# darioShar/DLPM

Hardware: AMD Instinct MI355X
Metric: samples/sec at T=1000 (CIFAR-10 32x32, alpha=1.7) (higher is better)
Workload: dtype f32 (1x1 / stride-2 convolutions: fp32 operands split exactly into 3 bf16 planes, bf16 MFMA products, fp32 accumulate)

## Files before the change

### dlpm_amd/_lib.py

```python
import ctypes as C
import os

_HERE = os.path.dirname(os.path.abspath(__file__))
LIB_PATH = os.environ.get('DLPM_LIB') or os.path.join(_HERE, 'lib', 'libdlpm_amd.so')

vp, i32, i64, u32, u64, f32, f64 = C.c_void_p, C.c_int32, C.c_int64, C.c_uint32, C.c_uint64, C.c_float, C.c_double

ABI_VERSION = 6
UPD_DLIM, UPD_CLIP, UPD_ADVANCE, SMP_NO_FUSED_MLP, UPD_ELEMENTWISE, SMP_LIM = 1, 2, 4, 8, 16, 32
MEAN_TYPES = {'EPSILON': 0, 'START_X': 1, 'Z': 2, 'PREVIOUS_X': 3}
PRED_TO_XSTART, PRED_CLIP, PRED_TO_EPS, PRED_ELEMENTWISE = 1, 2, 4, 16
CONV_AUTO, CONV_F4, CONV_F2, CONV_IGEMM = 0, 1, 2, 3
GEMM_AUTO, GEMM_F32, GEMM_BF16X3 = 0, 1, 2


class MT19937(C.Structure):
    _fields_ = [('key', u32 * 624), ('pos', i32), ('has_cached', i32), ('cached', f64)]


class UpdateArgs(C.Structure):
    _fields_ = [('x_dev', vp), ('eps_dev', vp), ('z_dev', vp), ('t_dev', vp), ('g_dev', vp), ('bg_dev', vp),
                ('bs_dev', vp), ('c_eps_dev', vp), ('c_noise_dev', vp), ('A_dev', vp), ('B', i64), ('D', i64),
                ('T', i32), ('flags', i32), ('dlim_eta', f32), ('alpha', f32), ('seed', u64), ('sample_offset', i64), ('key_dev', vp),
                ('hist_pp', vp)]


class PredictArgs(C.Structure):
    _fields_ = [('x_dev', vp), ('in_dev', vp), ('out_dev', vp), ('t_dev', vp), ('g_dev', vp), ('bg_dev', vp), ('bs_dev', vp),
                ('c_eps_dev', vp), ('A_dev', vp), ('B', i64), ('D', i64), ('T', i32), ('mean_type', i32), ('flags', i32)]


class LimUpdateArgs(C.Structure):
    _fields_ = [('x_dev', vp), ('eps_dev', vp), ('z_dev', vp), ('t_dev', vp), ('tmp_dev', vp), ('cx_dev', vp),
                ('cs_dev', vp), ('cn_dev', vp), ('A_dev', vp), ('B', i64), ('D', i64), ('T', i32), ('flags', i32),
                ('clamp_eps', f32), ('seed', u64), ('sample_offset', i64), ('key_dev', vp), ('hist_pp', vp)]


class UNetConfig(C.Structure):
    _fields_ = [('in_channels', i32), ('model_channels', i32), ('out_channels', i32), ('num_res_blocks', i32),
                ('num_heads', i32), ('image_size', i32), ('n_mult', i32), ('channel_mult', i32 * 8), ('n_attn', i32),
                ('attention_resolutions', i32 * 8)]


class ConvArgs(C.Structure):
    _fields_ = [('src0', vp), ('src1', vp), ('C0', i32), ('C1', i32), ('B', i32), ('Hin', i32), ('Win', i32),
                ('Hout', i32), ('Wout', i32), ('ksize', i32), ('stride', i32), ('upsample', i32), ('weight', vp),
                ('bias', vp), ('coefA', vp), ('coefB', vp), ('act_silu', i32), ('res0', vp), ('res1', vp), ('R0', i32),
                ('out', vp), ('Cout', i32), ('in_nchw', i32), ('out_nchw', i32), ('force_direct', i32), ('scratch_floats', i64)]


class ResBlockArgs(C.Structure):
    _fields_ = [('x0', vp), ('x1', vp), ('C0', i32), ('C1', i32), ('B', i32), ('H', i32), ('W', i32), ('gn1_w', vp), ('gn1_b', vp),
                ('conv1_w', vp), ('conv1_b', vp), ('ss', vp), ('ss_stride', i64), ('gn2_w', vp), ('gn2_b', vp), ('conv2_w', vp),
                ('conv2_b', vp), ('skip_w', vp), ('skip_b', vp), ('out', vp), ('stats_out', vp)]


class AttnBlockArgs(C.Structure):
    _fields_ = [('x', vp), ('C', i32), ('heads', i32), ('B', i32), ('H', i32), ('W', i32), ('gn_w', vp), ('gn_b', vp),
                ('qkv_w', vp), ('qkv_b', vp), ('proj_w', vp), ('proj_b', vp), ('out', vp), ('stats_out', vp)]


class SamplerConfig(C.Structure):
    _fields_ = [('unet', vp), ('mlp', vp), ('B', i64), ('C', i32), ('H', i32), ('W', i32), ('T', i32), ('alpha', f64),
                ('clamp_a', f64), ('clamp_eps', f64), ('flags', i32), ('dlim_eta', f32), ('seed', u64),
                ('sample_offset', i64), ('use_graph', i32), ('g', vp), ('bg', vp), ('s', vp), ('bs', vp),
                ('lim_ts', vp), ('lim_tmp', vp), ('lim_cx', vp), ('lim_cs', vp), ('lim_cn', vp), ('in_scale', vp),
                ('mean_type', i32)]


SIGNATURES = {
    'dlpm_last_error': (C.c_char_p, []),
    'dlpm_abi_version': (C.c_int, []),
    'dlpm_prof_enable': (C.c_int, [C.c_int]),
    'dlpm_prof_report': (C.c_int, [C.c_char_p, i64]),
    'dlpm_schedule_f32': (C.c_int, [C.c_int, f64, vp, vp, vp, vp]),
    'dlpm_schedule_exploding_f32': (C.c_int, [C.c_int, f64, vp, vp, vp, vp]),
    'dlpm_mt19937_seed': (C.c_int, [C.POINTER(MT19937), u32]),
    'dlpm_skewed_levy_host_f32': (C.c_int, [C.POINTER(MT19937), f64, i64, f64, vp]),
    'dlpm_randn_host_f32': (C.c_int, [C.POINTER(MT19937), i64, vp]),
    'dlpm_skewed_levy_philox_f32': (C.c_int, [vp, C.c_int, i64, f64, f64, u64, i64, vp]),
    'dlpm_skewed_levy_elem_philox_f32': (C.c_int, [vp, C.c_int, i64, i64, f64, f64, u64, i64, vp]),
    'dlpm_init_state_elem_philox_f32': (C.c_int, [vp, i64, i64, f64, f64, f32, u64, i64, vp]),
    'dlpm_init_state_philox_f32': (C.c_int, [vp, i64, i64, f64, f64, f32, u64, i64, vp]),
    'dlpm_coeff_tables_f32': (C.c_int, [vp, vp, vp, vp, C.c_int, i64, vp, vp, vp, vp]),
    'dlpm_update_f32': (C.c_int, [C.POINTER(UpdateArgs), vp]),
    'dlpm_predict_f32': (C.c_int, [C.POINTER(PredictArgs), vp]),
    'dlpm_fill_scaled_t_f32': (C.c_int, [vp, vp, i32, i64, vp]),
    'dlpm_postprocess_f32': (C.c_int, [vp, vp, i64, f32, C.c_int, vp]),
    'dlpm_scale_by_table_f32': (C.c_int, [vp, vp, i64, vp, vp, vp]),
    'dlpm_lim_tables_f32': (C.c_int, [f64, i32, i32, vp, vp, vp, vp, vp]),
    'dlpm_lim_update_f32': (C.c_int, [C.POINTER(LimUpdateArgs), vp]),
    'dlpm_fill_table_t_f32': (C.c_int, [vp, vp, vp, i32, i64, vp]),
    'dlpm_images_to_rgb8': (C.c_int, [vp, vp, i64, i32, i32, i32, vp]),
    'dlpm_png_bound': (i64, [i32, i32]),
    'dlpm_png_encode_rgb8': (C.c_int, [vp, i32, i32, i32, vp, i64, C.POINTER(i64)]),
    'dlpm_png_write_rgb8': (C.c_int, [vp, i64, i32, i32, C.c_char_p, i64, i32, i32]),
    'dlpm_unet_create': (C.c_int, [C.POINTER(UNetConfig), C.POINTER(vp)]),
    'dlpm_unet_set_param': (C.c_int, [vp, C.c_char_p, vp, i64]),
    'dlpm_unet_num_params': (C.c_int, [vp]),
    'dlpm_unet_param_key': (C.c_char_p, [vp, C.c_int, C.POINTER(i64)]),
    'dlpm_unet_finalize': (C.c_int, [vp]),
    'dlpm_unet_workspace_bytes': (i64, [vp, i64]),
    'dlpm_unet_forward': (C.c_int, [vp, vp, vp, vp, i64, vp, i64, vp]),
    'dlpm_unet_forward_uniform_t': (C.c_int, [vp, vp, vp, vp, i64, vp, i64, vp]),
    'dlpm_unet_forward_update': (C.c_int, [vp, vp, vp, C.POINTER(UpdateArgs), vp, i64, vp, i64, vp]),
    'dlpm_unet_time_embedding_width': (i64, [vp]),
    'dlpm_unet_time_embeddings_scratch_bytes': (i64, [vp, i64]),
    'dlpm_unet_time_embeddings': (C.c_int, [vp, vp, i64, vp, vp, i64, vp]),
    'dlpm_unet_bind_time_table': (C.c_int, [vp, vp, vp]),
    'dlpm_unet_keep_features': (C.c_int, [vp, C.c_int]),
    'dlpm_unet_num_features': (C.c_int, [vp]),
    'dlpm_unet_feature_shape': (C.c_int, [vp, C.c_int, C.POINTER(i32), C.POINTER(i32), C.POINTER(i32)]),
    'dlpm_unet_get_feature': (C.c_int, [vp, C.c_int, vp, i64, vp]),
    'dlpm_unet_flops_per_sample': (i64, [vp]),
    'dlpm_unet_set_conv_policy': (C.c_int, [vp, i32, i64]),
    'dlpm_unet_set_gemm_policy': (C.c_int, [vp, i32]),
    'dlpm_unet_plan_version': (i64, [vp]),
    'dlpm_unet_destroy': (None, [vp]),
    'dlpm_mlp_create': (C.c_int, [i32, i32, i32, i32, C.POINTER(vp)]),
    'dlpm_mlp_set_param': (C.c_int, [vp, C.c_char_p, vp, i64]),
    'dlpm_mlp_finalize': (C.c_int, [vp]),
    'dlpm_mlp_forward': (C.c_int, [vp, vp, vp, vp, i64, vp]),
    'dlpm_mlp_sample_steps_f32': (C.c_int, [vp, vp, vp, vp, vp, i32, i64, i32, i32, u64, i64, vp, vp]),
    'dlpm_mlp_destroy': (None, [vp]),
    'dlpm_conv2d_f32': (C.c_int, [C.POINTER(ConvArgs), vp, vp]),
    'dlpm_groupnorm_coeffs_f32': (C.c_int, [vp, vp, i32, i32, i32, i32, i32, vp, vp, vp, i64, i64, vp, vp, vp]),
    'dlpm_attention_f32': (C.c_int, [vp, vp, i32, i32, i32, i32, vp]),
    'dlpm_resblock_small_f32': (C.c_int, [C.POINTER(ResBlockArgs), vp, i64, vp]),
    'dlpm_resblock_img_f32': (C.c_int, [C.POINTER(ResBlockArgs), vp, i64, vp]),
    'dlpm_resblock_img_scratch_floats': (i64, [i64, i32]),
    'dlpm_attnblock_small_f32': (C.c_int, [C.POINTER(AttnBlockArgs), vp, i64, vp]),
    'dlpm_timestep_embedding_f32': (C.c_int, [vp, vp, i64, i32, vp]),
    'dlpm_nchw_to_nhwc_f32': (C.c_int, [vp, vp, i32, i32, i32, i32, vp]),
    'dlpm_nhwc_to_nchw_f32': (C.c_int, [vp, vp, i32, i32, i32, i32, vp]),
    'dlpm_sampler_create': (C.c_int, [C.POINTER(SamplerConfig), C.POINTER(vp)]),
    'dlpm_sampler_reseed': (C.c_int, [vp, u64, i64]),
    'dlpm_sampler_begin': (C.c_int, [vp, vp]),
    'dlpm_sampler_begin_injected': (C.c_int, [vp, vp, vp, vp]),
    'dlpm_sampler_set_state': (C.c_int, [vp, vp, i32, vp]),
    'dlpm_sampler_step_injected': (C.c_int, [vp, vp, vp]),
    'dlpm_sampler_steps': (C.c_int, [vp, i32, vp]),
    'dlpm_sampler_set_history': (C.c_int, [vp, vp, vp]),
    'dlpm_sampler_copy_state': (C.c_int, [vp, vp, vp]),
    'dlpm_sampler_state': (vp, [vp]),
    'dlpm_sampler_t': (i32, [vp]),
    'dlpm_sampler_table': (vp, [vp, C.c_int]),
    'dlpm_sampler_destroy': (None, [vp]),
}

_lib = None


class DlpmError(RuntimeError):
    pass


def lib():
    global _lib
    if _lib is None:
        if not os.path.exists(LIB_PATH):
            raise DlpmError('libdlpm_amd.so is missing at %s -- run `python -m dlpm_amd.build` '
                            '(or __graft_entry__.build()); there is no CPU fallback' % LIB_PATH)
        handle = C.CDLL(LIB_PATH)
        for name, (res, args) in SIGNATURES.items():
            fn = getattr(handle, name)
            fn.restype = res
            fn.argtypes = args
        got = handle.dlpm_abi_version()
        if got != ABI_VERSION:
            raise DlpmError('libdlpm_amd.so has ABI version %d, the Python mirror expects %d -- rebuild with '
                            '`python -m dlpm_amd.build`' % (got, ABI_VERSION))
        _lib = handle
    return _lib


def check(rc):
    if rc != 0:
        msg = lib().dlpm_last_error().decode('utf-8', 'replace')
        if rc == -1:
            raise ValueError(msg)
        raise DlpmError('[dlpm status %d] %s' % (rc, msg))


def stream_ptr():
    import torch
    return torch.cuda.current_stream().cuda_stream


def ptr(t):
    if t is None:
        return None
    import torch
    assert t.is_contiguous(), 'non-contiguous tensor crossing the C ABI'
    assert t.dtype in (torch.float32, torch.int32), t.dtype
    return t.data_ptr()
```

### dlpm_amd/csrc/conv.h

```cpp
#pragma once
#include "common.h"

namespace dlpm {

struct ConvLaunch {
    const float *src0 = nullptr, *src1 = nullptr;
    int C0 = 0, C1 = 0;
    int B = 0, Hin = 0, Win = 0, Hout = 0, Wout = 0;
    int ks = 1, stride = 1, ups = 0;
    const float *w = nullptr;
    const float *w_frag = nullptr;
    const float *w_wino = nullptr;
    const float *w_wino4 = nullptr;
    const float *w_wino4_n64 = nullptr, *w_wino4_n32 = nullptr;
    const void *w_split = nullptr;
    const float *w_small = nullptr;
    const float *w_taps = nullptr;
    const float *w_hfused = nullptr;
    const float *bias = nullptr;
    const float *coefA = nullptr, *coefB = nullptr;
    int act_silu = 0;
    const float *res0 = nullptr, *res1 = nullptr;
    int R0 = 0;
    float *out = nullptr;
    int Cout = 0;
    int in_nchw = 0, out_nchw = 0;
    int ws_gemm = 0;
    int abl = 0;
    int gen = 0;
    int64_t dispatch_B = 0;
    int gemm = 0;
    int ksplit = 0;
    int pers_total = 0;
    float2 *stats_out = nullptr;
#ifdef DLPM_PHASE_TIMING
    unsigned long long *phase = nullptr;
#endif
};

bool igemm_supported(const ConvLaunch &c);
int launch_conv_igemm(const ConvLaunch &c, hipStream_t st);
int launch_conv_direct(const ConvLaunch &c, hipStream_t st);
int launch_conv_stem(const ConvLaunch &c, hipStream_t st);
struct HeadUpdate {
    float *x = nullptr;
    const float *z = nullptr;
    const int32_t *t = nullptr;
    const float *g = nullptr, *c_eps = nullptr, *c_noise = nullptr;
    const uint64_t *key = nullptr;
    uint64_t seed = 0;
    int64_t sample_offset = 0;
    float *const *hist_pp = nullptr;
    float *eps_out = nullptr;
    int32_t T = 0;
    int64_t B = 0;
};
bool head_conv_ok(const ConvLaunch &c);
int launch_conv_head(const ConvLaunch &c, const HeadUpdate *hu, hipStream_t st);
int relayout_weight_head(const float *oihw_dev, float *dst_dev, int Cout, int Cin, hipStream_t st);
bool head_gemm_ok(const ConvLaunch &c);
int head_taps_rows(int Cout);
int64_t head_gemm_scratch_floats(const ConvLaunch &c);
int launch_conv_head_gemm(const ConvLaunch &c, const HeadUpdate *hu, float *P, hipStream_t st);
int relayout_weight_head_taps(const float *oihw_dev, float *dst_dev, int Cout, int Cin, hipStream_t st);
bool head_fused_ok(const ConvLaunch &c);
int64_t head_fused_weight_floats(int Cin);
int relayout_weight_head_fused(const float *oihw_dev, float *dst_dev, int Cout, int Cin, hipStream_t st);
int launch_conv_head_fused(const ConvLaunch &c, const HeadUpdate *hu, hipStream_t st);
bool wino_geometry(const ConvLaunch &c, int *bh, int *bw, int *nimg);
int wino_tiles(const ConvLaunch &c);
int launch_conv_wino(const ConvLaunch &c, hipStream_t st);
int64_t wino_weight_floats(int Cout, int Cin);
int relayout_weight_wino(const float *oihw_dev, float *dst_dev, int Cout, int Cin, hipStream_t st);
bool wino4_enabled();
bool wino4_vsplit();
bool wino4_image_stats(int cout);
bool wino4_geometry(const ConvLaunch &c, int *bh, int *bw, int *nimg);
bool wino4_preferred(const ConvLaunch &c, int *bh, int *bw, int *nimg);
int launch_conv_wino4(const ConvLaunch &c, hipStream_t st);
int64_t wino4_weight_floats(int Cout, int Cin);
int relayout_weight_wino4(const float *oihw_dev, float *dst_dev, int Cout, int Cin, hipStream_t st, int nq = 0);
struct ResImgLaunch {
    const float *x0 = nullptr, *x1 = nullptr;
    int C0 = 0, C1 = 0, B = 0;
    int H = 32;
    const float2 *st0 = nullptr, *st1 = nullptr;
    int nt0 = 1, nt1 = 1;
    const float *coefA1 = nullptr, *coefB1 = nullptr;
    const float *gn1_w = nullptr, *gn1_b = nullptr, *gn2_w = nullptr, *gn2_b = nullptr;
    const float *w1 = nullptr, *b1 = nullptr;
    const float *w2 = nullptr, *b2 = nullptr;
    const float *emb = nullptr;
    int64_t emb_stride = 0;
    int emb_off = 0;
    const float *res = nullptr;
    float *hbuf = nullptr;
    float *out = nullptr;
    float2 *stats_out = nullptr;
#ifdef DLPM_PHASE_TIMING
    unsigned long long *phase = nullptr;
#endif
};
bool res_img_ok(const ResImgLaunch &r);
int launch_resblock_img(const ResImgLaunch &r, hipStream_t st);

bool conv_split_ok(const ConvLaunch &c);
int launch_conv_split(const ConvLaunch &c, hipStream_t st);
int64_t split_weight_floats(int Cout, int Cin, int taps);
int relayout_weight_split(const float *oihw_dev, void *dst_dev, int Cout, int Cin, int taps, hipStream_t st);
int conv_stats_pixels(const ConvLaunch &c);
int conv_ksplit_for(const ConvLaunch &c);
int wino4_launch_nq(const ConvLaunch &c);
int64_t wino_grid_at(const ConvLaunch &c, int64_t B);
int wino_chunk_channels(const ConvLaunch &c);
int launch_splitk_reduce(const float *part, int S, int64_t npix, int Cout, const float *bias, const float *res0, const float *res1, int R0,
                         float *out, hipStream_t st);
inline int launch_conv_fallback(const ConvLaunch &L, hipStream_t st) {
    if (L.in_nchw && !L.out_nchw && L.ks == 3 && L.stride == 1 && !L.ups && L.C1 == 0 && L.Cout % 4 == 0 && !L.coefA &&
        !L.act_silu && !L.res0 && L.bias)
        return launch_conv_stem(L, st);
    return launch_conv_direct(L, st);
}

int relayout_weight(const float *oihw_dev, float *dst_dev, int Cout, int Cin, int ks, bool for_igemm, hipStream_t st);
int64_t frag_weight_floats(int Cout, int Cin, int taps = 9);
int relayout_weight_frag(const float *oihw_dev, float *dst_dev, int Cout, int Cin, hipStream_t st, int taps = 9);

int launch_gn_coeffs(const float *src0, const float *src1, int C0, int C1, int B, int HW, int groups,
                     const float *gamma, const float *beta, const float *ss, int64_t ss_stride, int64_t ss_offset,
                     float *coefA, float *coefB, hipStream_t st);
int launch_gn_coeffs_from_stats(const float2 *st0, const float2 *st1, int C0, int C1, int B, int nt0, int nt1, int HW, int groups,
                                const float *gamma, const float *beta, const float *ss, int64_t ss_stride,
                                int64_t ss_offset, float *coefA, float *coefB, hipStream_t st);
int launch_attention(const float *qkv, float *out, int B, int T, int C, int heads, hipStream_t st);

struct ResSmallLaunch {
    const float *x0 = nullptr, *x1 = nullptr;
    int C0 = 0, C1 = 0, B = 0, H = 0, W = 0;
    const float *gn1_w = nullptr, *gn1_b = nullptr, *gn2_w = nullptr, *gn2_b = nullptr;
    const float *w1f = nullptr, *b1 = nullptr;
    const float *w2f = nullptr, *b2 = nullptr;
    const float *wsf = nullptr, *bs = nullptr;
    const float *emb = nullptr;
    int64_t emb_stride = 0;
    int emb_off = 0;
    float *out = nullptr;
    float2 *stats_out = nullptr;
};
struct AttnSmallLaunch {
    const float *x = nullptr;
    int C = 0, heads = 0, B = 0, H = 0, W = 0;
    const float *gn_w = nullptr, *gn_b = nullptr;
    const float *wqkv = nullptr, *bqkv = nullptr;
    const float *wproj = nullptr, *bproj = nullptr;
    float *out = nullptr;
    float2 *stats_out = nullptr;
#ifdef DLPM_PHASE_TIMING
    unsigned long long *phase = nullptr;
#endif
};
bool attn_small_ok(const AttnSmallLaunch &a);
int launch_attnblock_small(const AttnSmallLaunch &a, hipStream_t st);
bool attn16_ok(const AttnSmallLaunch &a);
int launch_attnblock16(const AttnSmallLaunch &a, hipStream_t st);
bool gnqkv_small_ok(const AttnSmallLaunch &a);
int launch_gnqkv_small(const AttnSmallLaunch &a, hipStream_t st);
bool small_blocks_enabled();
bool small_weight_ok(int Cout, int Cin, int ks);
int64_t small_weight_floats(int Cout, int Cin, int ks);
int relayout_weight_small(const float *oihw_dev, float *dst_dev, int Cout, int Cin, int ks, hipStream_t st);
bool res_small_ok(const ResSmallLaunch &r);
int launch_resblock_small(const ResSmallLaunch &r, hipStream_t st);
int launch_timestep_embedding(const float *t, float *emb, int64_t B, int dim, hipStream_t st);

__device__ __forceinline__ float silu_f(float v) {
    return v * __builtin_amdgcn_rcpf(1.0f + __expf(-v));
}

}
```

### dlpm_amd/csrc/conv_igemm.hip

```cpp
#include <cstdlib>

#include <algorithm>

#include "conv.h"
#include "igemm_epilogue.h"

namespace dlpm {
namespace {

constexpr int KC = 32;
constexpr int LDS_LD = 36;

template <int BN, int WAVES_M, int WAVES_N, int RM, int RN>
__device__ __forceinline__ void epilogue_rows(const ConvLaunch &p, floatx16 (&acc)[RM][RN], float *lds, int64_t m0, int n0,
                                              int64_t M, int tid, int wm, int wn, int l31, int kh) {
    constexpr int LD = BN + 4, PR = RM * 32, C4 = BN / 4, RG = 256 / C4;
    const int R1 = p.Cout - p.R0;
    const bool do_stats = p.stats_out != nullptr;
    float4 K = make_float4(0.f, 0.f, 0.f, 0.f), s1 = K, s2 = K;
    int cnt = 0;
    for (int ph = 0; ph < WAVES_M; ph++) {
        if (wm == ph) {
#pragma unroll
            for (int i = 0; i < RM; i++)
// ... 719 lines not shown
    const float4 bias = reinterpret_cast<const float4 *>(p.bias)[nq];
    const int64_t m_lo = (int64_t)blockIdx.x * ppb;
    const bool do_stats = p.stats_out != nullptr;
    float4 K = make_float4(0.f, 0.f, 0.f, 0.f), s1 = K, s2 = K;
    for (int it = 0; it < ppb / pl_n; it++) {
        const int64_t m = m_lo + it * pl_n + pl;
        if (m >= M) break;
        const int b = (int)(m / HWo);
        const int rem = (int)(m - (int64_t)b * HWo);
        const int oy = rem / p.Wout, ox = rem - oy * p.Wout;
        float v[9 * CIN];
#pragma unroll
        for (int ky = 0; ky < 3; ky++)
#pragma unroll
            for (int kx = 0; kx < 3; kx++) {
                const int iy = oy + ky - 1, ix = ox + kx - 1;
                const bool ok = iy >= 0 && iy < p.Hin && ix >= 0 && ix < p.Win;
                const int cy = min(max(iy, 0), p.Hin - 1), cx = min(max(ix, 0), p.Win - 1);
#pragma unroll
                for (int c = 0; c < CIN; c++) {
                    const float x = p.src0[(((int64_t)b * CIN + c) * p.Hin + cy) * p.Win + cx];
                    v[(ky * 3 + kx) * CIN + c] = ok ? x : 0.f;
                }
            }
        float4 acc = bias;
#pragma unroll
        for (int k = 0; k < 9 * CIN; k++) {
            acc.x = fmaf(v[k], w[k].x, acc.x);
            acc.y = fmaf(v[k], w[k].y, acc.y);
            acc.z = fmaf(v[k], w[k].z, acc.z);
            acc.w = fmaf(v[k], w[k].w, acc.w);
        }
        reinterpret_cast<float4 *>(p.out + m * p.Cout)[nq] = acc;
        if (do_stats) {
            if (it == 0) K = acc;
            float d;
            d = acc.x - K.x; s1.x += d; s2.x = fmaf(d, d, s2.x);
            d = acc.y - K.y; s1.y += d; s2.y = fmaf(d, d, s2.y);
            d = acc.z - K.z; s1.z += d; s2.z = fmaf(d, d, s2.z);
            d = acc.w - K.w; s1.w += d; s2.w = fmaf(d, d, s2.w);
        }
    }
    if (do_stats) {
        __shared__ float2 part[1024];
        const float fc = (float)(ppb / pl_n);
        const float mx = s1.x / fc, my = s1.y / fc, mz = s1.z / fc, mw = s1.w / fc;
        part[pl * p.Cout + nq * 4 + 0] = make_float2(K.x + mx, fmaxf(s2.x - s1.x * mx, 0.f));
        part[pl * p.Cout + nq * 4 + 1] = make_float2(K.y + my, fmaxf(s2.y - s1.y * my, 0.f));
        part[pl * p.Cout + nq * 4 + 2] = make_float2(K.z + mz, fmaxf(s2.z - s1.z * mz, 0.f));
        part[pl * p.Cout + nq * 4 + 3] = make_float2(K.w + mw, fmaxf(s2.w - s1.w * mw, 0.f));
        __syncthreads();
        if ((int)threadIdx.x < p.Cout) {
            float mean = part[threadIdx.x].x, M2 = part[threadIdx.x].y, na = fc;
            for (int g = 1; g < pl_n; g++) {
                const float2 q = part[g * p.Cout + threadIdx.x];
                const float d = q.x - mean, N = na + fc;
                mean += d * (fc / N);
                M2 += q.y + d * d * (na * fc / N);
                na = N;
            }
            p.stats_out[(int64_t)blockIdx.x * p.Cout + threadIdx.x] = make_float2(mean, M2);
        }
    }
}

template <int CIN>
__global__ void __launch_bounds__(256) k_conv_stem_lds(ConvLaunch p, int ppb) {
    extern __shared__ __attribute__((aligned(16))) float4 patch[];
    const int Cq = p.Cout >> 2;
    const int pl_n = 256 / Cq;
    const int nq = threadIdx.x & (Cq - 1), pl = threadIdx.x / Cq;
    const int W = p.Wout, H = p.Hout, HWo = H * W, W2 = W + 2;
    const int rows = ppb / W, bpi = HWo / ppb;
    const int b = blockIdx.x / bpi, y0 = (blockIdx.x % bpi) * rows;
    float4 w[9 * CIN];
#pragma unroll
    for (int k = 0; k < 9 * CIN; k++) w[k] = reinterpret_cast<const float4 *>(p.w + (int64_t)k * p.Cout)[nq];
    const float4 bias = reinterpret_cast<const float4 *>(p.bias)[nq];
    const float *xb = p.src0 + (int64_t)b * CIN * HWo;
    for (int idx = threadIdx.x; idx < (rows + 2) * W2; idx += 256) {
        const int hy = idx / W2, hx = idx - hy * W2;
        const int iy = y0 + hy - 1, ix = hx - 1;
        float4 v = make_float4(0.f, 0.f, 0.f, 0.f);
        if ((unsigned)iy < (unsigned)H && (unsigned)ix < (unsigned)W) {
            const float *s = xb + iy * W + ix;
            v.x = s[0];
            if (CIN > 1) v.y = s[HWo];
            if (CIN > 2) v.z = s[2 * HWo];
        }
        patch[idx] = v;
    }
    __syncthreads();
    const bool do_stats = p.stats_out != nullptr;
    float4 K = make_float4(0.f, 0.f, 0.f, 0.f), s1 = K, s2 = K;
    const int lw = 31 - __builtin_clz(W);
    float *ob = p.out + ((int64_t)b * HWo + (int64_t)y0 * W) * p.Cout;
    for (int it = 0; it < ppb / pl_n; it++) {
        const int lp = it * pl_n + pl;
        const int ly = lp >> lw, lx = lp & (W - 1);
        const float4 *src = patch + ly * W2 + lx;
        float4 acc = bias;
#pragma unroll
        for (int ky = 0; ky < 3; ky++)
#pragma unroll
            for (int kx = 0; kx < 3; kx++) {
                const float4 t = src[ky * W2 + kx];
                const float v[3] = {t.x, t.y, t.z};
#pragma unroll
                for (int c = 0; c < CIN; c++) {
                    const float4 ww = w[(ky * 3 + kx) * CIN + c];
                    acc.x = fmaf(v[c], ww.x, acc.x);
                    acc.y = fmaf(v[c], ww.y, acc.y);
                    acc.z = fmaf(v[c], ww.z, acc.z);
                    acc.w = fmaf(v[c], ww.w, acc.w);
                }
            }
        reinterpret_cast<float4 *>(ob + (int64_t)lp * p.Cout)[nq] = acc;
        if (do_stats) {
            if (it == 0) K = acc;
            float d;
            d = acc.x - K.x; s1.x += d; s2.x = fmaf(d, d, s2.x);
            d = acc.y - K.y; s1.y += d; s2.y = fmaf(d, d, s2.y);
            d = acc.z - K.z; s1.z += d; s2.z = fmaf(d, d, s2.z);
            d = acc.w - K.w; s1.w += d; s2.w = fmaf(d, d, s2.w);
        }
    }
    if (do_stats) {
        __syncthreads();
        float2 *part = reinterpret_cast<float2 *>(patch);
        const float fc = (float)(ppb / pl_n);
        const float mx = s1.x / fc, my = s1.y / fc, mz = s1.z / fc, mw = s1.w / fc;
        part[pl * p.Cout + nq * 4 + 0] = make_float2(K.x + mx, fmaxf(s2.x - s1.x * mx, 0.f));
        part[pl * p.Cout + nq * 4 + 1] = make_float2(K.y + my, fmaxf(s2.y - s1.y * my, 0.f));
        part[pl * p.Cout + nq * 4 + 2] = make_float2(K.z + mz, fmaxf(s2.z - s1.z * mz, 0.f));
        part[pl * p.Cout + nq * 4 + 3] = make_float2(K.w + mw, fmaxf(s2.w - s1.w * mw, 0.f));
        __syncthreads();
        if ((int)threadIdx.x < p.Cout) {
            float mean = part[threadIdx.x].x, M2 = part[threadIdx.x].y, na = fc;
            for (int g = 1; g < pl_n; g++) {
                const float2 q = part[g * p.Cout + threadIdx.x];
                const float d = q.x - mean, N = na + fc;
                mean += d * (fc / N);
                M2 += q.y + d * d * (na * fc / N);
                na = N;
            }
            p.stats_out[(int64_t)blockIdx.x * p.Cout + threadIdx.x] = make_float2(mean, M2);
        }
    }
}

__global__ void k_relayout_weight(const float *oihw, float *dst, int Cout, int Cin, int ks, int for_igemm) {
    const int64_t n = (int64_t)Cout * Cin * ks * ks;
    int64_t i = (int64_t)blockIdx.x * blockDim.x + threadIdx.x;
    if (i >= n) return;
    const int taps = ks * ks;
    int tap = (int)(i % taps);
    int64_t r = i / taps;
    int ci = (int)(r % Cin);
    int co = (int)(r / Cin);
    int64_t d = for_igemm ? ((int64_t)tap * Cout + co) * Cin + ci : ((int64_t)tap * Cin + ci) * Cout + co;
    dst[d] = oihw[i];
}

}

bool igemm_supported(const ConvLaunch &c) {
    const int Cin = c.C0 + c.C1;
    if (c.in_nchw) return false;
    if (Cin % KC != 0 || c.C0 % KC != 0) return false;
    if (c.Cout < 16 && !c.out_nchw) return false;
    if (c.ks != 1 && c.ks != 3) return false;
    return true;
}

static bool ws_disabled() {
    static int v = -1;
    if (v < 0) { const char *e = getenv("DLPM_NO_WS"); v = (e && e[0] == '1') ? 1 : 0; }
    return v == 1;
}

static bool halo_ok(const ConvLaunch &c, int *th, int *nimg) {
    static int disabled = -1;
    if (disabled < 0) { const char *e = getenv("DLPM_NO_HALO"); disabled = (e && e[0] == '1') ? 1 : 0; }
    if (disabled || c.ks != 3 || c.stride != 1) return false;
    if (c.ups && (!c.w_frag || ws_disabled() || (c.Wout & 1) || (c.Hout & 1))) return false;
    const int W = c.Wout, HW = c.Hout * c.Wout;
    if (W < 4 || W > 64 || BM % W != 0) return false;
    if (HW >= BM) {
        if (HW % BM != 0) return false;
        *th = BM / W;
        *nimg = 1;
    } else {
        if (BM % HW != 0) return false;
        *th = c.Hout;
        *nimg = BM / HW;
    }
    if (c.ups && ((*th & 1) || (c.C0 + c.C1) % KC != 0 || c.abl)) return false;
    return *nimg * (*th + 2) * (W + 2) * 8 <= HALO_NIT * 256;
}

template <int BN, int WAVES_M, int WAVES_N, int RM, int RN, int RING, bool UPS, int TAPS = 9>
static int launch_halo_ws_r(const ConvLaunch &c, int th, int nimg, int64_t grid, hipStream_t st) {
    constexpr int PADW = TAPS == 9 ? 1 : 0;
    const int hp = nimg * ((UPS ? th / 2 : th) + 2 * PADW) * ((UPS ? c.Wout / 2 : c.Wout) + 2 * PADW);
    size_t shmem = (size_t)((hp + 3) & ~3) * LDS_LD * sizeof(float) + (size_t)nimg * 64 * sizeof(float);
    const size_t epi = (size_t)(RM * 32) * (BN + 4) * sizeof(float);
    const size_t stats = (size_t)(256 / (BN / 4)) * BN * 2 * sizeof(float);
    if (shmem < epi) shmem = epi;
    if (shmem < stats) shmem = stats;
    {
        int r = ensure_dynamic_lds(reinterpret_cast<const void *>(&k_conv3x3_halo_ws<BN, WAVES_M, WAVES_N, RM, RN, RING, UPS, TAPS>), 64 * 1024);
        if (r != DLPM_OK) return r;
    }
    k_conv3x3_halo_ws<BN, WAVES_M, WAVES_N, RM, RN, RING, UPS, TAPS><<<(unsigned)grid, 256, shmem, st>>>(c, th, nimg);
    return DLPM_OK;
}

template <int BN, int WAVES_M, int WAVES_N, int RM, int RN>
static int launch_halo_ws(const ConvLaunch &c, int th, int nimg, int64_t grid, hipStream_t st) {
    if (c.ups) return launch_halo_ws_r<BN, WAVES_M, WAVES_N, RM, RN, 2, true>(c, th, nimg, grid, st);
    return launch_halo_ws_r<BN, WAVES_M, WAVES_N, RM, RN, 2, false>(c, th, nimg, grid, st);
}

static bool gemm_ws_ok(const ConvLaunch &c, int *th, int *nimg) {
    if (!c.ws_gemm || ws_disabled() || !c.w_frag || c.ks != 1 || c.stride != 1 || c.ups || c.in_nchw || c.abl) return false;
    if ((c.C0 + c.C1) % KC != 0 || (c.C0 & 3) || c.Hin != c.Hout || c.Win != c.Wout) return false;
    const int W = c.Wout, HW = c.Hout * c.Wout;
    if (HW >= BM) {
        if (HW % BM != 0 || BM % W != 0) return false;
        *th = BM / W;
        *nimg = 1;
    } else {
        if (BM % HW != 0) return false;
        *th = c.Hout;
        *nimg = BM / HW;
        if (c.coefA && *nimg > 16) return false;
    }
    return true;
}

template <int BN, int WAVES_M, int WAVES_N, int RM, int RN>
static int launch_gemm_ws(const ConvLaunch &c, int th, int nimg, int64_t grid, hipStream_t st) {
    return launch_halo_ws_r<BN, WAVES_M, WAVES_N, RM, RN, 2, false, 1>(c, th, nimg, grid, st);
}

template <int BN, int WAVES_M, int WAVES_N, int RM, int RN>
static int launch_halo(const ConvLaunch &c, int th, int nimg, int64_t grid, hipStream_t st) {
    const int hp = nimg * (th + 2) * (c.Wout + 2);
    const size_t shmem = (size_t)(((hp + 3) & ~3) + 2 * BN) * LDS_LD * sizeof(float) + (size_t)nimg * 64 * sizeof(float);
    {
        int r = ensure_dynamic_lds(reinterpret_cast<const void *>(&k_conv3x3_halo<BN, WAVES_M, WAVES_N, RM, RN>), 100 * 1024);
        if (r != DLPM_OK) return r;
    }
    k_conv3x3_halo<BN, WAVES_M, WAVES_N, RM, RN><<<(unsigned)grid, 256, shmem, st>>>(c, th, nimg);
    return DLPM_OK;
}

static bool stem_stats_ok(const ConvLaunch &c) {
    const int Cq = c.Cout / 4;
    return c.in_nchw && !c.out_nchw && c.ks == 3 && c.stride == 1 && !c.ups && c.C1 == 0 && (c.C0 == 3 || c.C0 == 1) && c.Cout % 4 == 0 &&
           Cq >= 1 && Cq <= 256 && (Cq & (Cq - 1)) == 0 && ((int64_t)c.Hout * c.Wout) % 1024 == 0;
}

int launch_conv_stem(const ConvLaunch &c, hipStream_t st) {
    const int64_t total = (int64_t)c.B * c.Hout * c.Wout * (c.Cout / 4);
    ProfScope ps("conv_stem", 2.0 * total * 4 * c.C0 * 9, 4.0 * ((double)c.B * c.Hin * c.Win * c.C0 + total * 4.0), st);
    const int Cq = c.Cout / 4;
    const bool regw = Cq >= 1 && Cq <= 256 && (Cq & (Cq - 1)) == 0;
    const int64_t Mpix = (int64_t)c.B * c.Hout * c.Wout;
    const int ppb = 1024;
    if (c.stats_out && !stem_stats_ok(c)) {
        set_error("launch_conv_stem: statistics requested for a shape that cannot emit them");
        return DLPM_ERR_UNSUPPORTED;
    }
    static int nolds = -1;
    if (nolds < 0) { const char *e = getenv("DLPM_NO_STEM_LDS"); nolds = (e && e[0] == '1') ? 1 : 0; }
    const int W = c.Wout;
    const bool lds_ok = !nolds && regw && c.Hin == c.Hout && c.Win == c.Wout && (W & (W - 1)) == 0 && W >= 4 && W <= 64 && ppb % W == 0 &&
                        ((int64_t)c.Hout * W) % ppb == 0 && c.bias;
    if (lds_ok && (c.C0 == 3 || c.C0 == 1)) {
        const size_t shmem = std::max((size_t)(ppb / W + 2) * (W + 2) * sizeof(float4), (size_t)(256 / Cq) * c.Cout * sizeof(float2));
        if (c.C0 == 3) k_conv_stem_lds<3><<<(unsigned)(Mpix / ppb), 256, shmem, st>>>(c, ppb);
        else k_conv_stem_lds<1><<<(unsigned)(Mpix / ppb), 256, shmem, st>>>(c, ppb);
        DLPM_LAUNCH_CHECK();
        return DLPM_OK;
    }
    if (c.C0 == 3 && regw) k_conv_stem_regw<3><<<(unsigned)ceil_div(Mpix, ppb), 256, 0, st>>>(c, ppb);
    else if (c.C0 == 1 && regw) k_conv_stem_regw<1><<<(unsigned)ceil_div(Mpix, ppb), 256, 0, st>>>(c, ppb);
    else if (c.C0 == 3) k_conv_stem<3><<<(unsigned)ceil_div(total, 256), 256, 0, st>>>(c);
    else if (c.C0 == 1) k_conv_stem<1><<<(unsigned)ceil_div(total, 256), 256, 0, st>>>(c);
    else return launch_conv_direct(c, st);
    DLPM_LAUNCH_CHECK();
    return DLPM_OK;
}

int conv_stats_pixels(const ConvLaunch &c) {
    int a, b, n;
    if (conv_ksplit_for(c) > 1) return 0;
    if (c.in_nchw) return stem_stats_ok(c) ? 1024 : 0;
    if (conv_split_ok(c)) {
        const int64_t hw = (int64_t)c.Hout * c.Wout;
        return (c.R0 & 3) ? 0 : hw % BM == 0 ? BM : hw == 64 ? 64 : 0;
    }
    if (wino4_preferred(c, &a, &b, &n)) return n == 1 ? 256 : (n == 4 && a * b == 4 && wino4_image_stats(c.Cout)) ? 64 : 0;
    if (wino_geometry(c, &a, &b, &n)) return n == 1 ? 4 * wino_tiles(c) : 0;
    if (c.out_nchw || (c.Cout & 3) || (c.R0 & 3)) return 0;
    return ((int64_t)c.Hout * c.Wout) % BM == 0 ? BM : 0;
}

int launch_conv_igemm(const ConvLaunch &c, hipStream_t st) {
    const int64_t M = (int64_t)c.B * c.Hout * c.Wout;
    const int64_t mt = ceil_div(M, BM);
    const double K = (double)(c.C0 + c.C1) * c.ks * c.ks;
    const double bytes = 4.0 * ((double)c.B * c.Hin * c.Win * (c.C0 + c.C1) + K * c.Cout + (double)M * c.Cout * (c.res0 ? 2 : 1));
    char pname[96];
    int th = 0, nimg = 1;
    if (prof_enabled() && prof_detail())
        snprintf(pname, sizeof(pname), "conv%dx%d_igemm:H%d:Cin%d+%d:Cout%d:s%d:u%d:coef%d", c.ks, c.ks, c.Hout, c.C0, c.C1, c.Cout,
                 c.stride, c.ups, c.coefA ? 1 : 0);
    else
        snprintf(pname, sizeof(pname), "%s", c.ks == 3 ? (halo_ok(c, &th, &nimg) ? "conv3x3_halo" : "conv3x3_igemm") : "conv1x1_igemm");
    if (conv_split_ok(c)) {
        if (prof_enabled() && prof_detail())
            snprintf(pname, sizeof(pname), "conv%dx%d_bf16x3:H%d:Cin%d+%d:Cout%d:s%d:coef%d", c.ks, c.ks, c.Hout, c.C0, c.C1, c.Cout, c.stride,
                     c.coefA ? 1 : 0);
        else
            snprintf(pname, sizeof(pname), c.ks == 1 ? "conv1x1_bf16x3" : "conv3x3_bf16x3");
        ProfScope pss(pname, 2.0 * M * c.Cout * K, bytes + 2.0 * K * c.Cout, st);
#ifdef DLPM_PHASE_TIMING
        const_cast<ConvLaunch &>(c).phase = phase_buffer();
#endif
#ifdef DLPM_IGEMM_ABLATIONS
        { const char *e = getenv("DLPM_ABL"); if (e) const_cast<ConvLaunch &>(c).abl = atoi(e); }
#endif
        return launch_conv_split(c, st);
    }
    {
        int wb, ww, wi;
        if (wino4_preferred(c, &wb, &ww, &wi)) {
            if (prof_enabled() && prof_detail())
                snprintf(pname, sizeof(pname), "conv3x3_wino4:H%d:Cin%d+%d:Cout%d:u%d:coef%d", c.Hout, c.C0, c.C1, c.Cout, c.ups, c.coefA ? 1 : 0);
            else
                snprintf(pname, sizeof(pname), "conv3x3_wino4");
            ProfScope psw(pname, 2.0 * M * c.Cout * K, bytes, st);
            return launch_conv_wino4(c, st);
        }
        if (wino_geometry(c, &wb, &ww, &wi)) {
            if (prof_enabled() && prof_detail())
                snprintf(pname, sizeof(pname), "conv3x3_wino:H%d:Cin%d+%d:Cout%d:u%d:coef%d", c.Hout, c.C0, c.C1, c.Cout, c.ups, c.coefA ? 1 : 0);
            else
                snprintf(pname, sizeof(pname), "conv3x3_wino");
            ProfScope psw(pname, 2.0 * M * c.Cout * K, bytes, st);
            return launch_conv_wino(c, st);
        }
    }
    ProfScope ps(pname, 2.0 * M * c.Cout * K, bytes, st);
#ifdef DLPM_IGEMM_ABLATIONS
    static int abl = -1;
    if (abl < 0) { const char *e = getenv("DLPM_ABL"); abl = e ? atoi(e) : 0; }
    if (abl) const_cast<ConvLaunch &>(c).abl = abl;
#endif
#ifdef DLPM_PHASE_TIMING
    const_cast<ConvLaunch &>(c).phase = phase_buffer();
#endif
    if (gemm_ws_ok(c, &th, &nimg)) {
        int r;
        if (c.Cout > 64) r = launch_gemm_ws<128, 2, 2, 2, 2>(c, th, nimg, mt * ceil_div(c.Cout, 128), st);
        else if (c.Cout > 32) r = launch_gemm_ws<64, 2, 2, 2, 1>(c, th, nimg, mt * ceil_div(c.Cout, 64), st);
        else r = launch_gemm_ws<32, 4, 1, 1, 1>(c, th, nimg, mt * ceil_div(c.Cout, 32), st);
        if (r != DLPM_OK) return r;
        DLPM_LAUNCH_CHECK();
        return DLPM_OK;
    }
    if (halo_ok(c, &th, &nimg)) {
        int r;
        if (c.w_frag && !ws_disabled() && !c.abl && (c.C0 + c.C1) % KC == 0) {
            if (c.Cout > 64) r = launch_halo_ws<128, 2, 2, 2, 2>(c, th, nimg, mt * ceil_div(c.Cout, 128), st);
            else if (c.Cout > 32) r = launch_halo_ws<64, 2, 2, 2, 1>(c, th, nimg, mt * ceil_div(c.Cout, 64), st);
            else r = launch_halo_ws<32, 4, 1, 1, 1>(c, th, nimg, mt * ceil_div(c.Cout, 32), st);
            if (r != DLPM_OK) return r;
            DLPM_LAUNCH_CHECK();
            return DLPM_OK;
        }
        if (c.Cout > 64) r = launch_halo<128, 2, 2, 2, 2>(c, th, nimg, mt * ceil_div(c.Cout, 128), st);
        else if (c.Cout > 32) r = launch_halo<64, 2, 2, 2, 1>(c, th, nimg, mt * ceil_div(c.Cout, 64), st);
        else r = launch_halo<32, 4, 1, 1, 1>(c, th, nimg, mt * ceil_div(c.Cout, 32), st);
        if (r != DLPM_OK) return r;
        DLPM_LAUNCH_CHECK();
        return DLPM_OK;
    }
    static int nofast = -1;
    if (nofast < 0) { const char *e = getenv("DLPM_NO_FAST_IGEMM"); nofast = (e && e[0] == '1') ? 1 : 0; }
    const int bn = c.Cout > 64 ? 128 : c.Cout > 32 ? 64 : 32;
    const bool full = !nofast && !c.abl && M % BM == 0 && c.Cout % bn == 0 && !c.out_nchw && (c.R0 & 3) == 0;
    const bool g1 = full && c.ks == 1 && c.stride == 1 && !c.ups && !c.in_nchw && c.C0 % KC == 0 && (c.C0 + c.C1) % KC == 0;
    const int mode = g1 ? 2 : full ? 1 : 0;
    const unsigned grid = (unsigned)(mt * ceil_div(c.Cout, bn));
#define DLPM_IGEMM_LAUNCH(BN_, WM_, WN_, RM_, RN_)                                                   \
    do {                                                                                             \
        if (mode == 2) k_conv_igemm<BN_, WM_, WN_, RM_, RN_, 2><<<grid, 256, 0, st>>>(c);            \
        else if (mode == 1) k_conv_igemm<BN_, WM_, WN_, RM_, RN_, 1><<<grid, 256, 0, st>>>(c);       \
        else k_conv_igemm<BN_, WM_, WN_, RM_, RN_, 0><<<grid, 256, 0, st>>>(c);                      \
    } while (0)
    if (bn == 128) DLPM_IGEMM_LAUNCH(128, 2, 2, 2, 2);
    else if (bn == 64) DLPM_IGEMM_LAUNCH(64, 2, 2, 2, 1);
    else DLPM_IGEMM_LAUNCH(32, 4, 1, 1, 1);
#undef DLPM_IGEMM_LAUNCH
    DLPM_LAUNCH_CHECK();
    return DLPM_OK;
}

int64_t frag_weight_floats(int Cout, int Cin, int taps) {
    return ((int64_t)((Cout + 31) / 32) * (Cin / 32) * taps * 4 + 2) * 256;
}

int relayout_weight_frag(const float *oihw_dev, float *dst_dev, int Cout, int Cin, hipStream_t st, int taps) {
    const int64_t n = (int64_t)((Cout + 31) / 32) * (Cin / 32) * taps * 4 * 256;
    DLPM_HIP(hipMemsetAsync(dst_dev + n, 0, 2 * 256 * sizeof(float), st));
    k_relayout_weight_frag<<<(unsigned)ceil_div(n, 256), 256, 0, st>>>(oihw_dev, dst_dev, Cout, Cin, taps);
    DLPM_LAUNCH_CHECK();
    return DLPM_OK;
}

int relayout_weight(const float *oihw_dev, float *dst_dev, int Cout, int Cin, int ks, bool for_igemm, hipStream_t st) {
    const int64_t n = (int64_t)Cout * Cin * ks * ks;
    k_relayout_weight<<<(unsigned)ceil_div(n, 256), 256, 0, st>>>(oihw_dev, dst_dev, Cout, Cin, ks, for_igemm ? 1 : 0);
    DLPM_LAUNCH_CHECK();
    return DLPM_OK;
}

}
```

### dlpm_amd/csrc/conv_wino4.hip

```cpp
#include <cstdlib>
#include <type_traits>

#include "conv.h"
#include "gn_stats.h"

namespace dlpm {
namespace {

typedef float floatx4 __attribute__((ext_vector_type(4)));

constexpr int F4_TILES = 16;
constexpr int F4_NQ = 128;
constexpr int F4_KC = 8;
constexpr int F4_RAWPIX = 576;
constexpr int F4_PRLD = F4_KC + 4;
constexpr int F4_NT = 512;
constexpr int F4_QNIT = (F4_RAWPIX * 2 + F4_NT - 1) / F4_NT;
constexpr int F4_RAWBUF = F4_RAWPIX * F4_PRLD + 16;
constexpr int F4_RAWPIX_N = 400;
constexpr int F4_RAWBUF_N = F4_RAWPIX_N * F4_PRLD + 16;
constexpr int f4_nq_of(int cout) { return cout % 128 == 0 ? 128 : cout % 64 == 0 ? 64 : 32; }
constexpr int F4_CFS = 16 * 2 * F4_KC;
constexpr int F4_VBUF = 36 * F4_TILES * F4_KC;
#ifndef F4_RING_DEPTH
// ... 1272 lines not shown
    };
    int rbase, vofs;
    {
        const int cp = (wave >> 1) & 1, tile = lane & 15, pair = 4 * cp + (lane >> 4);
        const int ty = tile >> 2, tx = tile & 3;
        rbase = (4 * ty * F6_RW + 4 * tx) * F6_PRLD + pair * 2 + 4 * ty;
        vofs = (pair * F6_TILES + tile) * 4;
    }
    const int th = wave & 1;
    auto transform = [&]() __attribute__((always_inline)) {
        const float *rb = raw + rbase;
        float *vb = V + vofs;
        auto d = [&](int i, int c) {
            return *reinterpret_cast<const float2 *>(rb + (i * F6_RW + c) * F6_PRLD + (i >= 4 ? 4 : 0));
        };
        auto row_out = [&](const float2 (&T)[6], int a) {
            float *vr = vb + a * 3 * F6_VPP;
            const float2 e1 = f2fma(-PB2, T[2], T[4]), o1 = f2fma(-PB2, T[1], T[3]);
            const float2 e2 = f2fma(-PA2, T[2], T[4]), o2 = f2fma(-PA2, T[1], T[3]);
            const float2 v0 = f2fma(PP2, T[0], f2fma(-PS2, T[2], T[4])), v1 = f2fma(PA, o1, e1), v2 = f2fma(-PA, o1, e1);
            const float2 v3 = f2fma(PB, o2, e2), v4 = f2fma(-PB, o2, e2), v5 = f2fma(PP2, T[1], f2fma(-PS2, T[3], T[5]));
            *reinterpret_cast<float4 *>(vr + 0 * F6_VPP) = make_float4(v0.x, v0.y, v1.x, v1.y);
            *reinterpret_cast<float4 *>(vr + 1 * F6_VPP) = make_float4(v2.x, v2.y, v3.x, v3.y);
            *reinterpret_cast<float4 *>(vr + 2 * F6_VPP) = make_float4(v4.x, v4.y, v5.x, v5.y);
        };
        float2 Ta[6], Tb[6];
        if (th == 0) {
#pragma unroll
            for (int c = 0; c < 6; c++) {
                const float2 e = f2fma(-PB2, d(2, c), d(4, c)), o = f2fma(-PB2, d(1, c), d(3, c));
                Ta[c] = f2fma(PA, o, e);
                Tb[c] = f2fma(-PA, o, e);
            }
            row_out(Ta, 1);
            row_out(Tb, 2);
#pragma unroll
            for (int c = 0; c < 6; c++) Ta[c] = f2fma(PP2, d(0, c), f2fma(-PS2, d(2, c), d(4, c)));
            row_out(Ta, 0);
        } else {
#pragma unroll
            for (int c = 0; c < 6; c++) {
                const float2 e = f2fma(-PA2, d(2, c), d(4, c)), o = f2fma(-PA2, d(1, c), d(3, c));
                Ta[c] = f2fma(PB, o, e);
                Tb[c] = f2fma(-PB, o, e);
            }
            row_out(Ta, 3);
            row_out(Tb, 4);
#pragma unroll
            for (int c = 0; c < 6; c++) Tb[c] = f2fma(PP2, d(1, c), f2fma(-PS2, d(3, c), d(5, c)));
            row_out(Tb, 5);
        }
    };
    constexpr int AHEAD = F4_RING - 1;
    const float *asrc = V + ((4 * kh + lk) * F6_TILES + li) * 4;
    floatx4 acc[36];
    auto conv_pass = [&](const float *wfrag, int nch16, auto first_pass) __attribute__((always_inline)) {
        constexpr bool P1 = decltype(first_pass)::value;
        const int last = nch16 - 1;
        const float4 *__restrict__ wp = reinterpret_cast<const float4 *>(wfrag) + ((int64_t)nw * (2 * nch16) + kh) * 18 * 64;
        float4 bq[F4_RING];
#pragma unroll
        for (int q = 0; q < 36; q++)
#pragma unroll
            for (int r = 0; r < 4; r++) acc[q][r] = 0.f;
        store_raw(0, first_pass);
        F4_LDS_BARRIER();
#pragma unroll 1
        for (int chunk = 0; chunk < nch16; chunk++) {
            if (wave < 4) transform();
#pragma unroll
            for (int a = 0; a < AHEAD; a++) bq[a] = wp[a * 64 + lane];
            if (P1) load_raw(min(chunk + 1, last));
            F4_LDS_BARRIER();
            float4 aq[2];
            aq[0] = *reinterpret_cast<const float4 *>(asrc);
#pragma unroll
            for (int pp = 0; pp < 18; pp++) {
                if (pp + AHEAD < 18) bq[(pp + AHEAD) % F4_RING] = wp[(pp + AHEAD) * 64 + lane];
                if (pp + 1 < 18) aq[(pp + 1) & 1] = *reinterpret_cast<const float4 *>(asrc + (pp + 1) * F6_VPP);
                const float4 aa = aq[pp & 1];
                const float4 b = bq[pp % F4_RING];
                acc[2 * pp] = __builtin_amdgcn_mfma_f32_16x16x4f32(aa.x, b.x, acc[2 * pp], 0, 0, 0);
                acc[2 * pp + 1] = __builtin_amdgcn_mfma_f32_16x16x4f32(aa.z, b.z, acc[2 * pp + 1], 0, 0, 0);
                acc[2 * pp] = __builtin_amdgcn_mfma_f32_16x16x4f32(aa.y, b.y, acc[2 * pp], 0, 0, 0);
                acc[2 * pp + 1] = __builtin_amdgcn_mfma_f32_16x16x4f32(aa.w, b.w, acc[2 * pp + 1], 0, 0, 0);
            }
            wp += 2 * 18 * 64;
            if (chunk < last) store_raw(chunk + 1, first_pass);
            F4_LDS_BARRIER();
        }
    };
    auto exchange = [&](auto ra_c) __attribute__((always_inline)) {
        constexpr int RA = decltype(ra_c)::value, RO = 2 - RA;
        float2 *xb2 = reinterpret_cast<float2 *>(xb);
#pragma unroll
        for (int hh = 0; hh < 2; hh++) {
#pragma unroll
            for (int q = 0; q < 18; q++) xb2[(wave * 18 + q) * 64 + lane] = make_float2(acc[18 * hh + q][RO], acc[18 * hh + q][RO + 1]);
            F4_LDS_BARRIER();
#pragma unroll
            for (int q0 = 0; q0 < 18; q0 += 6) {
                float2 t[6];
#pragma unroll
                for (int q = 0; q < 6; q++) t[q] = xb2[((wave ^ 4) * 18 + q0 + q) * 64 + lane];
#pragma unroll
                for (int q = 0; q < 6; q++) {
                    acc[18 * hh + q0 + q][RA] += t[q].x;
                    acc[18 * hh + q0 + q][RA + 1] += t[q].y;
                }
                asm volatile("" ::: "memory");
            }
            F4_LDS_BARRIER();
        }
    };
    auto out_tile = [&](auto r_c, float (&Yt)[16]) __attribute__((always_inline)) {
        constexpr int r = decltype(r_c)::value;
        float Z[4][6];
#pragma unroll
        for (int b = 0; b < 6; b++) {
            const float m0 = acc[0 * 6 + b][r], m1 = acc[1 * 6 + b][r], m2 = acc[2 * 6 + b][r];
            const float m3 = acc[3 * 6 + b][r], m4 = acc[4 * 6 + b][r], m5 = acc[5 * 6 + b][r];
            const float s12 = m1 + m2, d12 = m1 - m2, s34 = m3 + m4, d34 = m3 - m4;
            Z[0][b] = m0 + s12 + s34;
            Z[1][b] = fmaf(PB, d34, PA * d12);
            Z[2][b] = fmaf(PB2, s34, PA2 * s12);
            Z[3][b] = fmaf(PB3, d34, PA3 * d12) + m5;
        }
#pragma unroll
        for (int i = 0; i < 4; i++) {
            const float s12 = Z[i][1] + Z[i][2], d12 = Z[i][1] - Z[i][2], s34 = Z[i][3] + Z[i][4], d34 = Z[i][3] - Z[i][4];
            Yt[i * 4 + 0] = Z[i][0] + s12 + s34;
            Yt[i * 4 + 1] = fmaf(PB, d34, PA * d12);
            Yt[i * 4 + 2] = fmaf(PB2, s34, PA2 * s12);
            Yt[i * 4 + 3] = fmaf(PB3, d34, PA3 * d12) + Z[i][5];
        }
    };
    auto half_stats = [&](float K, float s1, float s2, float &mean, float &M2) __attribute__((always_inline)) {
        mean = K + s1 * (1.f / 32.f);
        M2 = fmaxf(s2 - s1 * s1 * (1.f / 32.f), 0.f);
        float na = 32.f;
#pragma unroll
        for (int sft = 16; sft <= 32; sft <<= 1) {
            const float om = __shfl_xor(mean, sft), oM2 = __shfl_xor(M2, sft);
            const float lo_m = (lane & sft) ? om : mean, hi_m = (lane & sft) ? mean : om;
            const float lo_M = (lane & sft) ? oM2 : M2, hi_M = (lane & sft) ? M2 : oM2;
            const float dd = hi_m - lo_m;
            mean = lo_m + dd * 0.5f;
            M2 = lo_M + hi_M + dd * dd * (na * 0.5f);
            na *= 2.f;
        }
    };

    const int Cin = p.C0 + p.C1;
    load_raw(0);
    if (p.st0) {
        gn_coeffs_from_stats_image(p.st0 + (int64_t)img * p.nt0 * p.C0, p.st1 ? p.st1 + (int64_t)img * p.nt1 * p.C1 : nullptr, p.C0, p.C1, p.nt0,
                                   p.nt1, H * W, Cin < 32 ? Cin : 32, p.gn1_w, p.gn1_b, nullptr, gsh, Cf, Cf + 128, 1e-5f, tid, FI_NT,
                                   [] { F4_LDS_BARRIER(); });
    } else {
        for (int i = tid; i < 2 * Cin; i += FI_NT) {
            if (i < Cin) Cf[i] = p.coefA1[(int64_t)img * Cin + i];
            else Cf[128 + (i - Cin)] = p.coefB1[(int64_t)img * Cin + (i - Cin)];
        }
    }
    F4_LDS_BARRIER();
    conv_pass(p.w1, Cin / F6_KC, std::integral_constant<bool, true>());
    DLPM_PHASE(p, 8);

    auto between = [&](auto ra_c) __attribute__((always_inline)) {
        constexpr int RA = decltype(ra_c)::value;
        exchange(ra_c);
        int chv = ch, lkv = lk;
        asm volatile("" : "+v"(chv), "+v"(lkv));
        const float bias_v = p.b1[chv];
        float hv[2][16];
        float K = 0.f, s1 = 0.f, s2 = 0.f;
        {
            float Yt[16];
            out_tile(std::integral_constant<int, RA>(), Yt);
#pragma unroll
            for (int k = 0; k < 16; k++) {
                const float v = Yt[k] + bias_v;
                if (k == 0) K = v;
                const float dd = v - K;
                s1 += dd;
                s2 = fmaf(dd, dd, s2);
                hv[0][k] = v;
            }
            out_tile(std::integral_constant<int, RA + 1>(), Yt);
#pragma unroll
            for (int k = 0; k < 16; k++) {
                const float v = Yt[k] + bias_v;
                const float dd = v - K;
                s1 += dd;
                s2 = fmaf(dd, dd, s2);
                hv[1][k] = v;
            }
        }
        float mean, M2;
        half_stats(K, s1, s2, mean, M2);
        if (lkv == 0) part[kh * CO + chv] = make_float2(mean, M2);
        F4_LDS_BARRIER();
        gn_coeffs_from_stats_image(part, nullptr, CO, 0, 2, 1, H * W, 32, p.gn2_w, p.gn2_b, p.emb + (int64_t)img * p.emb_stride + p.emb_off, gsh, Cf,
                                   Cf + 128, 1e-5f, tid, FI_NT, [] { F4_LDS_BARRIER(); });
        F4_LDS_BARRIER();
        const float a2 = Cf[chv], b2 = Cf[128 + chv];
#pragma unroll
        for (int rr = 0; rr < 2; rr++) {
            const int tile = 4 * lkv + RA + rr;
            const int tpix = (4 * (tile >> 2)) * W + 4 * (tile & 3);
#pragma unroll
            for (int k = 0; k < 16; k++) hL[(tpix + (k >> 2) * W + (k & 3)) * F6_HLD + chv] = silu_f(fmaf(hv[rr][k], a2, b2));
        }
    };
    if (kh == 0) between(std::integral_constant<int, 0>());
    else between(std::integral_constant<int, 2>());
    F4_LDS_BARRIER();

    conv_pass(p.w2, CO / F6_KC, std::integral_constant<bool, false>());
    DLPM_PHASE(p, 9);
    auto epilogue = [&](auto ra_c) __attribute__((always_inline)) {
        constexpr int RA = decltype(ra_c)::value;
        exchange(ra_c);
        int chv = ch, lkv = lk;
        asm volatile("" : "+v"(chv), "+v"(lkv));
        const float bias_v = p.b2[chv];
        const int64_t pix0 = (int64_t)img * H * W;
        float *__restrict__ out_blk = p.out + pix0 * CO;
        const float *__restrict__ res_blk = p.res + pix0 * CO;
        const bool do_stats = p.stats_out != nullptr;
        float K = 0.f, s1 = 0.f, s2 = 0.f;
        auto one = [&](auto r_c, int rr) __attribute__((always_inline)) {
            const int tile = 4 * lkv + RA + rr;
            const int tpix = (4 * (tile >> 2)) * W + 4 * (tile & 3);
            float rs[16];
#pragma unroll
            for (int k = 0; k < 16; k++) rs[k] = res_blk[(tpix + (k >> 2) * W + (k & 3)) * CO + chv];
            float Yt[16];
            out_tile(r_c, Yt);
#pragma unroll
            for (int k = 0; k < 16; k++) {
                const float v = (Yt[k] + bias_v) + rs[k];
                if (rr == 0 && k == 0) K = v;
                const float dd = v - K;
                s1 += dd;
                s2 = fmaf(dd, dd, s2);
                out_blk[(tpix + (k >> 2) * W + (k & 3)) * CO + chv] = v;
            }
        };
        one(std::integral_constant<int, RA>(), 0);
        one(std::integral_constant<int, RA + 1>(), 1);
        if (do_stats) {
            float mean, M2;
            half_stats(K, s1, s2, mean, M2);
            if (lkv == 0) part[kh * CO + chv] = make_float2(mean, M2);
            F4_LDS_BARRIER();
            if (kh == 0 && lkv == 0) {
                const float2 a = part[chv], b = part[CO + chv];
                const float dd = b.x - a.x;
                p.stats_out[(int64_t)img * CO + chv] = make_float2(a.x + dd * 0.5f, a.y + b.y + dd * dd * 64.f);
            }
        }
    };
    if (kh == 0) epilogue(std::integral_constant<int, 0>());
    else epilogue(std::integral_constant<int, 2>());
    DLPM_PHASE(p, 10);
    DLPM_PHASE_FLUSH(p, 8);
#ifdef DLPM_PHASE_TIMING
    if (p.phase && tid == 0) atomicAdd(p.phase + 11, 1ull);
#endif
}

__global__ void k_relayout_weight_wino4(const float *oihw, float *dst, int Cout, int Cin, int vs, int nw) {
    const int nch = Cin / F4_KC;
    const int64_t total = (int64_t)Cout * Cin * 36;
    const int64_t i = (int64_t)blockIdx.x * blockDim.x + threadIdx.x;
    if (i >= total) return;
    const int e = (int)(i & 3);
    const int lane = (int)((i >> 2) & 63);
    int64_t r = i >> 8;
    const int pp = (int)(r % 18); r /= 18;
    const int chunk = (int)(r % nch); r /= nch;
    const int wave = (int)(r % nw);
    const int nt = (int)(r / nw);
    const int lk = lane >> 4, li = lane & 15;
    const int pos = vs ? 18 * (wave >> 2) + 2 * (pp >> 1) + (e >> 1) : 2 * pp + (e >> 1);
    const int cin = chunk * F4_KC + 2 * lk + (e & 1);
    const int cout = vs ? nt * F4_NQ + 32 * (wave & 3) + 16 * (pp & 1) + li : nt * (16 * nw) + wave * 16 + li;
    const float *g = oihw + ((int64_t)cout * Cin + cin) * 9;
    const double a = F4_PA, b = F4_PB, a2 = a * a, b2 = b * b;
    const double n0 = a2 * b2, na = 2. * a2 * (a2 - b2), nb = 2. * b2 * (b2 - a2);
    const double G[6][3] = {{1. / n0, 0., 0.},         {1. / na, a / na, a2 / na}, {1. / na, -a / na, a2 / na},
                            {1. / nb, b / nb, b2 / nb}, {1. / nb, -b / nb, b2 / nb}, {0., 0., 1.}};
    const int ra = pos / 6, rb = pos % 6;
    double u = 0.;
    for (int ii = 0; ii < 3; ii++) {
        double row = 0.;
        for (int jj = 0; jj < 3; jj++) row += (double)g[ii * 3 + jj] * G[rb][jj];
        u += G[ra][ii] * row;
    }
    dst[i] = (float)u;
}

int f4_mode() {
    static int v = -1;
    if (v < 0) { const char *e = getenv("DLPM_WINO_F4"); v = e ? atoi(e) : 1; }
    return v;
}

}

bool wino4_enabled() { return f4_mode() != 0; }
bool wino4_vsplit() {
    static int v = -1;
    if (v < 0) { const char *e = getenv("DLPM_WINO_VS"); v = e ? atoi(e) : 0; }
    return v != 0;
}
bool wino4_image_stats(int cout) { (void)cout; return F4_EPI_T == 0; }

static bool narrow_enabled() {
    static int v = -1;
    if (v < 0) { const char *e = getenv("DLPM_WINO4_NARROW"); v = e ? atoi(e) : 1; }
    return v != 0;
}

static bool wino4_geometry_nq(const ConvLaunch &c, int nq, int *bh, int *bw, int *nimg) {
    if (nq != F4_NQ && !narrow_enabled()) return false;
    if (!c.w_wino4 || c.ks != 3 || c.stride != 1 || c.in_nchw || c.out_nchw || c.abl) return false;
    if ((c.Hout & 3) || (c.Wout & 3) || c.Cout % 32 != 0 || (c.C0 + c.C1) % F4_KC != 0 || c.C0 % F4_KC != 0) return false;
    const int rawpix = nq == F4_NQ ? F4_RAWPIX : F4_RAWPIX_N;
    if ((c.R0 & 15) != 0) return false;
    const int TH = c.Hout / 4, TW = c.Wout / 4;
    int h, w, n;
    if (TH * TW >= F4_TILES) {
        w = TW < 4 ? TW : 4;
        if (F4_TILES % w != 0) return false;
        h = F4_TILES / w;
        if (TW % w != 0 || TH % h != 0) return false;
        n = 1;
    } else {
        if (F4_TILES % (TH * TW) != 0) return false;
        h = TH; w = TW; n = F4_TILES / (TH * TW);
    }
    const int RH = c.ups ? 2 * h + 2 : 4 * h + 2, RW = c.ups ? 2 * w + 2 : 4 * w + 2;
    if (n * RH * RW > rawpix) return false;
    *bh = h; *bw = w; *nimg = n;
    return true;
}

static int wino4_nq_for(const ConvLaunch &c) {
    const int base = f4_nq_of(c.Cout);
    if (base != F4_NQ || c.dispatch_B <= 0 || (!c.w_wino4_n64 && !c.w_wino4_n32)) return base;
    static int floor_nq = -1;
    if (floor_nq < 0) { const char *e = getenv("DLPM_WINO4_NQ"); floor_nq = e ? atoi(e) : 32; }
    int best = F4_NQ;
    for (int nq = F4_NQ; nq >= 32 && nq >= floor_nq; nq >>= 1) {
        if (nq == 64 && !c.w_wino4_n64) continue;
        if (nq == 32 && !c.w_wino4_n32) continue;
        int h, w, n;
        if (!wino4_geometry_nq(c, nq, &h, &w, &n)) continue;
        best = nq;
        const int64_t tiles = c.dispatch_B * (c.Hout / 4) * (c.Wout / 4);
        const int64_t mblocks = n == 1 ? tiles / F4_TILES : ceil_div(c.dispatch_B, (int64_t)n);
        if (mblocks * (c.Cout / nq) >= 256) break;
    }
    return best;
}

bool wino4_geometry(const ConvLaunch &c, int *bh, int *bw, int *nimg) { return wino4_geometry_nq(c, wino4_nq_for(c), bh, bw, nimg); }
int wino4_launch_nq(const ConvLaunch &c) { return wino4_nq_for(c); }

bool wino4_preferred(const ConvLaunch &c, int *bh, int *bw, int *nimg) {
    if (c.gen == DLPM_CONV_F2 || c.gen == DLPM_CONV_IGEMM) return false;
    if (!wino4_geometry(c, bh, bw, nimg)) return false;
    if (!c.w_wino || c.gen == DLPM_CONV_F4) return true;
    if (*nimg > 4) return false;
    if (c.dispatch_B <= 0) return true;
    const int64_t tiles = c.dispatch_B * (c.Hout / 4) * (c.Wout / 4);
    const int64_t mblocks = *nimg == 1 ? tiles / F4_TILES : ceil_div(c.dispatch_B, (int64_t)*nimg);
    return mblocks * (c.Cout / wino4_nq_for(c)) >= 256;
}

static bool wino4_whole_image(const ConvLaunch &c) {
    static int v = -1;
    if (v < 0) { const char *e = getenv("DLPM_WINO4_IMG"); v = e ? atoi(e) : 1; }
    return v != 0 && c.Cout == 32 && !c.ups && c.Hout == 32 && c.Wout == 32 && (c.C0 + c.C1) <= 1024;
}

static int launch_conv_wino4_nq(const ConvLaunch &c, int nq, int bh, int bw, int nimg, hipStream_t st);

int launch_conv_wino4(const ConvLaunch &c, hipStream_t st) {
    int bh, bw, nimg;
    if (!wino4_geometry(c, &bh, &bw, &nimg)) {
        set_error("launch_conv_wino4: unsupported shape");
        return DLPM_ERR_UNSUPPORTED;
    }
#ifdef DLPM_PHASE_TIMING
    const_cast<ConvLaunch &>(c).phase = phase_buffer();
#endif
    const int nq = wino4_nq_for(c);
    if (nq != f4_nq_of(c.Cout)) {
        ConvLaunch cn = c;
        cn.w_wino4 = nq == 64 ? c.w_wino4_n64 : c.w_wino4_n32;
        cn.w_wino4_n64 = cn.w_wino4_n32 = nullptr;
        cn.dispatch_B = 0;
        return launch_conv_wino4_nq(cn, nq, bh, bw, nimg, st);
    }
    return launch_conv_wino4_nq(c, nq, bh, bw, nimg, st);
}

static int launch_conv_wino4_nq(const ConvLaunch &c, int nq, int bh, int bw, int nimg, hipStream_t st) {
    using KFn = void (*)(ConvLaunch, int, int, int);
    const int64_t tiles = (int64_t)c.B * (c.Hout / 4) * (c.Wout / 4);
    const int64_t mblocks = nimg == 1 ? tiles / F4_TILES : ceil_div(c.B, nimg);
    if (wino4_whole_image(c)) {
        const int r = ensure_dynamic_lds(reinterpret_cast<const void *>(&k_conv3x3_wino4_img), 160 * 1024);
        if (r != DLPM_OK) return r;
        const size_t lds = (size_t)(FI_VBUF + FI_RAWBUF + 2 * (c.C0 + c.C1)) * sizeof(float);
        k_conv3x3_wino4_img<<<(unsigned)c.B, FI_NT, lds, st>>>(c);
        DLPM_LAUNCH_CHECK();
        return DLPM_OK;
    }
    if (nq != F4_NQ) {
        KFn fn = nq == 64 ? (c.ups ? &k_conv3x3_wino4<true, 0, 2, 0, 0, 4> : &k_conv3x3_wino4<false, 0, 2, 0, 0, 4>)
                          : (c.ups ? &k_conv3x3_wino4<true, 0, 4, 0, 0, 2> : &k_conv3x3_wino4<false, 0, 4, 0, 0, 2>);
        const int r = ensure_dynamic_lds(reinterpret_cast<const void *>(fn), 160 * 1024);
        if (r != DLPM_OK) return r;
        const size_t lds = (size_t)(2 * F4_VBUF + 2 * F4_RAWBUF_N + 2 * F4_CFS) * sizeof(float);
        const int ks = c.ksplit > 1 ? c.ksplit : 1;
        if (ks > 1 && (c.bias || c.res0 || c.stats_out || ((c.C0 + c.C1) / F4_KC) % ks != 0)) {
            set_error("launch_conv_wino4: a split-K launch carries no bias / residual / statistics and divides its chunks evenly");
            return DLPM_ERR_ARG;
        }
        fn<<<(unsigned)(mblocks * (c.Cout / nq) * ks), (nq == 64 ? 7 : 4) * 64, lds, st>>>(c, bh, bw, nimg);
        DLPM_LAUNCH_CHECK();
        return DLPM_OK;
    }
    if (c.ksplit > 1) {
        set_error("launch_conv_wino4: split-K is a narrow-shape launch");
        return DLPM_ERR_ARG;
    }
    const int RHp = c.ups ? 2 * bh + 2 : 4 * bh + 2, RWp = c.ups ? 2 * bw + 2 : 4 * bw + 2;
    const bool small = nimg * RHp * RWp <= F4_NT;
    KFn fn = c.ups ? (small ? &k_conv3x3_wino4<true, 0, 2> : &k_conv3x3_wino4<true>) : (small ? &k_conv3x3_wino4<false, 0, 2> : &k_conv3x3_wino4<false>);
    if (wino4_vsplit()) fn = c.ups ? (small ? &k_conv3x3_wino4<true, 0, 2, 0, 1> : &k_conv3x3_wino4<true, 0, F4_QNIT, 0, 1>)
                                   : (small ? &k_conv3x3_wino4<false, 0, 2, 0, 1> : &k_conv3x3_wino4<false, 0, F4_QNIT, 0, 1>);
    static int spec_on = -1;
    if (spec_on < 0) { const char *e = getenv("DLPM_WINO_SPEC"); spec_on = e ? atoi(e) : 0; }
    if (spec_on && !wino4_vsplit() && !c.ups && c.Hout == 32 && c.Wout == 32 && c.C0 == 128 && c.C1 == 0 && c.Cout == 128 && c.coefA && c.coefB && c.bias &&
        c.act_silu && bh == 4 && bw == 4 && nimg == 1 && !c.res1 && (!c.res0 || c.R0 == 128))
        fn = c.res0 ? &k_conv3x3_wino4<false, 0, 2, 2> : &k_conv3x3_wino4<false, 0, 2, 1>;

#ifdef DLPM_WINO_ABLATIONS
    static int abl = -1;
    if (abl < 0) { const char *e = getenv("DLPM_WABL"); abl = e ? atoi(e) : 0; }
    if (!c.ups && small) {
        switch (abl) {
            case 1: fn = &k_conv3x3_wino4<false, 1, 2>; break;
            case 2: fn = &k_conv3x3_wino4<false, 2, 2>; break;
            case 3: fn = &k_conv3x3_wino4<false, 3, 2>; break;
            case 7: fn = &k_conv3x3_wino4<false, 7, 2>; break;
            case 8: fn = &k_conv3x3_wino4<false, 8, 2>; break;
            case 16: fn = &k_conv3x3_wino4<false, 16, 2>; break;
            case 32: fn = &k_conv3x3_wino4<false, 32, 2>; break;
            case 64: fn = &k_conv3x3_wino4<false, 64, 2>; break;
            case 80: fn = &k_conv3x3_wino4<false, 80, 2>; break;
            case 87: fn = &k_conv3x3_wino4<false, 87, 2>; break;
            default: break;
        }
    }
#endif
    {
        int r = ensure_dynamic_lds(reinterpret_cast<const void *>(fn), 160 * 1024);
        if (r != DLPM_OK) return r;
    }
    size_t loop_b = (size_t)(2 * F4_VBUF + 2 * F4_RAWBUF + 2 * F4_CFS) * sizeof(float);
    if (wino4_vsplit() && loop_b < (size_t)8 * 4 * 16 * 64 * sizeof(float)) loop_b = (size_t)8 * 4 * 16 * 64 * sizeof(float);
    const int64_t total = mblocks * (c.Cout / F4_NQ);
    static int pers = -1, ncu = 0;
    if (pers < 0) {
        const char *e = getenv("DLPM_WINO4_PERSIST"); pers = e ? atoi(e) : 0;
        int dev = 0; hipDeviceProp_t pr;
        if (hipGetDevice(&dev) == hipSuccess && hipGetDeviceProperties(&pr, dev) == hipSuccess) ncu = pr.multiProcessorCount;
    }
    if (pers && ncu > 0 && total > 2 * ncu && !wino4_vsplit() && fn == (c.ups ? (small ? (KFn)&k_conv3x3_wino4<true, 0, 2> : (KFn)&k_conv3x3_wino4<true>)
                                                                            : (small ? (KFn)&k_conv3x3_wino4<false, 0, 2> : (KFn)&k_conv3x3_wino4<false>))) {
        KFn pf = c.ups ? (small ? &k_conv3x3_wino4<true, 0, 2, 0, 0, 8, 1> : &k_conv3x3_wino4<true, 0, F4_QNIT, 0, 0, 8, 1>)
                       : (small ? &k_conv3x3_wino4<false, 0, 2, 0, 0, 8, 1> : &k_conv3x3_wino4<false, 0, F4_QNIT, 0, 0, 8, 1>);
        const int r = ensure_dynamic_lds(reinterpret_cast<const void *>(pf), 160 * 1024);
        if (r != DLPM_OK) return r;
        ConvLaunch cp = c;
        cp.pers_total = (int)total;
        pf<<<(unsigned)ncu, F4_NT, loop_b, st>>>(cp, bh, bw, nimg);
        DLPM_LAUNCH_CHECK();
        return DLPM_OK;
    }
    fn<<<(unsigned)total, F4_NT, loop_b, st>>>(c, bh, bw, nimg);
    DLPM_LAUNCH_CHECK();
    return DLPM_OK;
}

bool res_img_ok(const ResImgLaunch &r) {
    static int v = -1;
    if (v < 0) { const char *e = getenv("DLPM_RES_IMG"); v = e ? atoi(e) : 1; }
    const int Cin = r.C0 + r.C1;
    const bool common = v != 0 && wino4_enabled() && r.w1 && r.w2 && r.res && Cin <= 128 && Cin >= 32 &&
                        (r.st0 ? (r.C1 == 0 || r.st1 != nullptr) : (r.coefA1 && r.coefB1));
    if (r.H == 16) {
        static int v16 = -1;
        if (v16 < 0) { const char *e = getenv("DLPM_RES_IMG16"); v16 = e ? atoi(e) : 1; }
        return common && v16 != 0 && Cin % F6_KC == 0 && r.C0 % F6_KC == 0;
    }
    return common && r.H == 32 && r.hbuf && Cin % F4_KC == 0 && r.C0 % F4_KC == 0;
}

int launch_resblock_img(const ResImgLaunch &r, hipStream_t st) {
    if (!res_img_ok(r)) {
        set_error("launch_resblock_img: unsupported block");
        return DLPM_ERR_UNSUPPORTED;
    }
    const int Cin = r.C0 + r.C1;
#ifdef DLPM_PHASE_TIMING
    const_cast<ResImgLaunch &>(r).phase = phase_buffer();
#endif
    if (r.H == 16) {
        const double M16 = (double)r.B * 256;
        ProfScope ps16("resblock_img:H16", 2.0 * M16 * 64 * 9.0 * (Cin + 64), 4.0 * (M16 * (Cin + 64 + 64) + 64 * 9.0 * (Cin + 64)), st);
        const int e16 = ensure_dynamic_lds(reinterpret_cast<const void *>(&k_resblock_wino4_img16), 160 * 1024);
        if (e16 != DLPM_OK) return e16;
        const size_t lds16 = (size_t)(F6_VBUF + F6_RAWBUF + F6_HBUF + 256 + 512 + 256 + F6_QN * FI_NT) * sizeof(float);
        k_resblock_wino4_img16<<<(unsigned)r.B, FI_NT, lds16, st>>>(r);
        DLPM_LAUNCH_CHECK();
        return DLPM_OK;
    }
    const double M = (double)r.B * 1024;
    ProfScope ps("resblock_img:H32", 2.0 * M * 32 * 9.0 * (Cin + 32), 4.0 * (M * (Cin + 32 + 32) + 32 * 9.0 * (Cin + 32)), st);
    const int e = ensure_dynamic_lds(reinterpret_cast<const void *>(&k_resblock_wino4_img), 160 * 1024);
    if (e != DLPM_OK) return e;
    const size_t lds = (size_t)(FI_VBUF + FI_RAWBUF + 256 + 512 + 256 + FI_QN * FI_NT) * sizeof(float);
    k_resblock_wino4_img<<<(unsigned)r.B, FI_NT, lds, st>>>(r);
    DLPM_LAUNCH_CHECK();
    return DLPM_OK;
}

int64_t wino4_weight_floats(int Cout, int Cin) { return (int64_t)Cout * Cin * 36 + F4_PAD * 256; }

int relayout_weight_wino4(const float *oihw_dev, float *dst_dev, int Cout, int Cin, hipStream_t st, int nq_in) {
    const int64_t n = (int64_t)Cout * Cin * 36;
    DLPM_HIP(hipMemsetAsync(dst_dev + n, 0, (size_t)F4_PAD * 256 * sizeof(float), st));
    const int nq = nq_in > 0 ? nq_in : f4_nq_of(Cout);
    k_relayout_weight_wino4<<<(unsigned)ceil_div(n, 256), 256, 0, st>>>(oihw_dev, dst_dev, Cout, Cin, (nq == F4_NQ && wino4_vsplit()) ? 1 : 0, nq / 16);
    DLPM_LAUNCH_CHECK();
    return DLPM_OK;
}

}
```

### dlpm_amd/csrc/unet.hip

```cpp
#include <cmath>
#include <cstdlib>
#include <map>
#include <string>
#include <utility>
#include <vector>

#include "conv.h"

using namespace dlpm;

namespace {

struct Param {
    std::string key;
    int64_t numel = 0;
    float *dev = nullptr;
    bool set = false;
};

enum LayerKind { L_STEM, L_RES, L_ATTN, L_DOWN, L_UP };

struct ConvW {
    int p_w = -1, p_b = -1;
    int cout = 0, cin = 0, ks = 1;
    bool use_igemm = false;
    float *w_dev = nullptr;
    float *w_frag = nullptr;
    float *w_wino = nullptr;
    float *w_wino4 = nullptr;
    float *w_wino4_n64 = nullptr, *w_wino4_n32 = nullptr;
    float *w_small = nullptr;
    float *w_taps = nullptr;
    void *w_split = nullptr;
    float *w_rs = nullptr;
    float *w_hfused = nullptr;
    bool owns = false;
};

struct Layer {
    LayerKind kind;
    std::string pre;
    int cin = 0, cout = 0;
    int emb_off = 0;
    ConvW c1, c2, skip;
    bool has_skip = false;
    int p_gn1_w = -1, p_gn1_b = -1, p_gn2_w = -1, p_gn2_b = -1;
    int p_emb_w = -1, p_emb_b = -1;
};

struct Tensor4 {
    float *p = nullptr;
    int C = 0, H = 0, W = 0;
    float2 *stats = nullptr;
    int stats_px = 0;
};

struct Bump {
    char *base = nullptr;
    int64_t cap = 0, off = 0, peak = 0;
    bool dry = false, overflow = false, reuse = true;
    std::vector<std::pair<int64_t, int64_t>> holes;
    std::map<int64_t, int64_t> live;
    char *origin() const { return dry ? reinterpret_cast<char *>(uintptr_t(1) << 20) : base; }
    float *alloc(int64_t nfloats) {
        const int64_t bytes = (nfloats * 4 + 255) / 256 * 256;
        int64_t at = -1;
        if (reuse) {
            size_t best = holes.size();
            for (size_t i = 0; i < holes.size(); i++)
                if (holes[i].second >= bytes && (best == holes.size() || holes[i].second < holes[best].second)) best = i;
            if (best != holes.size()) {
                at = holes[best].first;
                if (holes[best].second == bytes) holes.erase(holes.begin() + best);
                else { holes[best].first += bytes; holes[best].second -= bytes; }
            }
        }
        if (at < 0) {
            at = off;
            off += bytes;
            if (off > peak) peak = off;
            if (!dry && off > cap) overflow = true;
        }
        live[at] = bytes;
        return reinterpret_cast<float *>(origin() + at);
    }
    void release(const void *p) {
        if (!p || !reuse) return;
        const int64_t at = reinterpret_cast<const char *>(p) - origin();
        auto it = live.find(at);
        if (it == live.end()) return;
        int64_t lo = at, n = it->second;
        live.erase(it);
        size_t i = 0;
        while (i < holes.size() && holes[i].first < lo) i++;
        if (i > 0 && holes[i - 1].first + holes[i - 1].second == lo) { lo = holes[i - 1].first; n += holes[i - 1].second; holes.erase(holes.begin() + --i); }
        if (i < holes.size() && lo + n == holes[i].first) { n += holes[i].second; holes.erase(holes.begin() + i); }
        if (lo + n == off) { off = lo; return; }
        holes.insert(holes.begin() + i, std::make_pair(lo, n));
    }
};

void policy_of(const dlpm_unet *u, ConvLaunch &L);

void plan_stats(const dlpm_unet *u, Bump &ws, Tensor4 &t, const ConvW &c, int B, int C0, int stride, int ups, bool stem = false) {
    static int off = -1;
    if (off < 0) { const char *e = getenv("DLPM_NO_GN_FUSION"); off = (e && e[0] == '1') ? 1 : 0; }
    t.stats = nullptr;
    t.stats_px = 0;
    if (off || (!c.use_igemm && !stem)) return;
    ConvLaunch L;
    L.w_wino = c.w_wino; L.w_wino4 = c.w_wino4; L.w_wino4_n64 = c.w_wino4_n64; L.w_wino4_n32 = c.w_wino4_n32; L.w_split = c.w_split; L.ks = c.ks; L.stride = stride; L.ups = ups; L.Hout = t.H; L.Wout = t.W; L.Cout = c.cout;
    L.Hin = ups ? t.H / 2 : t.H * stride; L.Win = ups ? t.W / 2 : t.W * stride;
    L.C0 = C0; L.C1 = c.cin - C0; L.B = B;
    L.in_nchw = stem ? 1 : 0;
    policy_of(u, L);
    const int px = conv_stats_pixels(L);
    if (px <= 0) return;
    t.stats_px = px;
    t.stats = reinterpret_cast<float2 *>(ws.alloc((int64_t)2 * B * (t.H * t.W / px) * t.C));
}

int gn_any(Tensor4 x0, Tensor4 x1, int B, int groups, const float *gamma, const float *beta, const float *ss,
           int64_t ss_stride, int64_t ss_offset, float *cA, float *cB, hipStream_t st) {
    const int HW = x0.H * x0.W;
    if (x0.stats && (x1.C == 0 || x1.stats))
        return launch_gn_coeffs_from_stats(x0.stats, x1.stats, x0.C, x1.C, B, HW / x0.stats_px, x1.C ? HW / x1.stats_px : 1, HW,
                                           groups, gamma, beta, ss, ss_stride, ss_offset, cA, cB, st);
    return launch_gn_coeffs(x0.p, x1.p, x0.C, x1.C, B, HW, groups, gamma, beta, ss, ss_stride, ss_offset, cA, cB, st);
}


void drop(Bump &ws, Tensor4 &t) {
    ws.release(t.p);
    ws.release(t.stats);
    t.p = nullptr;
    t.stats = nullptr;
}

}

struct dlpm_unet {
    dlpm_unet_config cfg;
    std::vector<Param> params;
    std::map<std::string, int> index;
    std::vector<std::vector<Layer>> in_blocks, out_blocks;
    std::vector<Layer> mid;
    std::vector<int> skip_ch;
    ConvW te0, te2, embcat, head;
    int p_head_gn_w = -1, p_head_gn_b = -1;
    float *embcat_w = nullptr, *embcat_b = nullptr;
    int emb_total = 0, ted = 0, final_ch = 0;
    bool finalized = false;
    std::vector<Tensor4> feats;
    int64_t flops = 0;
    bool keep_feats = false;
    int gen = DLPM_CONV_AUTO;
    int64_t dispatch_B = 0;
    int gemm = DLPM_GEMM_AUTO;
    int64_t plan_version = 0;

    int add(const std::string &key, int64_t numel) {
        Param p;
        p.key = key;
        p.numel = numel;
        params.push_back(p);
        index[key] = (int)params.size() - 1;
        return (int)params.size() - 1;
    }
    ConvW conv(const std::string &pre, int cout, int cin, int ks) {
        ConvW c;
        c.cout = cout; c.cin = cin; c.ks = ks;
        c.p_w = add(pre + "weight", (int64_t)cout * cin * ks * ks);
        c.p_b = add(pre + "bias", cout);
        return c;
    }
    Layer res(const std::string &pre, int cin, int cout) {
        Layer L;
        L.kind = L_RES; L.pre = pre; L.cin = cin; L.cout = cout;
        L.p_gn1_w = add(pre + "in_layers.0.weight", cin);
        L.p_gn1_b = add(pre + "in_layers.0.bias", cin);
        L.c1 = conv(pre + "in_layers.2.", cout, cin, 3);
        L.p_emb_w = add(pre + "emb_layers.1.weight", (int64_t)2 * cout * ted);
        L.p_emb_b = add(pre + "emb_layers.1.bias", 2 * cout);
        L.p_gn2_w = add(pre + "out_layers.0.weight", cout);
        L.p_gn2_b = add(pre + "out_layers.0.bias", cout);
        L.c2 = conv(pre + "out_layers.3.", cout, cout, 3);
        L.has_skip = cin != cout;
        if (L.has_skip) L.skip = conv(pre + "skip_connection.", cout, cin, 1);
        L.emb_off = emb_total;
        emb_total += 2 * cout;
        return L;
    }
    Layer attn(const std::string &pre, int ch) {
        Layer L;
        L.kind = L_ATTN; L.pre = pre; L.cin = L.cout = ch;
        L.p_gn1_w = add(pre + "norm.weight", ch);
        L.p_gn1_b = add(pre + "norm.bias", ch);
        L.c1 = conv(pre + "qkv.", 3 * ch, ch, 1);
        L.c2 = conv(pre + "proj_out.", ch, ch, 1);
        return L;
    }
    bool has_attn(int ds) const {
        for (int i = 0; i < cfg.n_attn; i++)
            if (cfg.attention_resolutions[i] == ds) return true;
        return false;
    }
};

namespace {

void policy_of(const dlpm_unet *u, ConvLaunch &L) {
    L.gen = u->gen;
    L.dispatch_B = u->dispatch_B;
    L.gemm = u->gemm;
}

void build_arch(dlpm_unet *u) {
    const dlpm_unet_config &c = u->cfg;
    const int mc = c.model_channels;
    u->ted = 4 * mc;
    u->te0 = u->conv("time_embed.0.", u->ted, mc, 1);
    u->te2 = u->conv("time_embed.2.", u->ted, u->ted, 1);
    {
        Layer L;
        L.kind = L_STEM; L.pre = "input_blocks.0.0."; L.cin = c.in_channels; L.cout = mc;
        L.c1 = u->conv(L.pre, mc, c.in_channels, 3);
        u->in_blocks.push_back({L});
        u->skip_ch.push_back(mc);
    }
    int ch = mc, ds = 1;
    for (int level = 0; level < c.n_mult; level++) {
        const int mult = c.channel_mult[level];
        for (int r = 0; r < c.num_res_blocks; r++) {
            const std::string pre = "input_blocks." + std::to_string(u->in_blocks.size()) + ".";
            std::vector<Layer> seq;
            seq.push_back(u->res(pre + "0.", ch, mult * mc));
            ch = mult * mc;
            if (u->has_attn(ds)) seq.push_back(u->attn(pre + "1.", ch));
            u->in_blocks.push_back(seq);
            u->skip_ch.push_back(ch);
        }
        if (level != c.n_mult - 1) {
            Layer L;
            L.kind = L_DOWN; L.pre = "input_blocks." + std::to_string(u->in_blocks.size()) + ".0.op.";
            L.cin = L.cout = ch;
            L.c1 = u->conv(L.pre, ch, ch, 3);
            u->in_blocks.push_back({L});
            u->skip_ch.push_back(ch);
            ds *= 2;
        }
    }
    u->mid.push_back(u->res("middle_block.0.", ch, ch));
    u->mid.push_back(u->attn("middle_block.1.", ch));
    u->mid.push_back(u->res("middle_block.2.", ch, ch));
    std::vector<int> stack = u->skip_ch;
    for (int level = c.n_mult - 1; level >= 0; level--) {
        const int mult = c.channel_mult[level];
        for (int i = 0; i <= c.num_res_blocks; i++) {
            const std::string pre = "output_blocks." + std::to_string(u->out_blocks.size()) + ".";
            const int ich = stack.back();
            stack.pop_back();
            std::vector<Layer> seq;
            seq.push_back(u->res(pre + "0.", ch + ich, mc * mult));
            ch = mc * mult;
            int k = 1;
            if (u->has_attn(ds)) seq.push_back(u->attn(pre + std::to_string(k++) + ".", ch));
            if (level && i == c.num_res_blocks) {
                Layer L;
                L.kind = L_UP; L.pre = pre + std::to_string(k++) + ".conv.";
                L.cin = L.cout = ch;
                L.c1 = u->conv(L.pre, ch, ch, 3);
                seq.push_back(L);
                ds /= 2;
            }
            u->out_blocks.push_back(seq);
        }
    }
    u->final_ch = ch;
    u->p_head_gn_w = u->add("out.0.weight", ch);
    u->p_head_gn_b = u->add("out.0.bias", ch);
    u->head = u->conv("out.2.", c.out_channels, mc, 3);
}

bool ws_gemm_enabled() {
    static int v = -1;
    if (v < 0) { const char *e = getenv("DLPM_WS1X1"); v = (e && e[0] == '1') ? 1 : 0; }
    return v == 1;
}

int prep_conv(dlpm_unet *u, ConvW &c, int C0, int boundary) {
    ConvLaunch probe;
    probe.C0 = C0; probe.C1 = c.cin - C0; probe.Cout = c.cout; probe.ks = c.ks;
    probe.in_nchw = boundary == 1; probe.out_nchw = boundary == 2;
    c.use_igemm = igemm_supported(probe);
    const float *src = u->params[c.p_w].dev;
    if (c.use_igemm && c.ks == 1) {
        c.w_dev = const_cast<float *>(src);
        if (small_weight_ok(c.cout, c.cin, 1) && boundary == 0) {
            DLPM_HIP(hipMalloc(&c.w_rs, (size_t)small_weight_floats(c.cout, c.cin, 1) * sizeof(float)));
            int r = relayout_weight_small(src, c.w_rs, c.cout, c.cin, 1, nullptr);
            if (r != DLPM_OK) return r;
        }
        if (c.cout % 128 == 0 && c.cin % 32 == 0 && boundary == 0) {
            DLPM_HIP(hipMalloc(&c.w_split, (size_t)split_weight_floats(c.cout, c.cin, 1) * sizeof(float)));
            int r = relayout_weight_split(src, c.w_split, c.cout, c.cin, 1, nullptr);
            if (r != DLPM_OK) return r;
        }
        if (ws_gemm_enabled() && c.cin % 32 == 0 && boundary == 0) {
            DLPM_HIP(hipMalloc(&c.w_frag, (size_t)frag_weight_floats(c.cout, c.cin, 1) * sizeof(float)));
            return relayout_weight_frag(src, c.w_frag, c.cout, c.cin, nullptr, 1);
        }
        return DLPM_OK;
    }
    DLPM_HIP(hipMalloc(&c.w_dev, (size_t)c.cout * c.cin * c.ks * c.ks * sizeof(float)));
    c.owns = true;
    if (c.ks == 3 && c.cout <= 4 && c.cin % 32 == 0) {
        DLPM_HIP(hipMalloc(&c.w_small, (size_t)9 * c.cin * 4 * sizeof(float)));
        int r = relayout_weight_head(src, c.w_small, c.cout, c.cin, nullptr);
        if (r != DLPM_OK) return r;
        if (c.cout <= 3) {
            DLPM_HIP(hipMalloc(&c.w_taps, (size_t)head_taps_rows(c.cout) * c.cin * sizeof(float)));
            r = relayout_weight_head_taps(src, c.w_taps, c.cout, c.cin, nullptr);
            if (r != DLPM_OK) return r;
            if (c.cin <= 128) {
                DLPM_HIP(hipMalloc(&c.w_hfused, (size_t)head_fused_weight_floats(c.cin) * sizeof(float)));
                r = relayout_weight_head_fused(src, c.w_hfused, c.cout, c.cin, nullptr);
                if (r != DLPM_OK) return r;
            }
        }
    }
    if (c.use_igemm && c.ks == 3 && boundary == 4 && c.cout % 128 == 0 && c.cin % 32 == 0) {
        DLPM_HIP(hipMalloc(&c.w_split, (size_t)split_weight_floats(c.cout, c.cin, 9) * sizeof(float)));
        int r = relayout_weight_split(src, c.w_split, c.cout, c.cin, 9, nullptr);
        if (r != DLPM_OK) return r;
    }
    if (c.use_igemm && c.ks == 3 && c.cin % 32 == 0) {
        DLPM_HIP(hipMalloc(&c.w_frag, (size_t)frag_weight_floats(c.cout, c.cin) * sizeof(float)));
        int r = relayout_weight_frag(src, c.w_frag, c.cout, c.cin, nullptr);
        if (r != DLPM_OK) return r;
        if (c.cout % 64 == 0 && c.cin % 16 == 0 && boundary == 0) {
            DLPM_HIP(hipMalloc(&c.w_wino, (size_t)wino_weight_floats(c.cout, c.cin) * sizeof(float)));
            r = relayout_weight_wino(src, c.w_wino, c.cout, c.cin, nullptr);
            if (r != DLPM_OK) return r;
        }
        if (wino4_enabled() && c.cout % 32 == 0 && c.cin % 8 == 0 && boundary == 0) {
            DLPM_HIP(hipMalloc(&c.w_wino4, (size_t)wino4_weight_floats(c.cout, c.cin) * sizeof(float)));
            r = relayout_weight_wino4(src, c.w_wino4, c.cout, c.cin, nullptr);
            if (r != DLPM_OK) return r;
        }
    }
    if (small_weight_ok(c.cout, c.cin, c.ks) && boundary == 0) {
        DLPM_HIP(hipMalloc(&c.w_rs, (size_t)small_weight_floats(c.cout, c.cin, c.ks) * sizeof(float)));
        int r = relayout_weight_small(src, c.w_rs, c.cout, c.cin, c.ks, nullptr);
        if (r != DLPM_OK) return r;
    }
    return relayout_weight(src, c.w_dev, c.cout, c.cin, c.ks, c.use_igemm, nullptr);
}

void attach_conv(const dlpm_unet *u, const ConvW &c, ConvLaunch &L) {
    policy_of(u, L);
    L.w = c.w_dev;
    L.w_frag = c.w_frag;
    L.w_wino = c.w_wino;
    L.w_wino4 = c.w_wino4;
    L.w_wino4_n64 = c.w_wino4_n64;
    L.w_wino4_n32 = c.w_wino4_n32;
    L.w_small = c.w_small;
    L.w_taps = c.w_taps;
    L.w_hfused = c.w_hfused;
    L.w_split = c.w_split;
    L.ws_gemm = (c.ks == 1 && c.w_frag) ? 1 : 0;
    L.ks = c.ks;
    L.Cout = c.cout;
}

int run_conv(const dlpm_unet *u, const ConvW &c, ConvLaunch L, hipStream_t st, const HeadUpdate *hu = nullptr, float *head_scratch = nullptr) {
    policy_of(u, L);
    L.w = c.w_dev;
    L.w_frag = c.w_frag;
    L.w_wino = c.w_wino;
    L.w_wino4 = c.w_wino4;
    L.w_wino4_n64 = c.w_wino4_n64;
    L.w_wino4_n32 = c.w_wino4_n32;
    L.w_small = c.w_small;
    L.w_taps = c.w_taps;
    L.w_hfused = c.w_hfused;
    L.w_split = c.w_split;
    L.ws_gemm = (c.ks == 1 && c.w_frag) ? 1 : 0;
    L.ks = c.ks;
    L.Cout = c.cout;
    if (head_fused_ok(L)) return launch_conv_head_fused(L, hu, st);
    if (head_scratch && head_gemm_ok(L)) return launch_conv_head_gemm(L, hu, head_scratch, st);
    if (head_conv_ok(L)) return launch_conv_head(L, hu, st);
    if (hu) { set_error("unet: the head convolution of this net cannot carry the fused update"); return DLPM_ERR_UNSUPPORTED; }
    return c.use_igemm ? launch_conv_igemm(L, st) : launch_conv_fallback(L, st);
}

#define TRY(expr)                  \
    do {                           \
        int _r = (expr);           \
        if (_r != DLPM_OK) return _r; \
    } while (0)

struct Ctx {
    dlpm_unet *u;
    int B;
    Bump ws;
    hipStream_t st;
    float *embout = nullptr;
    bool uniform_t = false;
    const HeadUpdate *hu = nullptr;
    bool dry() const { return ws.dry; }
};

int ksplit_of(const Ctx &cx, const ConvW &c, ConvLaunch L) {
    attach_conv(cx.u, c, L);
    L.bias = nullptr;
    return conv_ksplit_for(L);
}
int run_conv3(Ctx &cx, const ConvW &c, const ConvLaunch &L) {
    const int S = ksplit_of(cx, c, L);
    if (S <= 1) return run_conv(cx.u, c, L, cx.st);
    const int64_t npix = (int64_t)L.B * L.Hout * L.Wout;
    float *part = cx.ws.alloc((int64_t)S * npix * c.cout);
    ConvLaunch P = L;
    P.bias = nullptr; P.res0 = nullptr; P.res1 = nullptr; P.R0 = 0; P.stats_out = nullptr; P.out = part; P.ksplit = S;
    int rc = run_conv(cx.u, c, P, cx.st);
    if (rc == DLPM_OK) rc = launch_splitk_reduce(part, S, npix, c.cout, L.bias, L.res0, L.res1, L.R0, L.out, cx.st);
    cx.ws.release(part);
    return rc;
}
void reserve_ksplit(Ctx &cx, const ConvW &c, const ConvLaunch &L) {
    const int S = ksplit_of(cx, c, L);
    if (S > 1) cx.ws.release(cx.ws.alloc((int64_t)S * L.B * L.Hout * L.Wout * c.cout));
}

void release_res_temps(Ctx &cx, float *cA1, float *cB1, Tensor4 &h1, float *cA2, float *cB2, float *sk) {
    cx.ws.release(cA1);
    cx.ws.release(cB1);
    drop(cx.ws, h1);
    cx.ws.release(cA2);
    cx.ws.release(cB2);
    cx.ws.release(sk);
}

int run_res(Ctx &cx, const Layer &L, Tensor4 x0, Tensor4 x1, Tensor4 *out) {
    dlpm_unet *u = cx.u;
    const int B = cx.B, H = x0.H, W = x0.W, HW = H * W;
    const int C0 = x0.C, C1 = x1.C, Cin = C0 + C1, Co = L.cout;
    {
        ResSmallLaunch r;
        r.x0 = x0.p; r.x1 = x1.p; r.C0 = C0; r.C1 = C1; r.B = B; r.H = H; r.W = W;
        r.w1f = L.c1.w_rs; r.w2f = L.c2.w_rs; r.wsf = L.has_skip ? L.skip.w_rs : nullptr;
        if (u->gen == DLPM_CONV_AUTO && Co == 64 && (!L.has_skip || r.wsf) && res_small_ok(r)) {
            float *o = cx.ws.alloc((int64_t)B * HW * Co);
            out->p = o; out->C = Co; out->H = H; out->W = W;
            out->stats = reinterpret_cast<float2 *>(cx.ws.alloc((int64_t)2 * B * Co));
            out->stats_px = HW;
            if (cx.dry()) return DLPM_OK;
            r.gn1_w = u->params[L.p_gn1_w].dev; r.gn1_b = u->params[L.p_gn1_b].dev;
            r.gn2_w = u->params[L.p_gn2_w].dev; r.gn2_b = u->params[L.p_gn2_b].dev;
            r.b1 = u->params[L.c1.p_b].dev; r.b2 = u->params[L.c2.p_b].dev;
            r.bs = L.has_skip ? u->params[L.skip.p_b].dev : nullptr;
            r.emb = cx.embout; r.emb_stride = cx.uniform_t ? 0 : u->emb_total; r.emb_off = L.emb_off;
            r.out = o; r.stats_out = out->stats;
            return launch_resblock_small(r, cx.st);
        }
    }
    if (u->gen == DLPM_CONV_AUTO && ((Co == 32 && H == 32 && W == 32) || (Co == 64 && H == 16 && W == 16)) && L.c1.w_wino4 && L.c2.w_wino4) {
        ResImgLaunch r;
        r.x0 = x0.p; r.x1 = x1.p; r.C0 = C0; r.C1 = C1; r.B = B; r.H = H;
        const bool from_stats = x0.stats && (C1 == 0 || x1.stats);
        r.w1 = L.c1.w_wino4; r.w2 = L.c2.w_wino4;
        float *cA1 = from_stats ? nullptr : cx.ws.alloc((int64_t)B * Cin), *cB1 = from_stats ? nullptr : cx.ws.alloc((int64_t)B * Cin);
        float *sk = L.has_skip ? cx.ws.alloc((int64_t)B * HW * Co) : nullptr;
        float *hb = H == 32 ? cx.ws.alloc((int64_t)B * HW * Co) : nullptr;
        float *o = cx.ws.alloc((int64_t)B * HW * Co);
        r.hbuf = hb; r.res = L.has_skip ? sk : x0.p;
        if (from_stats) {
            r.st0 = x0.stats; r.nt0 = HW / x0.stats_px;
            if (C1) { r.st1 = x1.stats; r.nt1 = HW / x1.stats_px; }
        } else {
            r.coefA1 = cA1; r.coefB1 = cB1;
        }
        if ((L.has_skip || C1 == 0) && res_img_ok(r)) {
            out->p = o; out->C = Co; out->H = H; out->W = W;
            plan_stats(cx.u, cx.ws, *out, L.c2, B, Co, 1, 0);
            auto done = [&]() { cx.ws.release(cA1); cx.ws.release(cB1); cx.ws.release(sk); cx.ws.release(hb); };
            if (cx.dry()) { done(); return DLPM_OK; }
            if (!from_stats)
                TRY(gn_any(x0, x1, B, Cin < 32 ? Cin : 32, u->params[L.p_gn1_w].dev, u->params[L.p_gn1_b].dev, nullptr, 0, 0, cA1, cB1, cx.st));
            if (L.has_skip) {
                ConvLaunch s;
                s.src0 = x0.p; s.src1 = x1.p; s.C0 = C0; s.C1 = C1; s.B = B; s.Hin = s.Hout = H; s.Win = s.Wout = W;
                s.bias = u->params[L.skip.p_b].dev; s.out = sk;
                TRY(run_conv(u, L.skip, s, cx.st));
            }
            r.gn1_w = u->params[L.p_gn1_w].dev; r.gn1_b = u->params[L.p_gn1_b].dev;
            r.gn2_w = u->params[L.p_gn2_w].dev; r.gn2_b = u->params[L.p_gn2_b].dev;
            r.b1 = u->params[L.c1.p_b].dev; r.b2 = u->params[L.c2.p_b].dev;
            r.emb = cx.embout; r.emb_stride = cx.uniform_t ? 0 : u->emb_total; r.emb_off = L.emb_off;
            r.out = o; r.stats_out = out->stats;
            TRY(launch_resblock_img(r, cx.st));
            done();
            return DLPM_OK;
        }
        cx.ws.release(cA1); cx.ws.release(cB1); cx.ws.release(sk); cx.ws.release(hb); cx.ws.release(o);
    }
    float *cA1 = cx.ws.alloc((int64_t)B * Cin), *cB1 = cx.ws.alloc((int64_t)B * Cin);
    Tensor4 h1;
    h1.C = Co; h1.H = H; h1.W = W;
    h1.p = cx.ws.alloc((int64_t)B * HW * Co);
    plan_stats(cx.u, cx.ws, h1, L.c1, B, C0, 1, 0);
    float *cA2 = cx.ws.alloc((int64_t)B * Co), *cB2 = cx.ws.alloc((int64_t)B * Co);
    float *sk = L.has_skip ? cx.ws.alloc((int64_t)B * HW * Co) : nullptr;
    float *o = cx.ws.alloc((int64_t)B * HW * Co);
    out->p = o; out->C = Co; out->H = H; out->W = W;
    plan_stats(cx.u, cx.ws, *out, L.c2, B, Co, 1, 0);
    if (cx.dry()) {
        ConvLaunch g;
        g.C0 = C0; g.C1 = C1; g.B = B; g.Hin = g.Hout = H; g.Win = g.Wout = W;
        reserve_ksplit(cx, L.c1, g);
        g.C0 = Co; g.C1 = 0;
        reserve_ksplit(cx, L.c2, g);
        release_res_temps(cx, cA1, cB1, h1, cA2, cB2, sk);
        return DLPM_OK;
    }
    const int G1 = Cin < 32 ? Cin : 32, G2 = Co < 32 ? Co : 32;
    TRY(gn_any(x0, x1, B, G1, u->params[L.p_gn1_w].dev, u->params[L.p_gn1_b].dev, nullptr, 0, 0, cA1, cB1, cx.st));
    ConvLaunch a;
    a.src0 = x0.p; a.src1 = x1.p; a.C0 = C0; a.C1 = C1; a.B = B; a.Hin = a.Hout = H; a.Win = a.Wout = W;
    a.bias = u->params[L.c1.p_b].dev; a.coefA = cA1; a.coefB = cB1; a.act_silu = 1; a.out = h1.p; a.stats_out = h1.stats;
    TRY(run_conv3(cx, L.c1, a));
    TRY(gn_any(h1, Tensor4(), B, G2, u->params[L.p_gn2_w].dev, u->params[L.p_gn2_b].dev, cx.embout,
               cx.uniform_t ? 0 : u->emb_total, L.emb_off, cA2, cB2, cx.st));
    ConvLaunch b;
    b.src0 = h1.p; b.C0 = Co; b.B = B; b.Hin = b.Hout = H; b.Win = b.Wout = W;
    b.bias = u->params[L.c2.p_b].dev; b.coefA = cA2; b.coefB = cB2; b.act_silu = 1; b.out = o; b.stats_out = out->stats;
    if (L.has_skip) {
        ConvLaunch s;
        s.src0 = x0.p; s.src1 = x1.p; s.C0 = C0; s.C1 = C1; s.B = B; s.Hin = s.Hout = H; s.Win = s.Wout = W;
        s.bias = u->params[L.skip.p_b].dev; s.out = sk;
        TRY(run_conv(u, L.skip, s, cx.st));
        b.res0 = sk; b.R0 = Co;
    } else {
        b.res0 = x0.p; b.res1 = x1.p; b.R0 = C0;
    }
    TRY(run_conv3(cx, L.c2, b));
    release_res_temps(cx, cA1, cB1, h1, cA2, cB2, sk);
    return DLPM_OK;
}

int run_attn(Ctx &cx, const Layer &L, Tensor4 x, Tensor4 *out) {
    dlpm_unet *u = cx.u;
    const int B = cx.B, C = x.C, T = x.H * x.W;
    {
        AttnSmallLaunch a;
        a.x = x.p; a.C = C; a.heads = u->cfg.num_heads; a.B = B; a.H = x.H; a.W = x.W;
        a.wqkv = L.c1.w_rs; a.wproj = L.c2.w_rs;
        const bool whole16 = attn16_ok(a);
        if (u->gen == DLPM_CONV_AUTO && (attn_small_ok(a) || whole16)) {
            *out = x;
            out->p = cx.ws.alloc((int64_t)B * T * C);
            out->stats = reinterpret_cast<float2 *>(cx.ws.alloc((int64_t)2 * B * C));
            out->stats_px = T;
            if (cx.dry()) return DLPM_OK;
            a.gn_w = u->params[L.p_gn1_w].dev; a.gn_b = u->params[L.p_gn1_b].dev;
            a.bqkv = u->params[L.c1.p_b].dev; a.bproj = u->params[L.c2.p_b].dev;
            a.out = out->p; a.stats_out = out->stats;
            return whole16 ? launch_attnblock16(a, cx.st) : launch_attnblock_small(a, cx.st);
        }
    }
    float *cA = cx.ws.alloc((int64_t)B * C), *cB = cx.ws.alloc((int64_t)B * C);
    float *qkv = cx.ws.alloc((int64_t)B * T * 3 * C);
    float *av = cx.ws.alloc((int64_t)B * T * C);
    float *o = cx.ws.alloc((int64_t)B * T * C);
    const Tensor4 xin = x;
    *out = x;
    out->p = o;
    plan_stats(cx.u, cx.ws, *out, L.c2, B, C, 1, 0);
    auto done = [&]() { cx.ws.release(cA); cx.ws.release(cB); cx.ws.release(qkv); cx.ws.release(av); };
    if (cx.dry()) {
        done();
        return DLPM_OK;
    }
    AttnSmallLaunch gq;
    gq.x = x.p; gq.C = C; gq.heads = u->cfg.num_heads; gq.B = B; gq.H = x.H; gq.W = x.W; gq.wqkv = L.c1.w_rs;
    if (u->gen == DLPM_CONV_AUTO && gnqkv_small_ok(gq)) {
        gq.gn_w = u->params[L.p_gn1_w].dev; gq.gn_b = u->params[L.p_gn1_b].dev; gq.bqkv = u->params[L.c1.p_b].dev; gq.out = qkv;
        TRY(launch_gnqkv_small(gq, cx.st));
    } else {
        TRY(gn_any(xin, Tensor4(), B, C < 32 ? C : 32, u->params[L.p_gn1_w].dev, u->params[L.p_gn1_b].dev, nullptr, 0, 0, cA, cB,
                   cx.st));
        ConvLaunch q;
        q.src0 = x.p; q.C0 = C; q.B = B; q.Hin = q.Hout = x.H; q.Win = q.Wout = x.W;
        q.bias = u->params[L.c1.p_b].dev; q.coefA = cA; q.coefB = cB; q.out = qkv;
        TRY(run_conv(u, L.c1, q, cx.st));
    }
    TRY(launch_attention(qkv, av, B, T, C, u->cfg.num_heads, cx.st));
    ConvLaunch p;
    p.src0 = av; p.C0 = C; p.B = B; p.Hin = p.Hout = x.H; p.Win = p.Wout = x.W;
    p.bias = u->params[L.c2.p_b].dev; p.res0 = x.p; p.R0 = C; p.out = o; p.stats_out = out->stats;
    TRY(run_conv(u, L.c2, p, cx.st));
    done();
    return DLPM_OK;
}

int run_seq(Ctx &cx, const std::vector<Layer> &seq, Tensor4 x0, Tensor4 x1, const float *x_nchw, Tensor4 *out, bool free0 = false,
            bool free1 = false) {
    dlpm_unet *u = cx.u;
    const int B = cx.B;
    Tensor4 h = x0;
    for (size_t i = 0; i < seq.size(); i++) {
        const Layer &L = seq[i];
        Tensor4 o;
        switch (L.kind) {
            case L_STEM: {
                const int S = u->cfg.image_size;
                o.C = L.cout; o.H = S; o.W = S;
                o.p = cx.ws.alloc((int64_t)B * S * S * L.cout);
                plan_stats(cx.u, cx.ws, o, L.c1, B, L.cin, 1, 0, true);
                if (!cx.dry()) {
                    ConvLaunch a;
                    a.src0 = x_nchw; a.C0 = L.cin; a.B = B; a.Hin = a.Hout = S; a.Win = a.Wout = S;
                    a.bias = u->params[L.c1.p_b].dev; a.out = o.p; a.in_nchw = 1; a.stats_out = o.stats;
                    TRY(run_conv(u, L.c1, a, cx.st));
                }
                break;
            }
            case L_RES:
                TRY(run_res(cx, L, h, (i == 0) ? x1 : Tensor4(), &o));
                break;
            case L_ATTN:
                TRY(run_attn(cx, L, h, &o));
                break;
            case L_DOWN:
            case L_UP: {
                const bool up = L.kind == L_UP;
                o.C = h.C;
                o.H = up ? h.H * 2 : (h.H - 1) / 2 + 1;
                o.W = up ? h.W * 2 : (h.W - 1) / 2 + 1;
                o.p = cx.ws.alloc((int64_t)B * o.H * o.W * o.C);
                plan_stats(cx.u, cx.ws, o, L.c1, B, h.C, up ? 1 : 2, up ? 1 : 0);
                {
                    ConvLaunch a;
                    a.src0 = h.p; a.C0 = h.C; a.B = B; a.Hin = h.H; a.Win = h.W; a.Hout = o.H; a.Wout = o.W;
                    a.stride = up ? 1 : 2; a.ups = up ? 1 : 0;
                    a.bias = u->params[L.c1.p_b].dev; a.out = o.p; a.stats_out = o.stats;
                    if (cx.dry()) { if (up) reserve_ksplit(cx, L.c1, a); }
                    else TRY(up ? run_conv3(cx, L.c1, a) : run_conv(u, L.c1, a, cx.st));
                }
                break;
            }
        }
        if (i == 0) {
            if (free0) drop(cx.ws, x0);
            if (free1) drop(cx.ws, x1);
        } else {
            drop(cx.ws, h);
        }
        h = o;
    }
    *out = h;
    return DLPM_OK;
}

__global__ void k_table_row(const float *__restrict__ table, const int32_t *__restrict__ row, int n, float *__restrict__ out) {
    const int i = blockIdx.x * blockDim.x + threadIdx.x;
    if (i < n) out[i] = table[(int64_t)(*row) * n + i];
}

int time_path(dlpm_unet *u, const float *t, int M, float *e0, float *e1, float *e2, float *out, hipStream_t st) {
    const int mc = u->cfg.model_channels, ted = u->ted;
    TRY(launch_timestep_embedding(t, e0, M, mc, st));
    ConvLaunch g;
    g.B = M; g.Hin = g.Win = g.Hout = g.Wout = 1;
    g.src0 = e0; g.C0 = mc; g.bias = u->params[u->te0.p_b].dev; g.out = e1;
    TRY(run_conv(u, u->te0, g, st));
    g.src0 = e1; g.C0 = ted; g.bias = u->params[u->te2.p_b].dev; g.out = e2; g.act_silu = 1;
    TRY(run_conv(u, u->te2, g, st));
    g.src0 = e2; g.bias = u->embcat_b; g.out = out;
    return run_conv(u, u->embcat, g, st);
}

thread_local const dlpm_unet *tl_time_net = nullptr;
thread_local const float *tl_time_table = nullptr;
thread_local const int32_t *tl_time_index = nullptr;

int walk(dlpm_unet *u, Ctx &cx, const float *x, const float *t, float *eps) {
    const int B = cx.B, mc = u->cfg.model_channels, ted = u->ted;
    const int Bt = cx.uniform_t ? 1 : B;
    float *e0 = cx.ws.alloc((int64_t)B * mc), *e1 = cx.ws.alloc((int64_t)B * ted), *e2 = cx.ws.alloc((int64_t)B * ted);
    cx.embout = cx.ws.alloc((int64_t)B * u->emb_total);
    if (!cx.dry()) {
        if (cx.uniform_t && tl_time_net == u && tl_time_table) {
            k_table_row<<<(unsigned)ceil_div(u->emb_total, 256), 256, 0, cx.st>>>(tl_time_table, tl_time_index, u->emb_total, cx.embout);
            DLPM_LAUNCH_CHECK();
        } else {
            TRY(time_path(u, t, Bt, e0, e1, e2, cx.embout, cx.st));
        }
    }
    cx.ws.release(e0);
    cx.ws.release(e1);
    cx.ws.release(e2);
    u->feats.clear();
    std::vector<Tensor4> hs;
    Tensor4 h;
    for (auto &seq : u->in_blocks) {
        TRY(run_seq(cx, seq, h, Tensor4(), x, &h));
        hs.push_back(h);
        u->feats.push_back(h);
    }
    TRY(run_seq(cx, u->mid, h, Tensor4(), nullptr, &h));
    u->feats.push_back(h);
    for (auto &seq : u->out_blocks) {
        Tensor4 skip = hs.back();
        hs.pop_back();
        if (skip.H != h.H || skip.W != h.W) {
            set_error("unet: skip connection %dx%d does not match %dx%d (image_size must be divisible by 2^(levels-1))",
                      skip.H, skip.W, h.H, h.W);
            return DLPM_ERR_ARG;
        }
        TRY(run_seq(cx, seq, h, skip, nullptr, &h, true, true));
        u->feats.push_back(h);
    }
    float *cA = cx.ws.alloc((int64_t)B * h.C), *cB = cx.ws.alloc((int64_t)B * h.C);
    float *P = nullptr;
    {
        ConvLaunch a;
        a.C0 = h.C; a.B = B; a.Hin = a.Hout = h.H; a.Win = a.Wout = h.W; a.ks = 3; a.Cout = u->head.cout; a.w_taps = u->head.w_taps; a.out_nchw = 1;
        a.w_hfused = u->head.w_hfused; a.coefA = cA; a.coefB = cB; a.act_silu = 1;
        if (!head_fused_ok(a) && head_gemm_ok(a)) P = cx.ws.alloc(head_gemm_scratch_floats(a));
    }
    if (!cx.dry()) {
        TRY(gn_any(h, Tensor4(), B, h.C < 32 ? h.C : 32, u->params[u->p_head_gn_w].dev, u->params[u->p_head_gn_b].dev, nullptr,
                   0, 0, cA, cB, cx.st));
        ConvLaunch a;
        a.src0 = h.p; a.C0 = h.C; a.B = B; a.Hin = a.Hout = h.H; a.Win = a.Wout = h.W;
        a.bias = u->params[u->head.p_b].dev; a.coefA = cA; a.coefB = cB; a.act_silu = 1; a.out = eps; a.out_nchw = 1;
        TRY(run_conv(u, u->head, a, cx.st, cx.hu, P));
    }
    if (!cx.ws.reuse) return DLPM_OK;
    for (auto &f : u->feats) f.p = nullptr;
    return DLPM_OK;
}

int64_t count_flops(dlpm_unet *u) {
    int64_t f = 0;
    const int S = u->cfg.image_size;
    auto convf = [&](const ConvW &c, int H, int W) { f += 2LL * c.cout * c.cin * c.ks * c.ks * H * W; };
    convf(u->te0, 1, 1);
    convf(u->te2, 1, 1);
    f += 2LL * u->emb_total * u->ted;
    int H = S;
    auto seqf = [&](const std::vector<Layer> &seq) {
        for (auto &L : seq) {
            switch (L.kind) {
                case L_STEM: convf(L.c1, H, H); break;
                case L_RES:
                    convf(L.c1, H, H); convf(L.c2, H, H);
                    if (L.has_skip) convf(L.skip, H, H);
                    break;
                case L_ATTN:
                    convf(L.c1, H, H); convf(L.c2, H, H);
                    f += 4LL * (H * H) * (H * H) * L.cin;
                    break;
                case L_DOWN: H = (H - 1) / 2 + 1; convf(L.c1, H, H); break;
                case L_UP: H *= 2; convf(L.c1, H, H); break;
            }
        }
    };
    for (auto &s : u->in_blocks) seqf(s);
    seqf(u->mid);
    for (auto &s : u->out_blocks) seqf(s);
    convf(u->head, H, H);
    return f;
}

}

extern "C" int dlpm_unet_create(const dlpm_unet_config *cfg, dlpm_unet **out) {
    DLPM_CHECK_ARG(cfg && out, "dlpm_unet_create: null argument");
    DLPM_CHECK_ARG(cfg->in_channels > 0 && cfg->model_channels > 0 && cfg->out_channels > 0 && cfg->num_res_blocks > 0,
                   "dlpm_unet_create: channels / res blocks must be positive");
    DLPM_CHECK_ARG(cfg->n_mult > 0 && cfg->n_mult <= 8 && cfg->n_attn >= 0 && cfg->n_attn <= 8,
                   "dlpm_unet_create: bad channel_mult / attention_resolutions length");
    DLPM_CHECK_ARG(cfg->num_heads > 0 && cfg->image_size > 0, "dlpm_unet_create: bad num_heads / image_size");
    DLPM_CHECK_ARG(cfg->image_size % (1 << (cfg->n_mult - 1)) == 0,
                   "dlpm_unet_create: image_size %d not divisible by 2^%d (the reference UNet fails on such sizes too)",
                   cfg->image_size, cfg->n_mult - 1);
    dlpm_unet *u = new dlpm_unet();
    u->cfg = *cfg;
    build_arch(u);
    *out = u;
    return DLPM_OK;
}

extern "C" int dlpm_unet_num_params(const dlpm_unet *net) { return net ? (int)net->params.size() : 0; }

extern "C" const char *dlpm_unet_param_key(const dlpm_unet *net, int i, int64_t *numel_out) {
    if (!net || i < 0 || i >= (int)net->params.size()) return nullptr;
    if (numel_out) *numel_out = net->params[i].numel;
    return net->params[i].key.c_str();
}

extern "C" int dlpm_unet_set_param(dlpm_unet *net, const char *key, const float *host, int64_t numel) {
    DLPM_CHECK_ARG(net && key && host, "dlpm_unet_set_param: null argument");
    auto it = net->index.find(key);
    DLPM_CHECK_ARG(it != net->index.end(), "dlpm_unet_set_param: unexpected key '%s' for this architecture", key);
    Param &p = net->params[it->second];
    DLPM_CHECK_ARG(p.numel == numel, "dlpm_unet_set_param: '%s' has %lld elements, expected %lld", key, (long long)numel,
                   (long long)p.numel);
    if (!p.dev) DLPM_HIP(hipMalloc(&p.dev, (size_t)numel * sizeof(float)));
    DLPM_HIP(hipMemcpy(p.dev, host, (size_t)numel * sizeof(float), hipMemcpyHostToDevice));
    p.set = true;
    net->finalized = false;
    return DLPM_OK;
}

static void free_conv(ConvW &c) {
    if (c.owns && c.w_dev) (void)hipFree(c.w_dev);
    if (c.w_frag) (void)hipFree(c.w_frag);
    c.w_frag = nullptr;
    if (c.w_wino) (void)hipFree(c.w_wino);
    c.w_wino = nullptr;
    if (c.w_wino4) (void)hipFree(c.w_wino4);
    c.w_wino4 = nullptr;
    if (c.w_wino4_n64) (void)hipFree(c.w_wino4_n64);
    if (c.w_wino4_n32) (void)hipFree(c.w_wino4_n32);
    c.w_wino4_n64 = c.w_wino4_n32 = nullptr;
    if (c.w_small) (void)hipFree(c.w_small);
    c.w_small = nullptr;
    if (c.w_taps) (void)hipFree(c.w_taps);
    c.w_taps = nullptr;
    if (c.w_rs) (void)hipFree(c.w_rs);
    c.w_rs = nullptr;
    if (c.w_hfused) (void)hipFree(c.w_hfused);
    c.w_hfused = nullptr;
    if (c.w_split) (void)hipFree(c.w_split);
    c.w_split = nullptr;
    c.w_dev = nullptr;
    c.owns = false;
}

static void for_each_conv(dlpm_unet *u, void (*fn)(ConvW &)) {
    auto seq = [&](std::vector<Layer> &s) {
        for (auto &L : s) {
            fn(L.c1);
            if (L.kind == L_RES || L.kind == L_ATTN) fn(L.c2);
            if (L.kind == L_RES && L.has_skip) fn(L.skip);
        }
    };
    for (auto &s : u->in_blocks) seq(s);
    seq(u->mid);
    for (auto &s : u->out_blocks) seq(s);
    fn(u->te0);
    fn(u->te2);
    fn(u->head);
}

constexpr int64_t NARROW_COPIES_MAX_BATCH = 512;
static int narrow_wino4_copies(dlpm_unet *u) {
    const bool want = u->dispatch_B > 0 && u->dispatch_B <= NARROW_COPIES_MAX_BATCH;
    int rc = DLPM_OK;
    auto one = [&](ConvW &c) {
        if (rc != DLPM_OK || !c.w_wino4 || c.cout % 128 != 0) return;
        if (!want) {
            if (c.w_wino4_n64) (void)hipFree(c.w_wino4_n64);
            if (c.w_wino4_n32) (void)hipFree(c.w_wino4_n32);
            c.w_wino4_n64 = c.w_wino4_n32 = nullptr;
            return;
        }
        for (int nq : {64, 32}) {
            float *&dst = nq == 64 ? c.w_wino4_n64 : c.w_wino4_n32;
            if (dst) continue;
            if (hipMalloc(&dst, (size_t)wino4_weight_floats(c.cout, c.cin) * sizeof(float)) != hipSuccess) { dst = nullptr; rc = DLPM_ERR_HIP; set_error("narrow_wino4_copies: hipMalloc failed"); return; }
            rc = relayout_weight_wino4(u->params[c.p_w].dev, dst, c.cout, c.cin, nullptr, nq);
            if (rc != DLPM_OK) return;
        }
    };
    auto seq = [&](std::vector<Layer> &s) {
        for (auto &L : s) {
            one(L.c1);
            if (L.kind == L_RES) one(L.c2);
        }
    };
    for (auto &s : u->in_blocks) seq(s);
    seq(u->mid);
    for (auto &s : u->out_blocks) seq(s);
    if (rc == DLPM_OK && hipDeviceSynchronize() != hipSuccess) { set_error("narrow_wino4_copies: synchronize failed"); rc = DLPM_ERR_HIP; }
    return rc;
}

extern "C" int dlpm_unet_finalize(dlpm_unet *u) {
    DLPM_CHECK_ARG(u, "dlpm_unet_finalize: null handle");
    for (auto &p : u->params)
        if (!p.set) {
            set_error("dlpm_unet_finalize: parameter '%s' was never set", p.key.c_str());
            return DLPM_ERR_STATE;
        }
    for_each_conv(u, free_conv);
    auto prep_seq = [&](std::vector<Layer> &s, int C0_first) -> int {
        for (size_t i = 0; i < s.size(); i++) {
            Layer &L = s[i];
            const bool cat = (i == 0 && L.kind == L_RES && C0_first > 0);
            const int C0 = cat ? C0_first : L.c1.cin;
            TRY(prep_conv(u, L.c1, L.kind == L_STEM ? L.c1.cin : C0, L.kind == L_STEM ? 1 : L.kind == L_DOWN ? 4 : 0));
            if (L.kind == L_RES || L.kind == L_ATTN) TRY(prep_conv(u, L.c2, L.c2.cin, 0));
            if (L.kind == L_RES && L.has_skip) TRY(prep_conv(u, L.skip, cat ? C0_first : L.skip.cin, 0));
        }
        return DLPM_OK;
    };
    for (auto &s : u->in_blocks) TRY(prep_seq(s, 0));
    TRY(prep_seq(u->mid, 0));
    {
        int ch = u->mid.back().cout;
        for (auto &s : u->out_blocks) {
            TRY(prep_seq(s, ch));
            ch = s[0].cout;
        }
    }
    TRY(prep_conv(u, u->te0, u->te0.cin, 3));
    TRY(prep_conv(u, u->te2, u->te2.cin, 3));
    TRY(prep_conv(u, u->head, u->head.cin, 2));
    if (u->embcat_w) (void)hipFree(u->embcat_w);
    if (u->embcat_b) (void)hipFree(u->embcat_b);
    DLPM_HIP(hipMalloc(&u->embcat_w, (size_t)u->emb_total * u->ted * sizeof(float)));
    DLPM_HIP(hipMalloc(&u->embcat_b, (size_t)u->emb_total * sizeof(float)));
    auto cat_seq = [&](std::vector<Layer> &s) -> int {
        for (auto &L : s)
            if (L.kind == L_RES) {
                DLPM_HIP(hipMemcpy(u->embcat_w + (size_t)L.emb_off * u->ted, u->params[L.p_emb_w].dev,
                                   (size_t)2 * L.cout * u->ted * sizeof(float), hipMemcpyDeviceToDevice));
                DLPM_HIP(hipMemcpy(u->embcat_b + L.emb_off, u->params[L.p_emb_b].dev, (size_t)2 * L.cout * sizeof(float),
                                   hipMemcpyDeviceToDevice));
            }
        return DLPM_OK;
    };
    for (auto &s : u->in_blocks) TRY(cat_seq(s));
    TRY(cat_seq(u->mid));
    for (auto &s : u->out_blocks) TRY(cat_seq(s));
    u->embcat.cout = u->emb_total; u->embcat.cin = u->ted; u->embcat.ks = 1;
    {
        ConvLaunch probe;
        probe.C0 = u->ted; probe.Cout = u->emb_total; probe.ks = 1;
        u->embcat.use_igemm = igemm_supported(probe);
        if (u->embcat.use_igemm) {
            u->embcat.w_dev = u->embcat_w;
        } else {
            DLPM_HIP(hipMalloc(&u->embcat.w_dev, (size_t)u->emb_total * u->ted * sizeof(float)));
            u->embcat.owns = true;
            TRY(relayout_weight(u->embcat_w, u->embcat.w_dev, u->emb_total, u->ted, 1, false, nullptr));
        }
    }
    TRY(narrow_wino4_copies(u));
    DLPM_HIP(hipDeviceSynchronize());
    u->flops = count_flops(u);
    u->finalized = true;
    u->plan_version++;
    return DLPM_OK;
}

extern "C" int dlpm_unet_set_conv_policy(dlpm_unet *u, int32_t generation, int64_t dispatch_batch) {
    DLPM_CHECK_ARG(u, "dlpm_unet_set_conv_policy: null handle");
    DLPM_CHECK_ARG(generation >= DLPM_CONV_AUTO && generation <= DLPM_CONV_IGEMM, "dlpm_unet_set_conv_policy: unknown generation %d",
                   generation);
    DLPM_CHECK_ARG(dispatch_batch >= 0, "dlpm_unet_set_conv_policy: negative dispatch batch");
    if (u->gen == generation && u->dispatch_B == dispatch_batch) return DLPM_OK;
    u->gen = generation;
    u->dispatch_B = dispatch_batch;
    u->plan_version++;
    if (u->finalized) TRY(narrow_wino4_copies(u));
    return DLPM_OK;
}

extern "C" int dlpm_unet_set_gemm_policy(dlpm_unet *u, int32_t mode) {
    DLPM_CHECK_ARG(u, "dlpm_unet_set_gemm_policy: null handle");
    DLPM_CHECK_ARG(mode >= DLPM_GEMM_AUTO && mode <= DLPM_GEMM_BF16X3, "dlpm_unet_set_gemm_policy: unknown mode %d", mode);
    if (u->gemm == mode) return DLPM_OK;
    u->gemm = mode;
    u->plan_version++;
    return DLPM_OK;
}

extern "C" int64_t dlpm_unet_time_embedding_width(const dlpm_unet *u) { return u ? u->emb_total : -1; }
extern "C" int64_t dlpm_unet_time_embeddings_scratch_bytes(const dlpm_unet *u, int64_t M) {
    return (u && M > 0) ? M * (u->cfg.model_channels + 2 * (int64_t)u->ted) * (int64_t)sizeof(float) : -1;
}

extern "C" int dlpm_unet_time_embeddings(dlpm_unet *net, const float *t_dev, int64_t M, float *out_dev, void *scratch_dev, int64_t scratch_bytes,
                                         dlpm_stream_t stream) {
    DLPM_CHECK_ARG(net && t_dev && out_dev && scratch_dev && M > 0 && M < (1 << 24), "dlpm_unet_time_embeddings: bad argument");
    if (!net->finalized) {
        set_error("dlpm_unet_time_embeddings: call dlpm_unet_finalize first");
        return DLPM_ERR_STATE;
    }
    const int64_t need = dlpm_unet_time_embeddings_scratch_bytes(net, M);
    if (scratch_bytes < need) {
        set_error("dlpm_unet_time_embeddings: scratch of %lld bytes, need %lld", (long long)scratch_bytes, (long long)need);
        return DLPM_ERR_NOMEM;
    }
    float *e0 = static_cast<float *>(scratch_dev), *e1 = e0 + M * net->cfg.model_channels, *e2 = e1 + M * net->ted;
    return time_path(net, t_dev, (int)M, e0, e1, e2, out_dev, as_stream(stream));
}

extern "C" int dlpm_unet_bind_time_table(dlpm_unet *net, const float *table_dev, const int32_t *row_index_dev) {
    DLPM_CHECK_ARG(net && ((table_dev == nullptr) == (row_index_dev == nullptr)), "dlpm_unet_bind_time_table: give both pointers or neither");
    if (!table_dev && tl_time_net != net) return DLPM_OK;
    tl_time_net = table_dev ? net : nullptr;
    tl_time_table = table_dev;
    tl_time_index = row_index_dev;
    return DLPM_OK;
}

extern "C" int64_t dlpm_unet_plan_version(const dlpm_unet *u) { return u ? u->plan_version : -1; }

extern "C" int64_t dlpm_unet_workspace_bytes(const dlpm_unet *net, int64_t B) {
    if (!net || B <= 0) return -1;
    Ctx cx;
    cx.u = const_cast<dlpm_unet *>(net);
    cx.B = (int)B;
    cx.ws.dry = true;
    cx.ws.reuse = !net->keep_feats;
    cx.st = nullptr;
    std::vector<Tensor4> keep = net->feats;
    int r = walk(cx.u, cx, nullptr, nullptr, nullptr);
    cx.u->feats = keep;
    return r == DLPM_OK ? cx.ws.peak : -1;
}

static int unet_forward(dlpm_unet *net, const float *x_dev, const float *t_dev, float *eps_dev, int64_t B, void *workspace_dev,
                        int64_t workspace_bytes, dlpm_stream_t stream, bool uniform_t, const HeadUpdate *hu = nullptr);

extern "C" int dlpm_unet_forward(dlpm_unet *net, const float *x_dev, const float *t_dev, float *eps_dev, int64_t B,
                                 void *workspace_dev, int64_t workspace_bytes, dlpm_stream_t stream) {
    return unet_forward(net, x_dev, t_dev, eps_dev, B, workspace_dev, workspace_bytes, stream, false);
}

extern "C" int dlpm_unet_forward_uniform_t(dlpm_unet *net, const float *x_dev, const float *t_dev, float *eps_dev, int64_t B,
                                           void *workspace_dev, int64_t workspace_bytes, dlpm_stream_t stream) {
    return unet_forward(net, x_dev, t_dev, eps_dev, B, workspace_dev, workspace_bytes, stream, true);
}

static bool head_fusable(const dlpm_unet *u) {
    ConvLaunch L;
    const int H = u->cfg.image_size;
    L.C0 = u->head.cin; L.Hin = L.Hout = H; L.Win = L.Wout = H; L.ks = 3; L.Cout = u->head.cout; L.out_nchw = 1;
    L.w_small = u->head.w_small;
    L.w_taps = u->head.w_taps;
    L.w_hfused = u->head.w_hfused;
    L.coefA = L.coefB = reinterpret_cast<const float *>(u);
    L.act_silu = 1;
    return head_fused_ok(L) || head_gemm_ok(L) || head_conv_ok(L);
}

extern "C" int dlpm_unet_forward_update(dlpm_unet *net, const float *x_in_dev, const float *t_dev, const dlpm_update_args *upd,
                                        float *eps_scratch_dev, int64_t B, void *workspace_dev, int64_t workspace_bytes,
                                        dlpm_stream_t stream) {
    DLPM_CHECK_ARG(net && x_in_dev && t_dev && upd && upd->x_dev && upd->t_dev && upd->g_dev && upd->c_eps_dev && upd->c_noise_dev,
                   "dlpm_unet_forward_update: null argument");
    DLPM_CHECK_ARG(upd->B == B, "dlpm_unet_forward_update: update batch %lld != %lld", (long long)upd->B, (long long)B);
    const int64_t D = (int64_t)net->cfg.out_channels * net->cfg.image_size * net->cfg.image_size;
    DLPM_CHECK_ARG(upd->D == D, "dlpm_unet_forward_update: state of %lld elements per sample, the net emits %lld", (long long)upd->D,
                   (long long)D);
    const bool aligned = ((reinterpret_cast<uintptr_t>(upd->x_dev) | reinterpret_cast<uintptr_t>(upd->z_dev)) % 16) == 0;
    const bool fuse = net->finalized && head_fusable(net) && aligned &&
                      !(upd->flags & (DLPM_UPD_DLIM | DLPM_UPD_CLIP | DLPM_UPD_ELEMENTWISE));
    if (!fuse) {
        DLPM_CHECK_ARG(eps_scratch_dev, "dlpm_unet_forward_update: this update variant needs the eps scratch buffer");
        int r = unet_forward(net, x_in_dev, t_dev, eps_scratch_dev, B, workspace_dev, workspace_bytes, stream, true);
        if (r != DLPM_OK) return r;
        dlpm_update_args a = *upd;
        a.eps_dev = eps_scratch_dev;
        return dlpm_update_f32(&a, stream);
    }
    HeadUpdate hu;
    hu.x = upd->x_dev; hu.z = upd->z_dev; hu.t = upd->t_dev; hu.g = upd->g_dev; hu.c_eps = upd->c_eps_dev; hu.c_noise = upd->c_noise_dev;
    hu.key = upd->key_dev; hu.seed = upd->seed; hu.sample_offset = upd->sample_offset; hu.hist_pp = upd->hist_pp;
    hu.T = upd->T; hu.B = B;
    float dummy;
    int r = unet_forward(net, x_in_dev, t_dev, eps_scratch_dev ? eps_scratch_dev : &dummy, B, workspace_dev, workspace_bytes, stream, true, &hu);
    if (r != DLPM_OK) return r;
    if (upd->flags & DLPM_UPD_ADVANCE) return launch_step_advance(const_cast<int32_t *>(upd->t_dev), as_stream(stream));
    return DLPM_OK;
}

static int unet_forward(dlpm_unet *net, const float *x_dev, const float *t_dev, float *eps_dev, int64_t B, void *workspace_dev,
                        int64_t workspace_bytes, dlpm_stream_t stream, bool uniform_t, const HeadUpdate *hu) {
    DLPM_CHECK_ARG(net && x_dev && t_dev && eps_dev && workspace_dev, "dlpm_unet_forward: null argument");
    DLPM_CHECK_ARG(B > 0 && B < (1 << 24), "dlpm_unet_forward: bad batch %lld", (long long)B);
    if (!net->finalized) {
        set_error("dlpm_unet_forward: call dlpm_unet_finalize first");
        return DLPM_ERR_STATE;
    }
    const int64_t need = dlpm_unet_workspace_bytes(net, B);
    if (need < 0) return DLPM_ERR_ARG;
    if (workspace_bytes < need) {
        set_error("dlpm_unet_forward: workspace of %lld bytes, need %lld", (long long)workspace_bytes, (long long)need);
        return DLPM_ERR_NOMEM;
    }
    Ctx cx;
    cx.u = net;
    cx.B = (int)B;
    cx.ws.base = static_cast<char *>(workspace_dev);
    cx.ws.cap = workspace_bytes;
    cx.ws.reuse = !net->keep_feats;
    cx.st = as_stream(stream);
    cx.uniform_t = uniform_t;
    cx.hu = hu;
    return walk(net, cx, x_dev, t_dev, eps_dev);
}

extern "C" int dlpm_unet_keep_features(dlpm_unet *net, int on) {
    DLPM_CHECK_ARG(net, "dlpm_unet_keep_features: null handle");
    net->keep_feats = on != 0;
    net->plan_version++;
    return DLPM_OK;
}

extern "C" int dlpm_unet_num_features(const dlpm_unet *net) {
    return net ? (int)(net->in_blocks.size() + 1 + net->out_blocks.size()) : 0;
}

extern "C" int dlpm_unet_feature_shape(const dlpm_unet *net, int i, int32_t *C, int32_t *H, int32_t *W) {
    DLPM_CHECK_ARG(net && i >= 0 && i < (int)net->feats.size(), "dlpm_unet_feature_shape: no such feature (run a forward first)");
    if (C) *C = net->feats[i].C;
    if (H) *H = net->feats[i].H;
    if (W) *W = net->feats[i].W;
    return DLPM_OK;
}

extern "C" int dlpm_unet_get_feature(dlpm_unet *net, int i, float *out_nchw_dev, int64_t B, dlpm_stream_t stream) {
    DLPM_CHECK_ARG(net && out_nchw_dev && i >= 0 && i < (int)net->feats.size() && net->feats[i].p,
                   "dlpm_unet_get_feature: no such feature (call dlpm_unet_keep_features(net, 1), then run a forward)");
    const Tensor4 &f = net->feats[i];
    return dlpm_nhwc_to_nchw_f32(f.p, out_nchw_dev, (int32_t)B, f.C, f.H, f.W, stream);
}

extern "C" int64_t dlpm_unet_flops_per_sample(const dlpm_unet *net) { return net ? net->flops : 0; }

extern "C" void dlpm_unet_destroy(dlpm_unet *u) {
    if (!u) return;
    for_each_conv(u, free_conv);
    if (u->embcat.owns && u->embcat.w_dev) (void)hipFree(u->embcat.w_dev);
    if (u->embcat_w) (void)hipFree(u->embcat_w);
    if (u->embcat_b) (void)hipFree(u->embcat_b);
    for (auto &p : u->params)
        if (p.dev) (void)hipFree(p.dev);
    delete u;
}

extern "C" int dlpm_conv2d_f32(const dlpm_conv_args *a, float *scratch_dev, dlpm_stream_t stream) {
    DLPM_CHECK_ARG(a && a->src0 && a->weight && a->out && scratch_dev, "dlpm_conv2d_f32: null argument");
    DLPM_CHECK_ARG(a->ksize == 1 || a->ksize == 3, "dlpm_conv2d_f32: ksize must be 1 or 3");
    DLPM_CHECK_ARG(a->stride == 1 || a->stride == 2, "dlpm_conv2d_f32: stride must be 1 or 2");
    DLPM_CHECK_ARG((a->C1 == 0) == (a->src1 == nullptr), "dlpm_conv2d_f32: src1/C1 mismatch");
    ConvLaunch L;
    L.src0 = a->src0; L.src1 = a->src1; L.C0 = a->C0; L.C1 = a->C1; L.B = a->B;
    L.Hin = a->Hin; L.Win = a->Win; L.Hout = a->Hout; L.Wout = a->Wout;
    L.ks = a->ksize; L.stride = a->stride; L.ups = a->upsample;
    L.bias = a->bias; L.coefA = a->coefA; L.coefB = a->coefB; L.act_silu = a->act_silu;
    L.res0 = a->res0; L.res1 = a->res1; L.R0 = a->R0; L.out = a->out; L.Cout = a->Cout;
    L.in_nchw = a->in_nchw; L.out_nchw = a->out_nchw;
    const bool ig = !(a->force_direct & 1) && igemm_supported(L);
    if ((a->in_nchw || a->out_nchw) && a->C1 != 0) {
        set_error("dlpm_conv2d_f32: NCHW boundary layouts do not combine with a concat input");
        return DLPM_ERR_UNSUPPORTED;
    }
    hipStream_t st = as_stream(stream);
    TRY(relayout_weight(a->weight, scratch_dev, a->Cout, a->C0 + a->C1, a->ksize, ig, st));
    L.w = scratch_dev;
    if (ig && a->ksize == 1 && (a->C0 + a->C1) % 32 == 0 && (a->force_direct & 4) &&
        a->scratch_floats >= (int64_t)a->Cout * (a->C0 + a->C1) + frag_weight_floats(a->Cout, a->C0 + a->C1, 1)) {
        float *wf = scratch_dev + (int64_t)a->Cout * (a->C0 + a->C1);
        TRY(relayout_weight_frag(a->weight, wf, a->Cout, a->C0 + a->C1, st, 1));
        L.w_frag = wf;
        L.ws_gemm = 1;
    }
    L.gemm = DLPM_GEMM_F32;
    const int taps = a->ksize * a->ksize;
    if (ig && (a->force_direct & 16) && a->Cout % 128 == 0 && (a->C0 + a->C1) % 32 == 0 &&
        a->scratch_floats >= (int64_t)a->Cout * (a->C0 + a->C1) * taps + split_weight_floats(a->Cout, a->C0 + a->C1, taps)) {
        float *wsp = scratch_dev + (int64_t)a->Cout * (a->C0 + a->C1) * taps;
        TRY(relayout_weight_split(a->weight, wsp, a->Cout, a->C0 + a->C1, taps, st));
        L.w_split = wsp;
        L.gemm = DLPM_GEMM_BF16X3;
    }
    if (ig && a->ksize == 3 && !L.w_split && (a->C0 + a->C1) % 32 == 0 &&
        a->scratch_floats >= (int64_t)a->Cout * (a->C0 + a->C1) * 9 + frag_weight_floats(a->Cout, a->C0 + a->C1)) {
        float *wf = scratch_dev + (int64_t)a->Cout * (a->C0 + a->C1) * 9;
        TRY(relayout_weight_frag(a->weight, wf, a->Cout, a->C0 + a->C1, st));
        L.w_frag = wf;
        int64_t used = (int64_t)a->Cout * (a->C0 + a->C1) * 9 + frag_weight_floats(a->Cout, a->C0 + a->C1);
        const bool wino_shape = !(a->force_direct & 2) && a->stride == 1 && !a->in_nchw && !a->out_nchw;
        if (wino_shape && a->Cout % 64 == 0 && a->scratch_floats >= used + wino_weight_floats(a->Cout, a->C0 + a->C1)) {
            float *ww = scratch_dev + used;
            TRY(relayout_weight_wino(a->weight, ww, a->Cout, a->C0 + a->C1, st));
            L.w_wino = ww;
            used += wino_weight_floats(a->Cout, a->C0 + a->C1);
        }
        if (wino_shape && (a->force_direct & 8) && a->Cout % 32 == 0 && (a->C0 + a->C1) % 8 == 0 &&
            a->scratch_floats >= used + wino4_weight_floats(a->Cout, a->C0 + a->C1)) {
            float *w4 = scratch_dev + used;
            TRY(relayout_weight_wino4(a->weight, w4, a->Cout, a->C0 + a->C1, st));
            L.w_wino4 = w4;
            int bh_, bw_, ni_;
            if (!wino4_geometry(L, &bh_, &bw_, &ni_)) {
                set_error("dlpm_conv2d_f32: force_direct bit 8 asks for the F(4x4,3x3) kernel, which does not take this geometry");
                return DLPM_ERR_UNSUPPORTED;
            }
            L.w_wino = nullptr;
        }
    }
    if ((a->force_direct & 64) && a->ksize == 3 && a->Cout <= 3 && a->C0 % 32 == 0 && a->C1 == 0) {
        L.w_hfused = scratch_dev;
        L.gemm = (a->force_direct & 128) ? DLPM_GEMM_F32 : DLPM_GEMM_AUTO;
        if (a->scratch_floats >= head_fused_weight_floats(a->C0) && head_fused_ok(L)) {
            TRY(relayout_weight_head_fused(a->weight, scratch_dev, a->Cout, a->C0, st));
            return launch_conv_head_fused(L, nullptr, st);
        }
        set_error("dlpm_conv2d_f32: the one-pass head kernel does not take this shape / scratch size");
        return DLPM_ERR_UNSUPPORTED;
    }
    if ((a->force_direct & 32) && a->ksize == 3 && a->Cout <= 3 && a->C0 % 32 == 0 && a->C1 == 0) {
        const int64_t wsz = (int64_t)head_taps_rows(a->Cout) * a->C0;
        L.w_taps = scratch_dev;
        if (a->scratch_floats >= wsz + head_gemm_scratch_floats(L) && head_gemm_ok(L)) {
            TRY(relayout_weight_head_taps(a->weight, scratch_dev, a->Cout, a->C0, st));
            return launch_conv_head_gemm(L, nullptr, scratch_dev + wsz, st);
        }
        set_error("dlpm_conv2d_f32: the GEMM + gather head does not take this shape / scratch size");
        return DLPM_ERR_UNSUPPORTED;
    }
    if (!(a->force_direct & 7) && a->ksize == 3 && a->Cout <= 4 && a->C0 % 32 == 0 && a->C1 == 0) {
        const int64_t front = (int64_t)a->Cout * a->C0 * 9 + frag_weight_floats(a->Cout, a->C0);
        const int64_t wsz = (int64_t)9 * a->C0 * 4;
        if (a->scratch_floats >= front + wsz) {
            float *ws = scratch_dev + (a->scratch_floats - wsz);
            TRY(relayout_weight_head(a->weight, ws, a->Cout, a->C0, st));
            L.w_small = ws;
            if (head_conv_ok(L)) return launch_conv_head(L, nullptr, st);
        }
    }
    if (ig) return launch_conv_igemm(L, st);
    return (a->force_direct & 1) ? launch_conv_direct(L, st) : launch_conv_fallback(L, st);
}

extern "C" int dlpm_groupnorm_coeffs_f32(const float *src0, const float *src1, int32_t C0, int32_t C1, int32_t B, int32_t HW,
                                         int32_t groups, const float *gamma, const float *beta, const float *ss,
                                         int64_t ss_stride, int64_t ss_offset, float *coefA, float *coefB,
                                         dlpm_stream_t stream) {
    DLPM_CHECK_ARG(src0 && gamma && beta && coefA && coefB, "dlpm_groupnorm_coeffs_f32: null argument");
    DLPM_CHECK_ARG(groups > 0 && (C0 + C1) % groups == 0, "dlpm_groupnorm_coeffs_f32: %d channels not divisible by %d groups",
                   C0 + C1, groups);
    return launch_gn_coeffs(src0, src1, C0, C1, B, HW, groups, gamma, beta, ss, ss_stride, ss_offset, coefA, coefB,
                            as_stream(stream));
}

extern "C" int dlpm_attention_f32(const float *qkv, float *out, int32_t B, int32_t T, int32_t C, int32_t heads,
                                  dlpm_stream_t stream) {
    DLPM_CHECK_ARG(qkv && out && B > 0, "dlpm_attention_f32: null argument");
    return launch_attention(qkv, out, B, T, C, heads, as_stream(stream));
}

extern "C" int dlpm_resblock_small_f32(const dlpm_resblock_args *a, float *scratch_dev, int64_t scratch_floats, dlpm_stream_t stream) {
    DLPM_CHECK_ARG(a && a->x0 && a->conv1_w && a->conv2_w && a->ss && a->out && scratch_dev, "dlpm_resblock_small_f32: null argument");
    DLPM_CHECK_ARG(a->gn1_w && a->gn1_b && a->gn2_w && a->gn2_b && a->conv1_b && a->conv2_b, "dlpm_resblock_small_f32: null GroupNorm / bias parameter");
    DLPM_CHECK_ARG(!a->skip_w || a->skip_b, "dlpm_resblock_small_f32: skip_w without skip_b");
    DLPM_CHECK_ARG(a->B > 0 && a->H == a->W && (a->H == 8 || a->H == 4), "dlpm_resblock_small_f32: B %d, %d x %d images (8x8 or 4x4)", a->B, a->H, a->W);
    DLPM_CHECK_ARG((a->C1 == 0) == (a->x1 == nullptr), "dlpm_resblock_small_f32: x1/C1 mismatch");
    const int Cin = a->C0 + a->C1;
    const int64_t n1 = (int64_t)64 * Cin * 9, n2 = (int64_t)64 * 64 * 9, ns = a->skip_w ? (int64_t)64 * Cin : 0;
    DLPM_CHECK_ARG(scratch_floats >= n1 + n2 + ns, "dlpm_resblock_small_f32: scratch of %lld floats, need %lld", (long long)scratch_floats,
                   (long long)(n1 + n2 + ns));
    DLPM_CHECK_ARG(small_weight_ok(64, Cin, 3), "dlpm_resblock_small_f32: %d input channels (64 or 128)", Cin);
    hipStream_t st = as_stream(stream);
    TRY(relayout_weight_small(a->conv1_w, scratch_dev, 64, Cin, 3, st));
    TRY(relayout_weight_small(a->conv2_w, scratch_dev + n1, 64, 64, 3, st));
    if (a->skip_w) TRY(relayout_weight_small(a->skip_w, scratch_dev + n1 + n2, 64, Cin, 1, st));
    ResSmallLaunch r;
    r.x0 = a->x0; r.x1 = a->x1; r.C0 = a->C0; r.C1 = a->C1; r.B = a->B; r.H = a->H; r.W = a->W;
    r.gn1_w = a->gn1_w; r.gn1_b = a->gn1_b; r.gn2_w = a->gn2_w; r.gn2_b = a->gn2_b;
    r.w1f = scratch_dev; r.b1 = a->conv1_b; r.w2f = scratch_dev + n1; r.b2 = a->conv2_b;
    r.wsf = a->skip_w ? scratch_dev + n1 + n2 : nullptr; r.bs = a->skip_b;
    r.emb = a->ss; r.emb_stride = a->ss_stride; r.emb_off = 0;
    r.out = a->out; r.stats_out = reinterpret_cast<float2 *>(a->stats_out);
    return launch_resblock_small(r, st);
}

extern "C" int64_t dlpm_resblock_img_scratch_floats(int64_t B, int32_t Cin) {
    if (B <= 0 || Cin <= 0) return -1;
    return wino4_weight_floats(64, Cin) + wino4_weight_floats(64, 64) + 2 * B * Cin + 2 * B * 1024 * 32 + 64;
}

extern "C" int dlpm_resblock_img_f32(const dlpm_resblock_args *a, float *scratch_dev, int64_t scratch_floats, dlpm_stream_t stream) {
    DLPM_CHECK_ARG(a && a->x0 && a->conv1_w && a->conv2_w && a->ss && a->out && scratch_dev, "dlpm_resblock_img_f32: null argument");
    DLPM_CHECK_ARG(a->gn1_w && a->gn1_b && a->gn2_w && a->gn2_b && a->conv1_b && a->conv2_b, "dlpm_resblock_img_f32: null GroupNorm / bias parameter");
    DLPM_CHECK_ARG(a->B > 0 && a->H == a->W && (a->H == 32 || a->H == 16), "dlpm_resblock_img_f32: B %d, %d x %d images (32x32 or 16x16)", a->B, a->H, a->W);
    const int CO = a->H == 32 ? 32 : 64, HW = a->H * a->W;
    DLPM_CHECK_ARG((a->C1 == 0) == (a->x1 == nullptr), "dlpm_resblock_img_f32: x1/C1 mismatch");
    const int Cin = a->C0 + a->C1;
    DLPM_CHECK_ARG(Cin >= 32 && Cin <= 128 && Cin % 8 == 0 && a->C0 % 8 == 0, "dlpm_resblock_img_f32: %d + %d input channels", a->C0, a->C1);
    DLPM_CHECK_ARG((Cin == CO) == (a->skip_w == nullptr) && (!a->skip_w || a->skip_b), "dlpm_resblock_img_f32: skip_w / skip_b (required unless C0 + C1 = the output channels)");
    DLPM_CHECK_ARG(scratch_floats >= dlpm_resblock_img_scratch_floats(a->B, Cin), "dlpm_resblock_img_f32: scratch of %lld floats, need %lld",
                   (long long)scratch_floats, (long long)dlpm_resblock_img_scratch_floats(a->B, Cin));
    hipStream_t st = as_stream(stream);
    float *w1 = scratch_dev, *w2 = w1 + wino4_weight_floats(CO, Cin), *cA = w2 + wino4_weight_floats(CO, CO), *cB = cA + (int64_t)a->B * Cin;
    float *hb = cB + (int64_t)a->B * Cin, *sk = hb + (int64_t)a->B * HW * CO;
    hb += (64 - ((hb - scratch_dev) & 63)) & 63;
    sk = hb + (int64_t)a->B * HW * CO;
    TRY(relayout_weight_wino4(a->conv1_w, w1, CO, Cin, st));
    TRY(relayout_weight_wino4(a->conv2_w, w2, CO, CO, st));
    TRY(launch_gn_coeffs(a->x0, a->x1, a->C0, a->C1, a->B, HW, 32, a->gn1_w, a->gn1_b, nullptr, 0, 0, cA, cB, st));
    ResImgLaunch r;
    r.x0 = a->x0; r.x1 = a->x1; r.C0 = a->C0; r.C1 = a->C1; r.B = a->B; r.H = a->H;
    r.coefA1 = cA; r.coefB1 = cB;
    r.gn1_w = a->gn1_w; r.gn1_b = a->gn1_b; r.gn2_w = a->gn2_w; r.gn2_b = a->gn2_b;
    r.w1 = w1; r.b1 = a->conv1_b; r.w2 = w2; r.b2 = a->conv2_b;
    r.emb = a->ss; r.emb_stride = a->ss_stride; r.emb_off = 0;
    r.hbuf = hb; r.out = a->out; r.stats_out = reinterpret_cast<float2 *>(a->stats_out);
    if (a->skip_w) {
        ConvLaunch s;
        s.src0 = a->x0; s.src1 = a->x1; s.C0 = a->C0; s.C1 = a->C1; s.B = a->B; s.Hin = s.Hout = a->H; s.Win = s.Wout = a->W;
        s.ks = 1; s.Cout = CO; s.w = a->skip_w; s.bias = a->skip_b; s.out = sk; s.gemm = DLPM_GEMM_F32;
        TRY(launch_conv_igemm(s, st));
        r.res = sk;
    } else {
        r.res = a->x0;
    }
    if (!res_img_ok(r)) {
        set_error("dlpm_resblock_img_f32: the whole-image ResBlock kernel is switched off (DLPM_RES_IMG=0 / DLPM_WINO_F4=0)");
        return DLPM_ERR_UNSUPPORTED;
    }
    return launch_resblock_img(r, st);
}

extern "C" int dlpm_attnblock_small_f32(const dlpm_attnblock_args *a, float *scratch_dev, int64_t scratch_floats, dlpm_stream_t stream) {
    DLPM_CHECK_ARG(a && a->x && a->qkv_w && a->proj_w && a->out && scratch_dev, "dlpm_attnblock_small_f32: null argument");
    DLPM_CHECK_ARG(a->gn_w && a->gn_b && a->qkv_b && a->proj_b, "dlpm_attnblock_small_f32: null GroupNorm / bias parameter");
    DLPM_CHECK_ARG(a->B > 0 && a->H == a->W && (a->H == 16 || a->H == 8 || a->H == 4), "dlpm_attnblock_small_f32: B %d, %d x %d images (16x16, 8x8 or 4x4)", a->B, a->H, a->W);
    DLPM_CHECK_ARG(a->C == 64 && a->heads == 4, "dlpm_attnblock_small_f32: 64 channels, 4 heads (got %d, %d)", a->C, a->heads);
    const int64_t nq = (int64_t)192 * 64, np = (int64_t)64 * 64;
    DLPM_CHECK_ARG(scratch_floats >= nq + np, "dlpm_attnblock_small_f32: scratch of %lld floats, need %lld", (long long)scratch_floats,
                   (long long)(nq + np));
    hipStream_t st = as_stream(stream);
    TRY(relayout_weight_small(a->qkv_w, scratch_dev, 192, 64, 1, st));
    TRY(relayout_weight_small(a->proj_w, scratch_dev + nq, 64, 64, 1, st));
    AttnSmallLaunch l;
    l.x = a->x; l.C = a->C; l.heads = a->heads; l.B = a->B; l.H = a->H; l.W = a->W;
    l.gn_w = a->gn_w; l.gn_b = a->gn_b; l.wqkv = scratch_dev; l.bqkv = a->qkv_b; l.wproj = scratch_dev + nq; l.bproj = a->proj_b;
    l.out = a->out; l.stats_out = reinterpret_cast<float2 *>(a->stats_out);
    return a->H == 16 ? launch_attnblock16(l, st) : launch_attnblock_small(l, st);
}

extern "C" int dlpm_timestep_embedding_f32(const float *t, float *emb, int64_t B, int32_t dim, dlpm_stream_t stream) {
    DLPM_CHECK_ARG(t && emb && B > 0 && dim > 0, "dlpm_timestep_embedding_f32: bad argument");
    return launch_timestep_embedding(t, emb, B, dim, as_stream(stream));
}
```

### include/dlpm_amd.h

```cpp
#ifndef DLPM_AMD_H
#define DLPM_AMD_H

#include <stdint.h>

#ifdef __cplusplus
extern "C" {
#endif

typedef void *dlpm_stream_t;

enum dlpm_status {
    DLPM_OK = 0,
    DLPM_ERR_ARG = -1,
    DLPM_ERR_HIP = -2,
    DLPM_ERR_UNSUPPORTED = -3,
    DLPM_ERR_STATE = -4,
    DLPM_ERR_NOMEM = -5,
    DLPM_ERR_IO = -6
};

const char *dlpm_last_error(void);
int dlpm_abi_version(void);

int dlpm_prof_enable(int on);
int dlpm_prof_report(char *buf, int64_t buf_bytes);


int dlpm_schedule_f32(int T, double alpha, float *g, float *bg, float *s, float *bs);

int dlpm_schedule_exploding_f32(int T, double alpha, float *g, float *bg, float *s, float *bs);

typedef struct dlpm_mt19937 {
    uint32_t key[624];
    int32_t pos;
    int32_t has_cached;
    double cached;
} dlpm_mt19937;

int dlpm_mt19937_seed(dlpm_mt19937 *st, uint32_t seed);

int dlpm_skewed_levy_host_f32(dlpm_mt19937 *np_stream, double alpha, int64_t n, double clamp_a, float *out);

int dlpm_randn_host_f32(dlpm_mt19937 *torch_stream, int64_t n, float *out);


int dlpm_skewed_levy_philox_f32(float *A_dev, int T, int64_t B, double alpha, double clamp_a,
                                uint64_t seed, int64_t sample_offset, dlpm_stream_t stream);

int dlpm_skewed_levy_elem_philox_f32(float *A_dev, int T, int64_t B, int64_t D, double alpha, double clamp_a,
                                     uint64_t seed, int64_t sample_offset, dlpm_stream_t stream);

int dlpm_init_state_elem_philox_f32(float *x_dev, int64_t B, int64_t D, double alpha, double clamp_eps,
                                    float barsigma_last, uint64_t seed, int64_t sample_offset, dlpm_stream_t stream);

int dlpm_init_state_philox_f32(float *x_dev, int64_t B, int64_t D, double alpha, double clamp_eps,
                               float barsigma_last, uint64_t seed, int64_t sample_offset,
                               dlpm_stream_t stream);

int dlpm_coeff_tables_f32(const float *A_dev, const float *g_dev, const float *s_dev, const float *bs_dev,
                          int T, int64_t B, float *c_eps_dev, float *c_noise_dev, float *sigmas_out_dev,
                          dlpm_stream_t stream);

enum dlpm_update_flags {
    DLPM_UPD_DLIM = 1,
    DLPM_UPD_CLIP = 2,
    DLPM_UPD_ADVANCE = 4,
    DLPM_SMP_NO_FUSED_MLP = 8,
    DLPM_UPD_ELEMENTWISE = 16,
    DLPM_SMP_LIM = 32,
    DLPM_UPD_HIST_ON = 64
};

typedef struct dlpm_update_args {
    float *x_dev;
    const float *eps_dev;
    const float *z_dev;
    const int32_t *t_dev;
    const float *g_dev, *bg_dev, *bs_dev;
    const float *c_eps_dev, *c_noise_dev;
    const float *A_dev;
    int64_t B, D;
    int32_t T;
    int32_t flags;
    float dlim_eta;
    float alpha;
    uint64_t seed;
    int64_t sample_offset;
    const uint64_t *key_dev;
    float *const *hist_pp;
} dlpm_update_args;

int dlpm_update_f32(const dlpm_update_args *args, dlpm_stream_t stream);

enum dlpm_mean_type {
    DLPM_MEAN_EPSILON = 0,
    DLPM_MEAN_START_X = 1,
    DLPM_MEAN_Z = 2,
    DLPM_MEAN_PREVIOUS_X = 3
};
enum dlpm_predict_flags {
    DLPM_PRED_TO_XSTART = 1,
    DLPM_PRED_CLIP = 2,
    DLPM_PRED_TO_EPS = 4,
    DLPM_PRED_ELEMENTWISE = 16
};
typedef struct dlpm_predict_args {
    const float *x_dev;
    const float *in_dev;
    float *out_dev;
    const int32_t *t_dev;
    const float *g_dev, *bg_dev, *bs_dev;
    const float *c_eps_dev;
    const float *A_dev;
    int64_t B, D;
    int32_t T;
    int32_t mean_type;
    int32_t flags;
} dlpm_predict_args;
int dlpm_predict_f32(const dlpm_predict_args *args, dlpm_stream_t stream);

int dlpm_fill_scaled_t_f32(float *tvec_dev, const int32_t *t_dev, int32_t T, int64_t B, dlpm_stream_t stream);

int dlpm_scale_by_table_f32(const float *x_dev, float *out_dev, int64_t n, const int32_t *t_dev, const float *table_dev,
                            dlpm_stream_t stream);

int dlpm_postprocess_f32(const float *x_dev, float *out_dev, int64_t n, float clamp, int affine, dlpm_stream_t stream);


int dlpm_lim_tables_f32(double alpha, int32_t steps, int32_t ode, float *ts, float *tmp, float *cx, float *cs, float *cn);

typedef struct dlpm_lim_update_args {
    float *x_dev;
    const float *eps_dev;
    const float *z_dev;
    const int32_t *t_dev;
    const float *tmp_dev, *cx_dev, *cs_dev, *cn_dev;
    const float *A_dev;
    int64_t B, D;
    int32_t T;
    int32_t flags;
    float clamp_eps;
    uint64_t seed;
    int64_t sample_offset;
    const uint64_t *key_dev;
    float *const *hist_pp;
} dlpm_lim_update_args;

int dlpm_lim_update_f32(const dlpm_lim_update_args *args, dlpm_stream_t stream);

int dlpm_fill_table_t_f32(float *tvec_dev, const int32_t *t_dev, const float *ts_dev, int32_t T, int64_t B,
                          dlpm_stream_t stream);


int dlpm_images_to_rgb8(const float *x_dev, uint8_t *out_dev, int64_t B, int32_t C, int32_t H, int32_t W,
                        dlpm_stream_t stream);

int64_t dlpm_png_bound(int32_t H, int32_t W);

int dlpm_png_encode_rgb8(const uint8_t *hwc, int32_t H, int32_t W, int32_t level, uint8_t *out, int64_t cap,
                         int64_t *len);

int dlpm_png_write_rgb8(const uint8_t *hwc_batch, int64_t B, int32_t H, int32_t W, const char *dir,
                        int64_t first_index, int32_t level, int32_t nthreads);


typedef struct dlpm_unet_config {
    int32_t in_channels, model_channels, out_channels, num_res_blocks;
    int32_t num_heads, image_size;
    int32_t n_mult, channel_mult[8];
    int32_t n_attn, attention_resolutions[8];
} dlpm_unet_config;

typedef struct dlpm_unet dlpm_unet;

int dlpm_unet_create(const dlpm_unet_config *cfg, dlpm_unet **out);
int dlpm_unet_set_param(dlpm_unet *net, const char *key, const float *host_data, int64_t numel);
int dlpm_unet_num_params(const dlpm_unet *net);
const char *dlpm_unet_param_key(const dlpm_unet *net, int index, int64_t *numel_out);
int dlpm_unet_finalize(dlpm_unet *net);
int64_t dlpm_unet_workspace_bytes(const dlpm_unet *net, int64_t B);
int dlpm_unet_forward(dlpm_unet *net, const float *x_dev, const float *t_dev, float *eps_dev, int64_t B,
                      void *workspace_dev, int64_t workspace_bytes, dlpm_stream_t stream);
int64_t dlpm_unet_time_embedding_width(const dlpm_unet *net);
int64_t dlpm_unet_time_embeddings_scratch_bytes(const dlpm_unet *net, int64_t M);
int dlpm_unet_time_embeddings(dlpm_unet *net, const float *t_dev, int64_t M, float *out_dev, void *scratch_dev, int64_t scratch_bytes,
                              dlpm_stream_t stream);
int dlpm_unet_bind_time_table(dlpm_unet *net, const float *table_dev, const int32_t *row_index_dev);
int dlpm_unet_forward_uniform_t(dlpm_unet *net, const float *x_dev, const float *t_dev, float *eps_dev, int64_t B,
                                void *workspace_dev, int64_t workspace_bytes, dlpm_stream_t stream);
int dlpm_unet_forward_update(dlpm_unet *net, const float *x_in_dev, const float *t_dev, const dlpm_update_args *upd,
                             float *eps_scratch_dev, int64_t B, void *workspace_dev, int64_t workspace_bytes,
                             dlpm_stream_t stream);
int dlpm_unet_keep_features(dlpm_unet *net, int on);
int dlpm_unet_num_features(const dlpm_unet *net);
int dlpm_unet_feature_shape(const dlpm_unet *net, int index, int32_t *C, int32_t *H, int32_t *W);
int dlpm_unet_get_feature(dlpm_unet *net, int index, float *out_nchw_dev, int64_t B, dlpm_stream_t stream);
int64_t dlpm_unet_flops_per_sample(const dlpm_unet *net);

enum dlpm_conv_generation { DLPM_CONV_AUTO = 0, DLPM_CONV_F4 = 1, DLPM_CONV_F2 = 2, DLPM_CONV_IGEMM = 3 };
int dlpm_unet_set_conv_policy(dlpm_unet *net, int32_t generation, int64_t dispatch_batch);
enum dlpm_gemm_mode { DLPM_GEMM_AUTO = 0, DLPM_GEMM_F32 = 1, DLPM_GEMM_BF16X3 = 2 };
int dlpm_unet_set_gemm_policy(dlpm_unet *net, int32_t mode);
int64_t dlpm_unet_plan_version(const dlpm_unet *net);
void dlpm_unet_destroy(dlpm_unet *net);

typedef struct dlpm_mlp dlpm_mlp;
int dlpm_mlp_create(int32_t nfeatures, int32_t nunits, int32_t nblocks, int32_t time_emb_size, dlpm_mlp **out);
int dlpm_mlp_set_param(dlpm_mlp *net, const char *key, const float *host_data, int64_t numel);
int dlpm_mlp_finalize(dlpm_mlp *net);
int dlpm_mlp_forward(dlpm_mlp *net, const float *x_dev, const float *t_dev, float *eps_dev, int64_t B,
                     dlpm_stream_t stream);
int dlpm_mlp_sample_steps_f32(dlpm_mlp *net, float *x_dev, const float *c_eps_dev, const float *c_noise_dev,
                              const float *g_dev, int32_t T, int64_t B, int32_t t_start, int32_t nsteps,
                              uint64_t seed, int64_t sample_offset, const uint64_t *key_dev, dlpm_stream_t stream);
void dlpm_mlp_destroy(dlpm_mlp *net);


typedef struct dlpm_conv_args {
    const float *src0, *src1;
    int32_t C0, C1;
    int32_t B, Hin, Win, Hout, Wout;
    int32_t ksize;
    int32_t stride;
    int32_t upsample;
    const float *weight;
    const float *bias;
    const float *coefA, *coefB;
    int32_t act_silu;
    const float *res0, *res1;
    int32_t R0;
    float *out;
    int32_t Cout;
    int32_t in_nchw, out_nchw;
    int32_t force_direct;
    int64_t scratch_floats;
} dlpm_conv_args;

int dlpm_conv2d_f32(const dlpm_conv_args *args, float *scratch_dev, dlpm_stream_t stream);

int dlpm_groupnorm_coeffs_f32(const float *src0, const float *src1, int32_t C0, int32_t C1, int32_t B, int32_t HW,
                              int32_t groups, const float *gamma_dev, const float *beta_dev,
                              const float *ss_dev, int64_t ss_stride, int64_t ss_offset,
                              float *coefA_dev, float *coefB_dev, dlpm_stream_t stream);

int dlpm_attention_f32(const float *qkv_dev, float *out_dev, int32_t B, int32_t T, int32_t C, int32_t heads,
                       dlpm_stream_t stream);

typedef struct dlpm_resblock_args {
    const float *x0, *x1;
    int32_t C0, C1, B, H, W;
    const float *gn1_w, *gn1_b;
    const float *conv1_w, *conv1_b;
    const float *ss;
    int64_t ss_stride;
    const float *gn2_w, *gn2_b;
    const float *conv2_w, *conv2_b;
    const float *skip_w, *skip_b;
    float *out;
    float *stats_out;
} dlpm_resblock_args;
int dlpm_resblock_small_f32(const dlpm_resblock_args *args, float *scratch_dev, int64_t scratch_floats, dlpm_stream_t stream);

int64_t dlpm_resblock_img_scratch_floats(int64_t B, int32_t Cin);
int dlpm_resblock_img_f32(const dlpm_resblock_args *args, float *scratch_dev, int64_t scratch_floats, dlpm_stream_t stream);

typedef struct dlpm_attnblock_args {
    const float *x;
    int32_t C, heads, B, H, W;
    const float *gn_w, *gn_b;
    const float *qkv_w, *qkv_b;
    const float *proj_w, *proj_b;
    float *out;
    float *stats_out;
} dlpm_attnblock_args;
int dlpm_attnblock_small_f32(const dlpm_attnblock_args *args, float *scratch_dev, int64_t scratch_floats, dlpm_stream_t stream);

int dlpm_timestep_embedding_f32(const float *t_dev, float *emb_dev, int64_t B, int32_t dim, dlpm_stream_t stream);

int dlpm_nchw_to_nhwc_f32(const float *src, float *dst, int32_t B, int32_t C, int32_t H, int32_t W, dlpm_stream_t stream);
int dlpm_nhwc_to_nchw_f32(const float *src, float *dst, int32_t B, int32_t C, int32_t H, int32_t W, dlpm_stream_t stream);


typedef struct dlpm_sampler_config {
    dlpm_unet *unet;
    dlpm_mlp *mlp;
    int64_t B;
    int32_t C, H, W;
    int32_t T;
    double alpha;
    double clamp_a, clamp_eps;
    int32_t flags;
    float dlim_eta;
    uint64_t seed;
    int64_t sample_offset;
    int32_t use_graph;
    const float *g, *bg, *s, *bs;
    const float *lim_ts, *lim_tmp, *lim_cx, *lim_cs, *lim_cn;
    const float *in_scale;
    int32_t mean_type;
} dlpm_sampler_config;

typedef struct dlpm_sampler dlpm_sampler;

int dlpm_sampler_create(const dlpm_sampler_config *cfg, dlpm_sampler **out);
int dlpm_sampler_reseed(dlpm_sampler *s, uint64_t seed, int64_t sample_offset);
int dlpm_sampler_begin(dlpm_sampler *s, dlpm_stream_t stream);
int dlpm_sampler_begin_injected(dlpm_sampler *s, const float *A_dev, const float *xT_dev, dlpm_stream_t stream);
int dlpm_sampler_set_state(dlpm_sampler *s, const float *x_dev, int32_t t, dlpm_stream_t stream);
int dlpm_sampler_step_injected(dlpm_sampler *s, const float *z_dev, dlpm_stream_t stream);
int dlpm_sampler_steps(dlpm_sampler *s, int32_t nsteps, dlpm_stream_t stream);
int dlpm_sampler_set_history(dlpm_sampler *s, float *hist_dev, dlpm_stream_t stream);

int dlpm_sampler_copy_state(dlpm_sampler *s, float *out_dev, dlpm_stream_t stream);
float *dlpm_sampler_state(dlpm_sampler *s);
int32_t dlpm_sampler_t(const dlpm_sampler *s);
float *dlpm_sampler_table(dlpm_sampler *s, int which);
void dlpm_sampler_destroy(dlpm_sampler *s);

#ifdef __cplusplus
}
#endif
#endif
```

Before: 27.69.

## Add sub-pixel Winograd kernel for upsample+3x3 convolutions

Adds a sub-pixel decomposition for nearest-upsample followed by a 3x3 conv. The four output phases are computed directly from the low-resolution input, using per-phase 2x2 effective kernels in a Winograd-like 5-point transform (points ±0.5, ±1.25, infinity) with MFMA accumulation. This avoids the redundant work of convolving the upsampled image, in exchange for extra per-phase weight storage (4x25 per Cin/Cout pair), a new kernel and different numerical conditioning. The UNet upsample layers with Cout divisible by 128 get these weights at prep time and route to the new kernel. A stats-returning conv entry point is also added.

```diff
diff --git a/dlpm_amd/_lib.py b/dlpm_amd/_lib.py
--- a/dlpm_amd/_lib.py
+++ b/dlpm_amd/_lib.py
@@ -124,6 +124,7 @@
     'dlpm_mlp_sample_steps_f32': (C.c_int, [vp, vp, vp, vp, vp, i32, i64, i32, i32, u64, i64, vp, vp]),
     'dlpm_mlp_destroy': (None, [vp]),
     'dlpm_conv2d_f32': (C.c_int, [C.POINTER(ConvArgs), vp, vp]),
+    'dlpm_conv2d_stats_f32': (C.c_int, [C.POINTER(ConvArgs), vp, vp, vp]),
     'dlpm_groupnorm_coeffs_f32': (C.c_int, [vp, vp, i32, i32, i32, i32, i32, vp, vp, vp, i64, i64, vp, vp, vp]),
     'dlpm_attention_f32': (C.c_int, [vp, vp, i32, i32, i32, i32, vp]),
     'dlpm_resblock_small_f32': (C.c_int, [C.POINTER(ResBlockArgs), vp, i64, vp]),
diff --git a/dlpm_amd/csrc/conv.h b/dlpm_amd/csrc/conv.h
--- a/dlpm_amd/csrc/conv.h
+++ b/dlpm_amd/csrc/conv.h
@@ -12,6 +12,7 @@
     const float *w_frag = nullptr;
     const float *w_wino = nullptr;
     const float *w_wino4 = nullptr;
+    const float *w_subpix = nullptr;
     const float *w_wino4_n64 = nullptr, *w_wino4_n32 = nullptr;
     const void *w_split = nullptr;
     const float *w_small = nullptr;
@@ -80,6 +81,10 @@
 int launch_conv_wino4(const ConvLaunch &c, hipStream_t st);
 int64_t wino4_weight_floats(int Cout, int Cin);
 int relayout_weight_wino4(const float *oihw_dev, float *dst_dev, int Cout, int Cin, hipStream_t st, int nq = 0);
+bool wino4_subpix(const ConvLaunch &c);
+int subpix_stats_pixels(const ConvLaunch &c);
+int64_t subpix_weight_floats(int Cout, int Cin);
+int relayout_weight_subpix4(const float *oihw_dev, float *dst_dev, int Cout, int Cin, hipStream_t st);
 struct ResImgLaunch {
     const float *x0 = nullptr, *x1 = nullptr;
     int C0 = 0, C1 = 0, B = 0;
diff --git a/dlpm_amd/csrc/conv_igemm.hip b/dlpm_amd/csrc/conv_igemm.hip
--- a/dlpm_amd/csrc/conv_igemm.hip
+++ b/dlpm_amd/csrc/conv_igemm.hip
@@ -1045,6 +1045,7 @@
         const int64_t hw = (int64_t)c.Hout * c.Wout;
         return (c.R0 & 3) ? 0 : hw % BM == 0 ? BM : hw == 64 ? 64 : 0;
     }
+    if (wino4_preferred(c, &a, &b, &n) && wino4_subpix(c)) return subpix_stats_pixels(c);
     if (wino4_preferred(c, &a, &b, &n)) return n == 1 ? 256 : (n == 4 && a * b == 4 && wino4_image_stats(c.Cout)) ? 64 : 0;
     if (wino_geometry(c, &a, &b, &n)) return n == 1 ? 4 * wino_tiles(c) : 0;
     if (c.out_nchw || (c.Cout & 3) || (c.R0 & 3)) return 0;
@@ -1081,10 +1082,12 @@
     {
         int wb, ww, wi;
         if (wino4_preferred(c, &wb, &ww, &wi)) {
+            const bool sp = wino4_subpix(c);
             if (prof_enabled() && prof_detail())
-                snprintf(pname, sizeof(pname), "conv3x3_wino4:H%d:Cin%d+%d:Cout%d:u%d:coef%d", c.Hout, c.C0, c.C1, c.Cout, c.ups, c.coefA ? 1 : 0);
+                snprintf(pname, sizeof(pname), "%s:H%d:Cin%d+%d:Cout%d:u%d:coef%d", sp ? "conv3x3_subpix4" : "conv3x3_wino4", c.Hout, c.C0, c.C1, c.Cout,
+                         c.ups, c.coefA ? 1 : 0);
             else
-                snprintf(pname, sizeof(pname), "conv3x3_wino4");
+                snprintf(pname, sizeof(pname), "%s", sp ? "conv3x3_subpix4" : "conv3x3_wino4");
             ProfScope psw(pname, 2.0 * M * c.Cout * K, bytes, st);
             return launch_conv_wino4(c, st);
         }
diff --git a/dlpm_amd/csrc/conv_wino4.hip b/dlpm_amd/csrc/conv_wino4.hip
--- a/dlpm_amd/csrc/conv_wino4.hip
+++ b/dlpm_amd/csrc/conv_wino4.hip
@@ -1598,6 +1598,404 @@
     dst[i] = (float)u;
 }
 
+#ifndef SP_S0
+#define SP_S0 4
+#endif
+#ifndef SP_X
+#define SP_X 9
+#endif
+#define SP_PA 0.5
+#define SP_PB 1.25
+constexpr float QA = (float)SP_PA, QB = (float)SP_PB, QA2 = (float)(SP_PA * SP_PA), QB2 = (float)(SP_PB * SP_PB);
+constexpr float QA3 = (float)(SP_PA * SP_PA * SP_PA), QB3 = (float)(SP_PB * SP_PB * SP_PB);
+constexpr float QS2 = (float)(SP_PA * SP_PA + SP_PB * SP_PB), QP2 = (float)(SP_PA * SP_PA * SP_PB * SP_PB);
+constexpr int SP_NPP = 12;
+constexpr int SP_VBUF = 13 * 4 * F4_TILES * 4;
+constexpr int SP_WPH = 25 * 16 * F4_KC;
+static_assert(SP_NPP % F4_RING == 0, "the weight ring divides the position pairs of a phase");
+
+template <int QN>
+__global__ void __launch_bounds__(F4_NT, 1) k_conv3x3_subpix4(ConvLaunch p, int bh, int bw, int nimg) {
+    extern __shared__ __attribute__((aligned(16))) float wsm[];
+    float *V = wsm;
+    float *raw = wsm + 2 * SP_VBUF;
+    float *Cf = raw + 2 * F4_RAWBUF;
+    DLPM_PHASE_DECL;
+#ifdef DLPM_PHASE_TIMING
+    const long long _c0 = clock64(), _r0 = wall_clock64();
+    long long _wait = 0;
+#endif
+    const int tid = threadIdx.x, lane = tid & 63, wave = tid >> 6;
+    const int li = lane & 15, lk = lane >> 4;
+    const int W = p.Wout, H = p.Hout, Ws = W >> 1, Hs = H >> 1, TW = Ws >> 2, TH = Hs >> 2;
+    const int Cin = p.C0 + p.C1;
+    const int nch = Cin / F4_KC;
+    const int ntn = p.Cout / F4_NQ;
+    const int nmb = gridDim.x / (4 * ntn);
+    const int bid = blockIdx.x;
+    const int cls = bid / (ntn * nmb), r_ = bid - cls * (ntn * nmb);
+    const int nt = r_ / nmb, mb = r_ - nt * nmb, n0 = nt * F4_NQ;
+    const int py = cls >> 1, px = cls & 1;
+    int img0, ty0, tx0, blk_in_img = 0, bpi = 1;
+    if (nimg == 1) {
+        const int bpr = TW / bw;
+        bpi = (TH / bh) * bpr;
+        img0 = mb / bpi;
+        blk_in_img = mb - img0 * bpi;
+        ty0 = (blk_in_img / bpr) * bh;
+        tx0 = (blk_in_img % bpr) * bw;
+    } else {
+        img0 = mb * nimg;
+        ty0 = tx0 = 0;
+    }
+    const int RH = 4 * bh + 2, RW = 4 * bw + 2;
+    const int oy = 4 * ty0 - 1, ox = 4 * tx0 - 1;
+    const int rpi = RH * RW, npix = nimg * rpi;
+
+    const int squad = tid & 1;
+    auto pix_of = [&](int it) { return it == 1 ? (F4_NT / 2) + ((F4_NT - 1 - tid) >> 1) : it * (F4_NT / 2) + (tid >> 1); };
+    const bool skewed = nimg == 1 && bh <= 4;
+    int off[QN], lo[QN];
+#pragma unroll
+    for (int it = 0; it < QN; it++) {
+        const int pix = pix_of(it);
+        const int img = min(pix / rpi, nimg - 1), r = pix - img * rpi;
+        const int ry = r / RW, rx = r - ry * RW;
+        const int iy = oy + ry, ix = ox + rx;
+        const bool pad = iy < 0 || iy >= Hs || ix < 0 || ix >= Ws || (img0 + img) >= p.B;
+        off[it] = pix >= npix ? -2 : (pad ? -1 : (((img0 + img) * Hs + iy) * Ws + ix));
+        lo[it] = (pix * F4_PRLD + squad * 4 + (skewed ? 4 * (ry >> 2) : 0)) | ((img * 2 * F4_KC + squad * 4) << 16);
+    }
+    const bool has_coef = p.coefA != nullptr;
+    const int cf_img = tid >> 2, cf_isb = (tid >> 1) & 1;
+    const bool cf_mine = has_coef && tid < nimg * 4;
+    const float *cf_base = has_coef ? ((cf_isb ? p.coefB : p.coefA) + (int64_t)min(img0 + cf_img, p.B - 1) * Cin + squad * 4) : nullptr;
+    float4 xr[QN], cfr = make_float4(0.f, 0.f, 0.f, 0.f);
+    auto load_raw_into = [&](float4 (&dst)[QN], int chunk) {
+        const int c = chunk * F4_KC + squad * 4;
+        const bool first = c < p.C0;
+        const float *sb = first ? p.src0 + c : p.src1 + (c - p.C0);
+        const int ld = first ? p.C0 : p.C1;
+#pragma unroll
+        for (int it = 0; it < QN; it++) dst[it] = *reinterpret_cast<const float4 *>(sb + (int64_t)max(off[it], 0) * ld);
+    };
+    auto load_coef = [&](int chunk) {
+        if (cf_mine) cfr = *reinterpret_cast<const float4 *>(cf_base + chunk * F4_KC);
+    };
+    auto store_coef = [&](int slot) {
+        if (cf_mine) *reinterpret_cast<float4 *>(Cf + slot * F4_CFS + cf_img * 2 * F4_KC + cf_isb * F4_KC + squad * 4) = cfr;
+    };
+    auto store_raw_item = [&](int slot, int it) {
+        if (off[it] == -2) return;
+        float *rb = raw + slot * F4_RAWBUF;
+        float4 x = xr[it];
+        if (has_coef) {
+            const float4 ca = *reinterpret_cast<const float4 *>(Cf + slot * F4_CFS + (lo[it] >> 16));
+            const float4 cb = *reinterpret_cast<const float4 *>(Cf + slot * F4_CFS + (lo[it] >> 16) + F4_KC);
+            x.x = fmaf(x.x, ca.x, cb.x);
+            x.y = fmaf(x.y, ca.y, cb.y);
+            x.z = fmaf(x.z, ca.z, cb.z);
+            x.w = fmaf(x.w, ca.w, cb.w);
+        }
+        if (p.act_silu) {
+            x.x = silu_f(x.x);
+            x.y = silu_f(x.y);
+            x.z = silu_f(x.z);
+            x.w = silu_f(x.w);
+        }
+        if (off[it] < 0) x = make_float4(0.f, 0.f, 0.f, 0.f);
+        *reinterpret_cast<float4 *>(rb + (lo[it] & 0xffff)) = x;
+    };
+    auto store_raw = [&](int slot) {
+#pragma unroll
+        for (int it = 0; it < QN; it++) store_raw_item(slot, it);
+    };
+
+    int rbase, vofs;
+    {
+        const int tile = lane & 15, pair = lane >> 4;
+        const int timg = tile / (bh * bw), r = tile - timg * (bh * bw);
+        const int ty = r / bw, tx = r - ty * bw;
+        rbase = (timg * rpi + (4 * ty + py) * RW + 4 * tx + px) * F4_PRLD + pair * 2 + (skewed ? 4 * ty : 0);
+        vofs = (pair * F4_TILES + tile) * 4;
+    }
+    auto transform_rows = [&](int slot, int w) __attribute__((always_inline)) {
+        const float *rb = raw + slot * F4_RAWBUF + rbase;
+        float *vb = V + slot * SP_VBUF + vofs;
+        auto d = [&](int i, int c) __attribute__((always_inline)) {
+            return *reinterpret_cast<const float2 *>(rb + (i * RW + c) * F4_PRLD + ((skewed && i + py >= 4) ? 4 : 0));
+        };
+        auto row_out = [&](const float2 (&T)[5], int a) __attribute__((always_inline)) {
+            const float2 e1 = f2fma(-QB2, T[1], T[3]), o1 = f2fma(-QB2, T[0], T[2]);
+            const float2 e2 = f2fma(-QA2, T[1], T[3]), o2 = f2fma(-QA2, T[0], T[2]);
+            float2 v[5];
+            v[0] = f2fma(QA, o1, e1); v[1] = f2fma(-QA, o1, e1);
+            v[2] = f2fma(QB, o2, e2); v[3] = f2fma(-QB, o2, e2);
+            v[4] = f2fma(QP2, T[0], f2fma(-QS2, T[2], T[4]));
+            auto st4 = [&](int pos, float2 x, float2 y) {
+                *reinterpret_cast<float4 *>(vb + (pos >> 1) * (4 * F4_TILES * 4)) = make_float4(x.x, x.y, y.x, y.y);
+            };
+            auto st2 = [&](int pos, float2 x) { *reinterpret_cast<float2 *>(vb + (pos >> 1) * (4 * F4_TILES * 4) + 2 * (pos & 1)) = x; };
+            if ((a & 1) == 0) { st4(5 * a, v[0], v[1]); st4(5 * a + 2, v[2], v[3]); st2(5 * a + 4, v[4]); }
+            else { st2(5 * a, v[0]); st4(5 * a + 1, v[1], v[2]); st4(5 * a + 3, v[3], v[4]); }
+        };
+        if (w < 2) {
+            const float sq = w == 0 ? QB2 : QA2, pt = w == 0 ? QA : QB;
+            float2 Ta[5], Tb[5];
+#pragma unroll
+            for (int c = 0; c < 5; c++) {
+                const float2 e = f2fma(-sq, d(1, c), d(3, c)), o = f2fma(-sq, d(0, c), d(2, c));
+                Ta[c] = f2fma(pt, o, e);
+                Tb[c] = f2fma(-pt, o, e);
+            }
+            if (w == 0) { row_out(Ta, 0); row_out(Tb, 1); }
+            else { row_out(Ta, 2); row_out(Tb, 3); }
+        } else {
+            float2 T[5];
+#pragma unroll
+            for (int c = 0; c < 5; c++) T[c] = f2fma(QP2, d(0, c), f2fma(-QS2, d(2, c), d(4, c)));
+            row_out(T, 4);
+        }
+    };
+    auto transform = [&](int slot) __attribute__((always_inline)) {
+        if (wave == 0) transform_rows(slot, 0);
+        else if (wave == 1) transform_rows(slot, 1);
+        else if (wave == 3) transform_rows(slot, 2);
+    };
+
+    const float4 *__restrict__ wp = reinterpret_cast<const float4 *>(p.w_subpix) +
+                                    (int64_t)((cls * ntn + nt) * 8 + __builtin_amdgcn_readfirstlane(wave)) * nch * (SP_WPH / 4);
+    constexpr int AHEAD = F4_RING - 1;
+    float4 bq[F4_RING];
+    const float *asrc = V + lane * 4;
+
+    floatx4 acc[25];
+#pragma unroll
+    for (int q = 0; q < 25; q++)
+#pragma unroll
+        for (int r = 0; r < 4; r++) acc[q][r] = 0.f;
+
+    const int last = nch - 1;
+    float4 xr1[QN], cfr1 = make_float4(0.f, 0.f, 0.f, 0.f), cfr2 = cfr1;
+    load_raw_into(xr, 0);
+    load_raw_into(xr1, min(1, last));
+    load_coef(0);
+    if (cf_mine) {
+        cfr1 = *reinterpret_cast<const float4 *>(cf_base + min(1, last) * F4_KC);
+        cfr2 = *reinterpret_cast<const float4 *>(cf_base + min(2, last) * F4_KC);
+    }
+#pragma unroll
+    for (int a = 0; a < AHEAD; a++) bq[a] = wp[a * 64 + lane];
+    store_coef(0);
+    cfr = cfr1;
+    store_coef(1);
+    __syncthreads();
+    store_raw(0);
+#pragma unroll
+    for (int it = 0; it < QN; it++) xr[it] = xr1[it];
+    store_raw(1);
+    load_raw_into(xr, min(2, last));
+    __syncthreads();
+    transform(0);
+    cfr = cfr2;
+    store_coef(0);
+    __syncthreads();
+    DLPM_PHASE(p, 8);
+
+#pragma unroll 1
+    for (int chunk = 0; chunk < nch; chunk++) {
+        const int cur = chunk & 1, nxt = cur ^ 1;
+        const float *ab = asrc + cur * SP_VBUF;
+        load_coef(min(chunk + 3, last));
+        const float2 bt = reinterpret_cast<const float2 *>(wp + SP_NPP * 64)[lane];
+        float4 aq[2];
+        float2 at;
+        aq[0] = *reinterpret_cast<const float4 *>(ab);
+#pragma unroll
+        for (int pp = 0; pp < SP_NPP; pp++) {
+            if (pp >= SP_S0 && pp < SP_S0 + QN) store_raw_item(cur, pp - SP_S0);
+            if (pp == SP_S0 + QN) load_raw_into(xr, min(chunk + 3, last));
+            if (pp == SP_X) transform(nxt);
+            const int t = pp + AHEAD;
+            bq[t % F4_RING] = t < SP_NPP ? wp[t * 64 + lane] : wp[SP_WPH / 4 + (t - SP_NPP) * 64 + lane];
+            if (pp + 1 < SP_NPP) aq[(pp + 1) & 1] = *reinterpret_cast<const float4 *>(ab + (pp + 1) * (4 * F4_TILES * 4));
+            else at = *reinterpret_cast<const float2 *>(ab + SP_NPP * (4 * F4_TILES * 4));
+            const float4 aa = aq[pp & 1];
+            const float4 b = bq[pp % F4_RING];
+            if (F4_PRIO) __builtin_amdgcn_s_setprio(0);
+            acc[2 * pp] = __builtin_amdgcn_mfma_f32_16x16x4f32(aa.x, b.x, acc[2 * pp], 0, 0, 0);
+            acc[2 * pp + 1] = __builtin_amdgcn_mfma_f32_16x16x4f32(aa.z, b.z, acc[2 * pp + 1], 0, 0, 0);
+            acc[2 * pp] = __builtin_amdgcn_mfma_f32_16x16x4f32(aa.y, b.y, acc[2 * pp], 0, 0, 0);
+            acc[2 * pp + 1] = __builtin_amdgcn_mfma_f32_16x16x4f32(aa.w, b.w, acc[2 * pp + 1], 0, 0, 0);
+            if (F4_PRIO) __builtin_amdgcn_s_setprio(1);
+        }
+        {
+            if (F4_PRIO) __builtin_amdgcn_s_setprio(0);
+            acc[24] = __builtin_amdgcn_mfma_f32_16x16x4f32(at.x, bt.x, acc[24], 0, 0, 0);
+            acc[24] = __builtin_amdgcn_mfma_f32_16x16x4f32(at.y, bt.y, acc[24], 0, 0, 0);
+            if (F4_PRIO) __builtin_amdgcn_s_setprio(1);
+        }
+        wp += SP_WPH / 4;
+        store_coef(nxt);
+#ifdef DLPM_PHASE_TIMING
+        const long long _w0 = clock64();
+#endif
+        __syncthreads();
+#ifdef DLPM_PHASE_TIMING
+        _wait += clock64() - _w0;
+#endif
+    }
+    if (F4_PRIO) __builtin_amdgcn_s_setprio(0);
+    DLPM_PHASE(p, 9);
+
+    const int64_t pix0 = ((int64_t)img0 * H + 8 * ty0 + py) * W + 8 * tx0 + px;
+    const int ch = n0 + 16 * wave + li;
+    const float bias_v = p.bias ? p.bias[ch] : 0.f;
+    const bool has_res = p.res0 != nullptr;
+    const bool res_first = __builtin_amdgcn_readfirstlane(n0 + 16 * wave) < p.R0;
+    const float *res_u = has_res ? (res_first ? p.res0 : p.res1 - p.R0) : nullptr;
+    const int res_ld = res_first ? p.R0 : p.Cout - p.R0;
+    const int lbw = 31 - __builtin_clz(bw), lbhw = 31 - __builtin_clz(bh * bw);
+    float *__restrict__ out_blk = p.out + pix0 * p.Cout;
+    const float *__restrict__ res_blk = has_res ? res_u + pix0 * res_ld : nullptr;
+    const bool st_blk = p.stats_out != nullptr && nimg == 1, st_img = p.stats_out != nullptr && nimg == 4 && bh * bw == 4;
+    const bool st_tile = p.stats_out != nullptr && nimg == 16;
+    float K = 0.f, s1 = 0.f, s2 = 0.f;
+#pragma unroll
+    for (int r = 0; r < 4; r++) {
+        const int tile = 4 * lk + r;
+        const int timg = tile >> lbhw, ty = (tile & (bh * bw - 1)) >> lbw, tx = tile & (bw - 1);
+        const int tpix = (timg * H + 8 * ty) * W + 8 * tx;
+        const bool ok = img0 + timg < p.B;
+        const uint32_t bo_o = (uint32_t)(tpix * p.Cout + ch) * 4u, bo_r = (uint32_t)(tpix * res_ld + ch) * 4u;
+        float rs[16];
+        if (has_res && ok) {
+#pragma unroll
+            for (int i = 0; i < 4; i++)
+#pragma unroll
+                for (int j = 0; j < 4; j++)
+                    rs[i * 4 + j] = *reinterpret_cast<const float *>(reinterpret_cast<const char *>(res_blk + (2 * i * W + 2 * j) * res_ld) + bo_r);
+        }
+        float Z[4][5], Yt[16];
+#pragma unroll
+        for (int b = 0; b < 5; b++) {
+            const float m0 = acc[0 * 5 + b][r], m1 = acc[1 * 5 + b][r], m2 = acc[2 * 5 + b][r], m3 = acc[3 * 5 + b][r], m4 = acc[4 * 5 + b][r];
+            const float sa = m0 + m1, da = m0 - m1, sb = m2 + m3, db = m2 - m3;
+            Z[0][b] = sa + sb;
+            Z[1][b] = fmaf(QB, db, QA * da);
+            Z[2][b] = fmaf(QB2, sb, QA2 * sa);
+            Z[3][b] = fmaf(QB3, db, QA3 * da) + m4;
+        }
+#pragma unroll
+        for (int i = 0; i < 4; i++) {
+            const float sa = Z[i][0] + Z[i][1], da = Z[i][0] - Z[i][1], sb = Z[i][2] + Z[i][3], db = Z[i][2] - Z[i][3];
+            Yt[i * 4 + 0] = sa + sb;
+            Yt[i * 4 + 1] = fmaf(QB, db, QA * da);
+            Yt[i * 4 + 2] = fmaf(QB2, sb, QA2 * sa);
+            Yt[i * 4 + 3] = fmaf(QB3, db, QA3 * da) + Z[i][4];
+        }
+        if (!ok) continue;
+        if (st_tile) { K = 0.f; s1 = 0.f; s2 = 0.f; }
+#pragma unroll
+        for (int i = 0; i < 4; i++) {
+#pragma unroll
+            for (int j = 0; j < 4; j++) {
+                float v = Yt[i * 4 + j] + bias_v;
+                if (has_res) v += rs[i * 4 + j];
+                if (st_blk || st_img || st_tile) {
+                    if ((st_tile || r == 0) && i == 0 && j == 0) K = v;
+                    const float dd = v - K;
+                    s1 += dd;
+                    s2 = fmaf(dd, dd, s2);
+                }
+                *reinterpret_cast<float *>(reinterpret_cast<char *>(out_blk + (2 * i * W + 2 * j) * p.Cout) + bo_o) = v;
+            }
+        }
+        if (st_tile)
+            p.stats_out[((int64_t)(img0 + tile) * 4 + cls) * p.Cout + ch] = make_float2(K + s1 * (1.f / 16.f), fmaxf(s2 - s1 * s1 * (1.f / 16.f), 0.f));
+    }
+    if (st_img) {
+        if (img0 + lk < p.B)
+            p.stats_out[((int64_t)(img0 + lk) * 4 + cls) * p.Cout + ch] = make_float2(K + s1 * (1.f / 64.f), fmaxf(s2 - s1 * s1 * (1.f / 64.f), 0.f));
+    } else if (st_blk) {
+        float mean = K + s1 * (1.f / 64.f), M2 = fmaxf(s2 - s1 * s1 * (1.f / 64.f), 0.f), na = 64.f;
+#pragma unroll
+        for (int sft = 16; sft <= 32; sft <<= 1) {
+            const float om = __shfl_xor(mean, sft), oM2 = __shfl_xor(M2, sft);
+            const float lo_m = (lane & sft) ? om : mean, hi_m = (lane & sft) ? mean : om;
+            const float lo_M = (lane & sft) ? oM2 : M2, hi_M = (lane & sft) ? M2 : oM2;
+            const float dd = hi_m - lo_m;
+            mean = lo_m + dd * 0.5f;
+            M2 = lo_M + hi_M + dd * dd * (na * 0.5f);
+            na *= 2.f;
+        }
+        if (lk == 0) p.stats_out[((int64_t)img0 * 4 * bpi + cls * bpi + blk_in_img) * p.Cout + ch] = make_float2(mean, M2);
+    }
+    DLPM_PHASE(p, 10);
+    DLPM_PHASE_FLUSH(p, 8);
+#ifdef DLPM_PHASE_TIMING
+    if (p.phase && lane == 0) atomicAdd(p.phase + 16 + wave, (unsigned long long)_wait);
+    if (p.phase && tid == 0) {
+        atomicAdd(p.phase + 11, 1ull);
+        atomicAdd(p.phase + 12, (unsigned long long)(clock64() - _c0));
+        atomicAdd(p.phase + 13, (unsigned long long)(wall_clock64() - _r0));
+    }
+#endif
+}
+
+__global__ void k_relayout_weight_subpix4(const float *oihw, float *dst, int Cout, int Cin) {
+    const int nch = Cin / F4_KC;
+    const int64_t total = (int64_t)4 * Cout * Cin * 25;
+    const int64_t i = (int64_t)blockIdx.x * blockDim.x + threadIdx.x;
+    if (i >= total) return;
+    const int q = (int)(i % SP_WPH);
+    int64_t r = i / SP_WPH;
+    const int chunk = (int)(r % nch); r /= nch;
+    const int wave = (int)(r % 8); r /= 8;
+    const int nt = (int)(r % (Cout / F4_NQ));
+    const int cls = (int)(r / (Cout / F4_NQ));
+    int lane, pos, kk;
+    if (q < SP_NPP * 256) {
+        const int e = q & 3;
+        lane = (q >> 2) & 63;
+        pos = 2 * (q >> 8) + (e >> 1);
+        kk = e & 1;
+    } else {
+        lane = (q - SP_NPP * 256) >> 1;
+        pos = 24;
+        kk = q & 1;
+    }
+    const int lk = lane >> 4, li = lane & 15;
+    const int cin = chunk * F4_KC + 2 * lk + kk;
+    const int cout = nt * F4_NQ + wave * 16 + li;
+    const float *g = oihw + ((int64_t)cout * Cin + cin) * 9;
+    const int py = cls >> 1, px = cls & 1;
+    const double FR[2][2][3] = {{{1., 0., 0.}, {0., 1., 1.}}, {{1., 1., 0.}, {0., 0., 1.}}};
+    double f[2][2];
+    for (int a = 0; a < 2; a++)
+        for (int b = 0; b < 2; b++) {
+            double s = 0.;
+            for (int ii = 0; ii < 3; ii++)
+                for (int jj = 0; jj < 3; jj++) s += FR[py][a][ii] * FR[px][b][jj] * (double)g[ii * 3 + jj];
+            f[a][b] = s;
+        }
+    const double pts[4] = {SP_PA, -SP_PA, SP_PB, -SP_PB};
+    double G[5][2];
+    for (int j = 0; j < 4; j++) {
+        double n = 1.;
+        for (int l = 0; l < 4; l++)
+            if (l != j) n *= pts[j] - pts[l];
+        G[j][0] = 1. / n;
+        G[j][1] = pts[j] / n;
+    }
+    G[4][0] = 0.;
+    G[4][1] = 1.;
+    const int ra = pos / 5, rb = pos % 5;
+    double u = 0.;
+    for (int a = 0; a < 2; a++) u += G[ra][a] * (G[rb][0] * f[a][0] + G[rb][1] * f[a][1]);
+    dst[i] = (float)u;
+}
+
 int f4_mode() {
     static int v = -1;
     if (v < 0) { const char *e = getenv("DLPM_WINO_F4"); v = e ? atoi(e) : 1; }
@@ -1685,6 +2083,42 @@
 
 static int launch_conv_wino4_nq(const ConvLaunch &c, int nq, int bh, int bw, int nimg, hipStream_t st);
 
+static bool subpix_enabled() {
+    static int v = -1;
+    if (v < 0) { const char *e = getenv("DLPM_WINO4_SUBPIX"); v = e ? atoi(e) : 1; }
+    return v != 0;
+}
+
+static bool subpix_geometry(const ConvLaunch &c, int *bh, int *bw, int *nimg) {
+    if (!c.ups || !c.w_subpix || !subpix_enabled() || c.ksplit > 1) return false;
+    if (c.Cout % F4_NQ != 0 || (c.Hout & 7) || (c.Wout & 7) || wino4_nq_for(c) != F4_NQ) return false;
+    ConvLaunch lo = c;
+    lo.ups = 0; lo.Hout = c.Hout / 2; lo.Wout = c.Wout / 2;
+    return wino4_geometry_nq(lo, F4_NQ, bh, bw, nimg);
+}
+bool wino4_subpix(const ConvLaunch &c) {
+    int bh, bw, n;
+    return subpix_geometry(c, &bh, &bw, &n);
+}
+int subpix_stats_pixels(const ConvLaunch &c) {
+    int bh, bw, n;
+    if (!subpix_geometry(c, &bh, &bw, &n)) return 0;
+    return n == 1 ? 256 : (n == 4 && bh * bw == 4) ? 64 : n == 16 ? 16 : 0;
+}
+
+static int launch_conv_subpix4(const ConvLaunch &c, int bh, int bw, int nimg, hipStream_t st) {
+    using KFn = void (*)(ConvLaunch, int, int, int);
+    const int64_t mblocks = nimg == 1 ? (int64_t)c.B * (c.Hout / 8) * (c.Wout / 8) / F4_TILES : ceil_div(c.B, nimg);
+    const bool small = nimg * (4 * bh + 2) * (4 * bw + 2) <= F4_NT;
+    KFn fn = small ? &k_conv3x3_subpix4<2> : &k_conv3x3_subpix4<F4_QNIT>;
+    const int r = ensure_dynamic_lds(reinterpret_cast<const void *>(fn), 160 * 1024);
+    if (r != DLPM_OK) return r;
+    const size_t lds = (size_t)(2 * SP_VBUF + 2 * F4_RAWBUF + 2 * F4_CFS) * sizeof(float);
+    fn<<<(unsigned)(4 * mblocks * (c.Cout / F4_NQ)), F4_NT, lds, st>>>(c, bh, bw, nimg);
+    DLPM_LAUNCH_CHECK();
+    return DLPM_OK;
+}
+
 int launch_conv_wino4(const ConvLaunch &c, hipStream_t st) {
     int bh, bw, nimg;
     if (!wino4_geometry(c, &bh, &bw, &nimg)) {
@@ -1695,6 +2129,10 @@
     const_cast<ConvLaunch &>(c).phase = phase_buffer();
 #endif
     const int nq = wino4_nq_for(c);
+    {
+        int sbh, sbw, sni;
+        if (subpix_geometry(c, &sbh, &sbw, &sni)) return launch_conv_subpix4(c, sbh, sbw, sni, st);
+    }
     if (nq != f4_nq_of(c.Cout)) {
         ConvLaunch cn = c;
         cn.w_wino4 = nq == 64 ? c.w_wino4_n64 : c.w_wino4_n32;
@@ -1841,6 +2279,20 @@
 
 int64_t wino4_weight_floats(int Cout, int Cin) { return (int64_t)Cout * Cin * 36 + F4_PAD * 256; }
 
+int64_t subpix_weight_floats(int Cout, int Cin) { return (int64_t)4 * Cout * Cin * 25 + F4_PAD * 256; }
+
+int relayout_weight_subpix4(const float *oihw_dev, float *dst_dev, int Cout, int Cin, hipStream_t st) {
+    if (Cout % F4_NQ != 0 || Cin % F4_KC != 0) {
+        set_error("relayout_weight_subpix4: Cout must be a multiple of 128 and Cin of 8");
+        return DLPM_ERR_ARG;
+    }
+    const int64_t n = (int64_t)4 * Cout * Cin * 25;
+    DLPM_HIP(hipMemsetAsync(dst_dev + n, 0, (size_t)F4_PAD * 256 * sizeof(float), st));
+    k_relayout_weight_subpix4<<<(unsigned)ceil_div(n, 256), 256, 0, st>>>(oihw_dev, dst_dev, Cout, Cin);
+    DLPM_LAUNCH_CHECK();
+    return DLPM_OK;
+}
+
 int relayout_weight_wino4(const float *oihw_dev, float *dst_dev, int Cout, int Cin, hipStream_t st, int nq_in) {
     const int64_t n = (int64_t)Cout * Cin * 36;
     DLPM_HIP(hipMemsetAsync(dst_dev + n, 0, (size_t)F4_PAD * 256 * sizeof(float), st));
diff --git a/dlpm_amd/csrc/unet.hip b/dlpm_amd/csrc/unet.hip
--- a/dlpm_amd/csrc/unet.hip
+++ b/dlpm_amd/csrc/unet.hip
@@ -29,6 +29,7 @@
     float *w_wino = nullptr;
     float *w_wino4 = nullptr;
     float *w_wino4_n64 = nullptr, *w_wino4_n32 = nullptr;
+    float *w_subpix = nullptr;
     float *w_small = nullptr;
     float *w_taps = nullptr;
     void *w_split = nullptr;
@@ -109,7 +110,7 @@
     t.stats_px = 0;
     if (off || (!c.use_igemm && !stem)) return;
     ConvLaunch L;
-    L.w_wino = c.w_wino; L.w_wino4 = c.w_wino4; L.w_wino4_n64 = c.w_wino4_n64; L.w_wino4_n32 = c.w_wino4_n32; L.w_split = c.w_split; L.ks = c.ks; L.stride = stride; L.ups = ups; L.Hout = t.H; L.Wout = t.W; L.Cout = c.cout;
+    L.w_wino = c.w_wino; L.w_wino4 = c.w_wino4; L.w_wino4_n64 = c.w_wino4_n64; L.w_wino4_n32 = c.w_wino4_n32; L.w_subpix = c.w_subpix; L.w_split = c.w_split; L.ks = c.ks; L.stride = stride; L.ups = ups; L.Hout = t.H; L.Wout = t.W; L.Cout = c.cout;
     L.Hin = ups ? t.H / 2 : t.H * stride; L.Win = ups ? t.W / 2 : t.W * stride;
     L.C0 = C0; L.C1 = c.cin - C0; L.B = B;
     L.in_nchw = stem ? 1 : 0;
@@ -288,7 +289,7 @@
     return v == 1;
 }
 
-int prep_conv(dlpm_unet *u, ConvW &c, int C0, int boundary) {
+int prep_conv(dlpm_unet *u, ConvW &c, int C0, int boundary, bool ups = false) {
     ConvLaunch probe;
     probe.C0 = C0; probe.C1 = c.cin - C0; probe.Cout = c.cout; probe.ks = c.ks;
     probe.in_nchw = boundary == 1; probe.out_nchw = boundary == 2;
@@ -347,6 +348,11 @@
             DLPM_HIP(hipMalloc(&c.w_wino4, (size_t)wino4_weight_floats(c.cout, c.cin) * sizeof(float)));
             r = relayout_weight_wino4(src, c.w_wino4, c.cout, c.cin, nullptr);
             if (r != DLPM_OK) return r;
+            if (ups && c.cout % 128 == 0) {
+                DLPM_HIP(hipMalloc(&c.w_subpix, (size_t)subpix_weight_floats(c.cout, c.cin) * sizeof(float)));
+                r = relayout_weight_subpix4(src, c.w_subpix, c.cout, c.cin, nullptr);
+                if (r != DLPM_OK) return r;
+            }
         }
     }
     if (small_weight_ok(c.cout, c.cin, c.ks) && boundary == 0) {
@@ -365,6 +371,7 @@
     L.w_wino4 = c.w_wino4;
     L.w_wino4_n64 = c.w_wino4_n64;
     L.w_wino4_n32 = c.w_wino4_n32;
+    L.w_subpix = c.w_subpix;
     L.w_small = c.w_small;
     L.w_taps = c.w_taps;
     L.w_hfused = c.w_hfused;
@@ -382,6 +389,7 @@
     L.w_wino4 = c.w_wino4;
     L.w_wino4_n64 = c.w_wino4_n64;
     L.w_wino4_n32 = c.w_wino4_n32;
+    L.w_subpix = c.w_subpix;
     L.w_small = c.w_small;
     L.w_taps = c.w_taps;
     L.w_hfused = c.w_hfused;
@@ -829,6 +837,8 @@
     if (c.w_wino4_n64) (void)hipFree(c.w_wino4_n64);
     if (c.w_wino4_n32) (void)hipFree(c.w_wino4_n32);
     c.w_wino4_n64 = c.w_wino4_n32 = nullptr;
+    if (c.w_subpix) (void)hipFree(c.w_subpix);
+    c.w_subpix = nullptr;
     if (c.w_small) (void)hipFree(c.w_small);
     c.w_small = nullptr;
     if (c.w_taps) (void)hipFree(c.w_taps);
@@ -905,7 +915,7 @@
             Layer &L = s[i];
             const bool cat = (i == 0 && L.kind == L_RES && C0_first > 0);
             const int C0 = cat ? C0_first : L.c1.cin;
-            TRY(prep_conv(u, L.c1, L.kind == L_STEM ? L.c1.cin : C0, L.kind == L_STEM ? 1 : L.kind == L_DOWN ? 4 : 0));
+            TRY(prep_conv(u, L.c1, L.kind == L_STEM ? L.c1.cin : C0, L.kind == L_STEM ? 1 : L.kind == L_DOWN ? 4 : 0, L.kind == L_UP));
             if (L.kind == L_RES || L.kind == L_ATTN) TRY(prep_conv(u, L.c2, L.c2.cin, 0));
             if (L.kind == L_RES && L.has_skip) TRY(prep_conv(u, L.skip, cat ? C0_first : L.skip.cin, 0));
         }
@@ -1150,7 +1160,7 @@
     delete u;
 }
 
-extern "C" int dlpm_conv2d_f32(const dlpm_conv_args *a, float *scratch_dev, dlpm_stream_t stream) {
+static int conv2d_entry(const dlpm_conv_args *a, float *scratch_dev, float *stats_out, dlpm_stream_t stream) {
     DLPM_CHECK_ARG(a && a->src0 && a->weight && a->out && scratch_dev, "dlpm_conv2d_f32: null argument");
     DLPM_CHECK_ARG(a->ksize == 1 || a->ksize == 3, "dlpm_conv2d_f32: ksize must be 1 or 3");
     DLPM_CHECK_ARG(a->stride == 1 || a->stride == 2, "dlpm_conv2d_f32: stride must be 1 or 2");
@@ -1210,6 +1220,12 @@
                 return DLPM_ERR_UNSUPPORTED;
             }
             L.w_wino = nullptr;
+            used += wino4_weight_floats(a->Cout, a->C0 + a->C1);
+            if ((a->force_direct & 256) && a->upsample && a->Cout % 128 == 0 && a->scratch_floats >= used + subpix_weight_floats(a->Cout, a->C0 + a->C1)) {
+                float *wsp = scratch_dev + used;
+                TRY(relayout_weight_subpix4(a->weight, wsp, a->Cout, a->C0 + a->C1, st));
+                L.w_subpix = wsp;
+            }
         }
     }
     if ((a->force_direct & 64) && a->ksize == 3 && a->Cout <= 3 && a->C0 % 32 == 0 && a->C1 == 0) {
@@ -1242,8 +1258,24 @@
             if (head_conv_ok(L)) return launch_conv_head(L, nullptr, st);
         }
     }
+    if (stats_out) {
+        if (!ig || conv_stats_pixels(L) <= 0) {
+            set_error("dlpm_conv2d_stats_f32: this launch's kernel emits no fused statistics");
+            return DLPM_ERR_UNSUPPORTED;
+        }
+        L.stats_out = reinterpret_cast<float2 *>(stats_out);
+    }
     if (ig) return launch_conv_igemm(L, st);
     return (a->force_direct & 1) ? launch_conv_direct(L, st) : launch_conv_fallback(L, st);
+}
+
+extern "C" int dlpm_conv2d_f32(const dlpm_conv_args *a, float *scratch_dev, dlpm_stream_t stream) {
+    return conv2d_entry(a, scratch_dev, nullptr, stream);
+}
+
+extern "C" int dlpm_conv2d_stats_f32(const dlpm_conv_args *a, float *scratch_dev, float *stats_out, dlpm_stream_t stream) {
+    DLPM_CHECK_ARG(stats_out, "dlpm_conv2d_stats_f32: null stats_out");
+    return conv2d_entry(a, scratch_dev, stats_out, stream);
 }
 
 extern "C" int dlpm_groupnorm_coeffs_f32(const float *src0, const float *src1, int32_t C0, int32_t C1, int32_t B, int32_t HW,
diff --git a/include/dlpm_amd.h b/include/dlpm_amd.h
--- a/include/dlpm_amd.h
+++ b/include/dlpm_amd.h
@@ -237,6 +237,7 @@
 } dlpm_conv_args;
 
 int dlpm_conv2d_f32(const dlpm_conv_args *args, float *scratch_dev, dlpm_stream_t stream);
+int dlpm_conv2d_stats_f32(const dlpm_conv_args *args, float *scratch_dev, float *stats_out, dlpm_stream_t stream);
 
 int dlpm_groupnorm_coeffs_f32(const float *src0, const float *src1, int32_t C0, int32_t C1, int32_t B, int32_t HW,
                               int32_t groups, const float *gamma_dev, const float *beta_dev,
```

Result: no change. 27.96, median of 6 (+1.0%).
